# iden3/rapidsnark-old

Measured on AMD Instinct MI355X. Metric: Groth16 proofs/sec, higher is better.
Workload: dtype i64 (v_mad_i64_i32 column sums over 9x29-bit signed limbs, BN254 Fr/Fq)

## Files before the change

### include/zkhip.h

```cpp
#ifndef ZKHIP_H
#define ZKHIP_H

#include <stdint.h>
#include <stddef.h>

#ifdef __cplusplus
extern "C" {
#endif

typedef struct zk_prover zk_prover;

typedef struct zk_zkey_view {
    uint32_t nVars;
    uint32_t nPublic;
    uint32_t domainSize;
    uint64_t nCoefs;
    const void *vk_alpha1;
    const void *vk_beta1;
    const void *vk_beta2;
    const void *vk_delta1;
    const void *vk_delta2;
    const void *coefs;
    const void *pointsA;
    const void *pointsB1;
// ... 36 lines not shown

const char *zk_last_error(void);
int zk_device_count(int *count);

int zk_prover_create(zk_prover **out, const zk_zkey_view *zkey, const zk_opts *opts);
void zk_prover_destroy(zk_prover *p);

int zk_prove(zk_prover *p, const uint8_t *wtns, const uint8_t *r32, const uint8_t *s32, zk_proof *out);
int zk_prove_dev(zk_prover *p, const void *d_wtns, const uint8_t *r32, const uint8_t *s32, zk_proof *out);

#define ZK_MAX_IN_FLIGHT 8
int zk_prove_dev_submit(zk_prover *p, const void *d_wtns, const uint8_t *r32, const uint8_t *s32);
int zk_prove_submit(zk_prover *p, const uint8_t *wtns, const uint8_t *r32, const uint8_t *s32);
int zk_host_alloc(void **out, size_t bytes);
void zk_host_free(void *ptr);
int zk_prove_collect(zk_prover *p, zk_proof *out);
int zk_prover_reserve(zk_prover *p, uint32_t in_flight, uint32_t host_witnesses);
typedef struct zk_prover_plan {
    uint32_t size;
    uint32_t window_bits_h, windows_h;
    uint32_t window_bits_w, windows_w;
    uint32_t precomputed_tables;
    uint32_t msm_a_b1_c_one_launch;
    uint32_t lanes;
    uint32_t follow_up_streams;
    uint32_t max_in_flight;
    uint32_t depth_host_witness;
    uint32_t depth_resident_witness;
    uint32_t batch;
    uint32_t shard_index, shard_count, chain_partitioned;
    uint64_t device_bytes_in_use;
    uint64_t device_bytes_total;
    uint64_t kernel_launches_last_proof;
    uint32_t table_rows_h, table_rows_w;
    uint32_t bucket_sets_h, bucket_sets_w;
    uint32_t spmv_row_cut;
    uint32_t spmv_long_rows;
    uint32_t spmv_longest_row;
    uint32_t spmv_chunks;
} zk_prover_plan;
int zk_prover_info(zk_prover *p, zk_prover_plan *plan);
int zk_prove_msm_collect(zk_prover *p, zk_msm_sums *partial);
int zk_prove_batch_submit(zk_prover *p, const uint8_t *const *wtns, uint32_t count, const uint8_t *r32s, const uint8_t *s32s);
int zk_prove_batch_collect(zk_prover *p, zk_proof *out, uint32_t count);

int zk_prove_msm_dev(zk_prover *p, const void *d_wtns, zk_msm_sums *partial);
int zk_prove_msm(zk_prover *p, const uint8_t *wtns, zk_msm_sums *partial);
int zk_prove_finish(zk_prover *p, const zk_msm_sums *partials, uint32_t n_partials,
                    const uint8_t *r32, const uint8_t *s32, zk_proof *out);

typedef struct zk_multi_prover zk_multi_prover;
int zk_multi_prover_create(zk_multi_prover **out, const zk_zkey_view *zkey, const int32_t *devices, uint32_t n_devices,
                           const zk_opts *opts );
void zk_multi_prover_destroy(zk_multi_prover *mp);
int zk_multi_prove(zk_multi_prover *mp, const uint8_t *wtns, const uint8_t *r32, const uint8_t *s32, zk_proof *out);
int zk_multi_prove_submit(zk_multi_prover *mp, const uint8_t *wtns, const uint8_t *r32, const uint8_t *s32);
int zk_multi_prove_collect(zk_multi_prover *mp, zk_proof *out);
int zk_multi_prover_info(zk_multi_prover *mp, uint32_t *n_shards, uint32_t *chain_partitioned);
int zk_multi_prover_shard_info(zk_multi_prover *mp, uint32_t shard, zk_prover_plan *plan);
enum { ZK_STEP_CROSS_INVERSE = 1, ZK_STEP_LOCAL = 2, ZK_STEP_CROSS_FORWARD = 3, ZK_STEP_FINISH = 4 };
int zk_shard_info(zk_prover *p, uint64_t *block_elems, uint32_t *chain_partitioned);
int zk_shard_set_exchange(zk_prover *p, void *d_send, void *d_recv);
int zk_shard_begin(zk_prover *p, const uint8_t *wtns, const void *d_wtns, const uint8_t *r32, const uint8_t *s32, void *stream);
int zk_shard_step(zk_prover *p, int step, void *stream);

int zk_assemble(const void *vk_alpha1, const void *vk_beta1, const void *vk_beta2, const void *vk_delta1,
                const void *vk_delta2, const zk_msm_sums *partials, uint32_t n_partials,
                const uint8_t *r32, const uint8_t *s32, zk_proof *out);

enum {
    ZK_T_SPMV = 0, ZK_T_NTT, ZK_T_DIGITS_SORT, ZK_T_MSM_H, ZK_T_JOIN_WAIT, ZK_T_MSM_REDUCE,
    ZK_T_TOTAL_DEVICE, ZK_T_G1_L1_KERNEL, ZK_T_G2_L1_KERNEL, ZK_T_WTNS_H2D, ZK_T_COUNT
};
int zk_prover_timings(zk_prover *p, double *ms, uint32_t n);

int zk_fr_mul_vec(uint8_t *out, const uint8_t *a, const uint8_t *b, uint64_t n);
int zk_fq_mul_vec(uint8_t *out, const uint8_t *a, const uint8_t *b, uint64_t n);
int zk_fr_coef_accumulate(uint8_t *a, uint8_t *b, const void *coefs, uint64_t nCoefs, uint32_t domainSize,
                          const uint8_t *wtns, uint32_t nVars);
int zk_fr_ntt(uint8_t *data, uint64_t n, int inverse);
int zk_fr_abc_to_h(uint8_t *h, const uint8_t *a, const uint8_t *b, uint64_t n);
int zk_msm_g1(uint8_t out[64], const uint8_t *bases, const uint8_t *scalars, uint64_t n);
int zk_msm_g2(uint8_t out[128], const uint8_t *bases, const uint8_t *scalars, uint64_t n);

int zk_synth_chain_g1(uint8_t *out, uint64_t n, const uint8_t p0[64], const uint8_t q[64]);
int zk_synth_chain_g2(uint8_t *out, uint64_t n, const uint8_t p0[128], const uint8_t q[128]);
int zk_fixed_base_g1(uint8_t *out, const uint8_t base[64], const uint8_t *scalars, uint64_t n);
int zk_fixed_base_g2(uint8_t *out, const uint8_t base[128], const uint8_t *scalars, uint64_t n);
int zk_g1_mul(uint8_t out[64], const uint8_t p[64], const uint8_t k[32]);
int zk_g2_mul(uint8_t out[128], const uint8_t p[128], const uint8_t k[32]);

size_t zk_proof_to_json(const zk_proof *proof, char *buf, size_t cap);
size_t zk_public_to_json(const uint8_t *wtns, uint32_t nPublic, char *buf, size_t cap);

typedef struct zk_r1cs zk_r1cs;
typedef struct zk_r1cs_view {
    uint32_t nWires, nPubOut, nPubIn, nPrvIn, nConstraints;
    const void *constraints;
    uint64_t constraints_bytes;
} zk_r1cs_view;
typedef struct zk_r1cs_report {
    uint32_t size;
    uint64_t failed;
    uint32_t first_failed;
    uint8_t a[32], b[32], c[32];
    uint32_t one_ok;
    uint32_t first_unreduced;
} zk_r1cs_report;
int zk_r1cs_create(zk_r1cs **out, const zk_r1cs_view *v, int32_t device);
void zk_r1cs_destroy(zk_r1cs *r);
int zk_r1cs_check(zk_r1cs *r, const uint8_t *wtns, uint32_t nVars, zk_r1cs_report *rep);
int zk_r1cs_check_dev(zk_r1cs *r, const void *d_wtns, uint32_t nVars, zk_r1cs_report *rep);
int zk_r1cs_match_zkey(zk_r1cs *r, const zk_zkey_view *zkey, uint64_t *rows_differing, uint32_t *first_row);

typedef struct zk_ptau_view {
    uint32_t power;
    const void *alpha1, *beta1, *beta2;
    const void *lagrange_g1, *lagrange_g2, *lagrange_alpha_g1, *lagrange_beta_g1;
    uint64_t lagrange_g1_bytes, lagrange_g2_bytes, lagrange_alpha_g1_bytes, lagrange_beta_g1_bytes;
} zk_ptau_view;
typedef struct zk_setup_sizes {
    uint32_t nVars, nPublic, domainSize, log_domain;
    uint64_t nCoefs;
} zk_setup_sizes;
typedef struct zk_setup_out {
    uint8_t *coefs;
    uint8_t *pointsIC;
    uint8_t *pointsA;
    uint8_t *pointsB1;
    uint8_t *pointsB2;
    uint8_t *pointsC;
    uint8_t *pointsH;
} zk_setup_out;
int zk_groth16_setup_sizes(const zk_r1cs_view *r1cs, const zk_ptau_view *ptau, zk_setup_sizes *sizes);
int zk_groth16_setup(const zk_r1cs_view *r1cs, const zk_ptau_view *ptau, int32_t device, zk_setup_out *out);

int zk_g1_lagrange(uint8_t *out, const uint8_t *points, uint64_t n_points, uint32_t log_n, int32_t device);
int zk_g2_lagrange(uint8_t *out, const uint8_t *points, uint64_t n_points, uint32_t log_n, int32_t device);
typedef struct zk_ptau_powers_view {
    uint32_t power;
    const void *tau_g1, *tau_g2, *alpha_tau_g1, *beta_tau_g1;
    uint64_t tau_g1_bytes, tau_g2_bytes, alpha_tau_g1_bytes, beta_tau_g1_bytes;
} zk_ptau_powers_view;
typedef struct zk_ptau_lagrange_sizes {
    uint64_t lagrange_g1_bytes, lagrange_g2_bytes, lagrange_alpha_g1_bytes, lagrange_beta_g1_bytes;
    uint64_t device_bytes;
} zk_ptau_lagrange_sizes;
typedef struct zk_ptau_lagrange_out {
    uint8_t *lagrange_g1, *lagrange_g2, *lagrange_alpha_g1, *lagrange_beta_g1;
} zk_ptau_lagrange_out;
int zk_ptau_prepare_sizes(const zk_ptau_powers_view *ptau, zk_ptau_lagrange_sizes *sizes);
int zk_ptau_prepare(const zk_ptau_powers_view *ptau, int32_t device, zk_ptau_lagrange_out *out);

int zk_g1_scale(uint8_t *out, const uint8_t *points, uint64_t n, const uint8_t k[32], int32_t device);
#define ZK_SCALE_PLAN_MAX 130
int zk_g1_scale_plan(const uint8_t k[32], int8_t *digits_p, int8_t *digits_phi, uint32_t cap, uint32_t *len);
typedef struct zk_zkey_contrib_view {
    const void *vk_delta1;
    const void *vk_delta2;
    const void *pointsC;
    const void *pointsH;
    uint64_t pointsC_bytes, pointsH_bytes;
} zk_zkey_contrib_view;
typedef struct zk_zkey_contrib_sizes {
    uint64_t pointsC_bytes, pointsH_bytes;
    uint64_t chunk_points;
// ... 125 lines not shown
```

### rapidsnark-old_amd/csrc/hiputil.hpp

```cpp
#pragma once
#include <hip/hip_runtime.h>
#include <string.h>
#include <stdexcept>
#include <exception>
#include <string>
#include <thread>
#include <vector>

#include "../../include/zkhip.h"
#include "common.hpp"
#include "hipcheck.hpp"
#include "kernels.hpp"

using namespace zk;

namespace zkp {

#define HIP_TRY(expr) ZK_HIP(expr)

template <class T>
struct DevBuf {
    T *p = nullptr;
    size_t n = 0;
    DevBuf() {}
// ... 30 lines not shown
                (void)hipEventDestroy(done[i]);
            }
            if (pin[i]) (void)hipHostFree(pin[i]);
        }
    }
    void copy(void *dst, const void *src, size_t bytes) {
        if (!bytes) return;
        hipPointerAttribute_t attr;
        const bool pinned = hipPointerGetAttributes(&attr, src) == hipSuccess && attr.type == hipMemoryTypeHost;
        (void)hipGetLastError();
        if (pinned || bytes < ((size_t)4 << 20)) {
            HIP_TRY(hipMemcpyAsync(dst, src, bytes, hipMemcpyHostToDevice, s));
            return;
        }
        for (size_t off = 0; off < bytes; off += CHUNK, k ^= 1) {
            const size_t len = bytes - off < CHUNK ? bytes - off : CHUNK;
            if (!pin[k]) {
                HIP_TRY(hipHostMalloc((void **)&pin[k], CHUNK, hipHostMallocDefault));
                HIP_TRY(hipEventCreateWithFlags(&done[k], hipEventDisableTiming));
            } else {
                HIP_TRY(hipEventSynchronize(done[k]));
            }
            const uint8_t *from = (const uint8_t *)src + off;
            uint8_t *to = pin[k];
            const size_t nt = 4, per = (len / nt + 4095) & ~(size_t)4095;
            std::vector<std::thread> th;
            for (size_t t = 1; t < nt; t++) {
                const size_t lo = t * per, hi = lo + per < len ? lo + per : len;
                if (lo < hi) th.emplace_back([=] { memcpy(to + lo, from + lo, hi - lo); });
            }
            memcpy(to, from, per < len ? per : len);
            for (auto &t : th) t.join();
            HIP_TRY(hipMemcpyAsync((uint8_t *)dst + off, to, len, hipMemcpyHostToDevice, s));
            HIP_TRY(hipEventRecord(done[k], s));
        }
    }
};

struct Stream {
    hipStream_t s = nullptr;
    Stream() { HIP_TRY(hipStreamCreateWithFlags(&s, hipStreamNonBlocking)); }
    Stream(const Stream &) = delete;
    Stream &operator=(const Stream &) = delete;
    ~Stream() {
        (void)hipStreamSynchronize(s);
        (void)hipStreamDestroy(s);
    }
};

struct SortBufs {
    MsmPlan plan;
    uint64_t n = 0;
    DevBuf<uint16_t> lo;
    DevBuf<uint32_t> counts, starts, offsets, entries, codes, val, bin_counts, bin_starts;
    uint32_t total_buckets() const { return plan.sets * plan.nbuckets; }
    uint64_t max_entries() const { return (n ? n : 1) * plan.W; }
    void alloc(uint64_t n_, uint32_t window_bits, uint32_t precomp = 0, uint32_t batch = 1) {
        plan = make_msm_plan(n_ ? n_ : 1, window_bits, precomp, batch);
        n = n_ * (batch > 1 ? batch : 1);
        if ((n ? n : 1) * plan.W >= (1ull << 32)) throw std::invalid_argument("MSM too large: n * windows >= 2^32 sort entries");
        if ((n ? n : 1) * msm_table_rows(plan) >= (1ull << 31)) throw std::invalid_argument("MSM too large: table rows >= 2^31");
        MsmSortSizes z = msm_sort_sizes(n, plan);
        lo.alloc(z.lo_u16);
        counts.alloc(z.counts_u32);
        starts.alloc(z.starts_u32);
        offsets.alloc(z.offsets_u32);
        entries.alloc(z.entries_u32);
        codes.alloc(z.codes_u32);
        val.alloc(z.val_u32);
        bin_counts.alloc(z.bin_counts_u32);
        bin_starts.alloc(z.bin_starts_u32);
    }
    void release() {
        lo.release(); counts.release(); starts.release(); offsets.release(); entries.release();
        codes.release(); val.release(); bin_counts.release(); bin_starts.release();
        n = 0; ran = false;
    }
    size_t bytes() const {
        return lo.bytes() + counts.bytes() + starts.bytes() + offsets.bytes() + entries.bytes() + codes.bytes() + val.bytes()
             + bin_counts.bytes() + bin_starts.bytes();
    }
    bool ran = false;
    void run(const Fr *scalars, hipStream_t s) {
        static const bool skip = probe_env("ZKHIP_PROBE_SKIP_SORT") != nullptr;
        if (skip && ran) return;
        ran = true;
        MsmSortBufs b{offsets.p, entries.p, counts.p, starts.p, codes.p, val.p, bin_counts.p, bin_starts.p, lo.p};
        launch_msm_sort(b, scalars, n, plan, s);
    }
};

inline void need_device_count() {
    int ndev = 0;
    HIP_TRY(hipGetDeviceCount(&ndev));
    if (ndev <= 0) throw std::runtime_error("no HIP device available (libzkhip has no CPU fallback)");
}

inline int resolve_device(int32_t device) {
    need_device_count();
    int dev = device;
    if (dev < 0) HIP_TRY(hipGetDevice(&dev));
    return dev;
}

struct DeviceGuard {
    int prev = -1;
    explicit DeviceGuard(int dev) {
        if (hipGetDevice(&prev) != hipSuccess) prev = -1;
        HIP_TRY(hipSetDevice(dev));
    }
    ~DeviceGuard() {
        if (prev >= 0) (void)hipSetDevice(prev);
    }
};

inline void need_hbm(const char *who, uint64_t need) {
    size_t fr = 0, tot = 0;
    HIP_TRY(hipMemGetInfo(&fr, &tot));
    const uint64_t margin = need / 32 + ((uint64_t)256 << 20);
    if (fr < need + margin)
        throw HipError(std::string(who) + ": out of memory (needs " + std::to_string((need + margin) >> 20) + " MiB of HBM, " +
                       std::to_string(fr >> 20) + " MiB free)");
}

template <class Fn>
int guarded(Fn fn) {
    try {
        fn();
        return 0;
    } catch (const HipError &e) {
        set_error(std::string("HIP failure: ") + e.what());
        return 2;
    } catch (const std::exception &e) {
        set_error(e.what());
        return 1;
    }
}

inline uint32_t ilog2_exact(uint64_t n) {
    uint32_t l = 0;
    while ((1ull << l) < n) l++;
    if ((1ull << l) != n) throw std::invalid_argument("domainSize is not a power of two");
    return l;
}

inline uint32_t nblocks(uint64_t n, uint32_t b) { return (uint32_t)((n + b - 1) / b); }

inline void normalize(G1Affine *out, const G1XYZZ *tmp, Fq *pref, uint64_t n, hipStream_t s) { launch_normalize_g1(out, tmp, pref, n, s); }
inline void normalize(G2Affine *out, const G2XYZZ *tmp, Fq2 *pref, uint64_t n, hipStream_t s) { launch_normalize_g2(out, tmp, pref, n, s); }

}
using namespace zkp;
```

### rapidsnark-old_amd/csrc/kernels.hpp

```cpp
#pragma once
#include <hip/hip_runtime.h>
#include <stdint.h>
#include "field.hpp"
#include "curve.hpp"

namespace zk {

void launch_fr_mul_vec(Fr *out, const Fr *a, const Fr *b, uint64_t n, hipStream_t s);
void launch_fq_mul_vec(Fq *out, const Fq *a, const Fq *b, uint64_t n, hipStream_t s);

struct CsrDev {
    const uint32_t *rowptr;
    const uint32_t *col;
    const Fr *val;
    const uint4 *chunk_desc = nullptr;
    const uint4 *long_desc = nullptr;
    uint32_t chunks = 0, long_rows = 0, cut = 0;
};
constexpr uint32_t SPMV_LANE_TERMS = 16;
constexpr uint32_t SPMV_ROW_CUT = 16;
uint32_t spmv_row_cut();
void launch_spmv_abc(Fr *a, Fr *b, Fr *c, CsrDev csr, const Fr *wtns, uint32_t n, hipStream_t s, uint32_t vectors = 1, uint64_t abc_stride = 0,
                     uint64_t wtns_stride = 0, Fr *partials = nullptr);
void launch_csr_build(uint32_t *rowptr, uint32_t *col, Fr *val, uint32_t *cursor, uint32_t *err, const uint8_t *records,
                      uint64_t nCoefs, uint32_t n, uint32_t nVars, uint32_t row_lo, uint32_t row_hi, uint32_t row_cut, hipStream_t s);
void launch_csr_long_rows(uint4 *long_desc, uint4 *chunk_desc, uint32_t *counters, const uint32_t *rowptr, uint32_t rows, uint32_t row_cut,
                          uint32_t long_rows, uint32_t chunks, hipStream_t s);
void launch_exclusive_scan_u32(uint32_t *out, const uint32_t *counts, uint32_t total, hipStream_t s);

struct TwEntry {
    uint32_t l[12];
};
struct NttTables {
    uint32_t logn;
    const TwEntry *fwd;
    const TwEntry *inv;
    const Fr *coset;
    const Fr *ninv;
};
struct NttPair {
    uint32_t L = 0, Lg = 0, m = 0;
    uint32_t ngroups = 0, g[2] = {0, 0};
    TwEntry *rfwd = nullptr, *rinv = nullptr;
    Fr *tinv = nullptr, *tfwd = nullptr, *dtab = nullptr, *t2inv = nullptr, *t2fwd = nullptr;
    NttPair() {}
    NttPair(const NttPair &) = delete;
    NttPair &operator=(const NttPair &) = delete;
    ~NttPair() { release(); }
    void build(uint32_t logn_global, uint32_t logn_local, uint32_t block_index, hipStream_t s, bool plain = false);
    void release();
};
bool ntt_pair_supported(uint32_t local_logn);
void launch_ntt_coset_pair(Fr *data, uint64_t stride_elems, uint32_t batch, const NttPair &t, hipStream_t s);
void launch_ntt_plain(Fr *out, Fr *data, uint64_t stride_elems, uint32_t batch, const NttPair &t, bool inverse, hipStream_t s);

void launch_ntt_build_tables(TwEntry *fwd, TwEntry *inv, Fr *coset, Fr *ninv, uint32_t logn, hipStream_t s);
#define NTT_FULL 0xffffffffu
void launch_ntt_dif_inverse(Fr *data, uint64_t stride_elems, uint32_t batch, const NttTables &t, hipStream_t s, uint32_t local_logn = NTT_FULL);
void launch_ntt_dit_forward(Fr *data, uint64_t stride_elems, uint32_t batch, const NttTables &t, hipStream_t s, const Fr *premul = nullptr,
                            uint32_t local_logn = NTT_FULL);
void launch_ntt_cross(bool inverse, const Fr *xb, uint64_t in_src_stride, uint64_t in_poly_stride, Fr *const out_base[8],
                      uint64_t out_poly_stride, uint64_t out_offset, uint32_t batch,
                      const NttTables &t, uint32_t log_shards, uint32_t rank, hipStream_t s);
void launch_chunk_scatter(Fr *const xb_of_gpu[8], const Fr *blockdata, uint32_t batch, uint32_t logn, uint32_t log_shards, uint32_t rank,
                          hipStream_t s);
void launch_chunk_pack(Fr *packed, const Fr *blockdata, uint32_t batch, uint32_t logn, uint32_t log_shards, hipStream_t s);
void launch_chunk_unpack(Fr *blockdata, const Fr *packed, uint32_t batch, uint32_t logn, uint32_t log_shards, hipStream_t s);
void launch_fr_to_internal(Fr *x, uint64_t n, int times, hipStream_t s);
void launch_fr_from_internal(Fr *x, uint64_t n, hipStream_t s);
void launch_fr_scale_by_table(Fr *data, uint64_t stride_elems, uint32_t batch, const Fr *table, uint64_t n, hipStream_t s);
void launch_fr_scale_const(Fr *data, const Fr *k, uint64_t n, hipStream_t s);
void launch_bitrev_permute(Fr *data, uint32_t logn, hipStream_t s);
void launch_abc_to_h(Fr *h, const Fr *a, const Fr *b, const Fr *c, uint64_t n, hipStream_t s, uint32_t vectors = 1, uint64_t abc_stride = 0);

struct MsmPlan {
    uint32_t c;
    uint32_t W;
    uint32_t nbuckets;
    uint32_t sets;
    uint32_t precomp;
    uint32_t batch;
    uint32_t batch_n;
};
MsmPlan make_msm_plan(uint64_t n, uint32_t window_bits, uint32_t precomp = 0, uint32_t batch = 1);
inline uint32_t msm_table_rows(const MsmPlan &p) { return p.precomp ? (p.W + p.precomp - 1) / p.precomp : 1u; }

struct MsmSortSizes {
    uint64_t counts_u32, starts_u32, offsets_u32, entries_u32;
    uint64_t codes_u32, lo_u16, val_u32, bin_counts_u32, bin_starts_u32;
};
struct MsmSortBufs {
    uint32_t *offsets, *entries;
    uint32_t *counts, *starts;
    uint32_t *codes, *val, *bin_counts, *bin_starts;
    uint16_t *lo;
};
MsmSortSizes msm_sort_sizes(uint64_t n, MsmPlan p);
uint32_t msm_scan_extra_words(uint32_t total);
void launch_msm_sort(const MsmSortBufs &b, const Fr *scalars, uint64_t n, MsmPlan p, hipStream_t s);
void launch_msm_precomp_g1(G1Affine *table, G1XYZZ *tmp, Fq *pref, uint64_t n, MsmPlan p, hipStream_t s);
void launch_msm_precomp_g2(G2Affine *table, G2XYZZ *tmp, Fq2 *pref, uint64_t n, MsmPlan p, hipStream_t s);
struct alignas(16) G1Acc {
    int32_t l[36];
};
struct alignas(16) G2Acc {
    int32_t l[72];
};
uint64_t msm_accum_workspace_slots(uint64_t max_entries);
struct AccumTail {
    hipStream_t stream = nullptr;
    hipEvent_t l1_done = nullptr;
    bool buckets_zeroed = false;
    uint32_t chunk_min = 0;
    uint32_t chunk_max = 0;
};
struct AccumBatch {
    uint32_t n;
    const void *points[3];
    uint32_t idx_min[3], idx_sub[3];
    uint64_t bucket_stride, ws_stride;
    uint32_t gather_mask;
};
void launch_msm_accum_g1_batch(G1Acc *buckets, const uint32_t *offsets, const uint32_t *entries, const AccumBatch &batch, uint32_t total_buckets,
                               uint64_t max_entries, G1Acc *ws_part, uint32_t *ws_key, uint32_t *ws_flag, hipStream_t s, hipEvent_t *ev = nullptr,
                               AccumTail tail = AccumTail());
void launch_msm_accum_g1(G1Acc *buckets, const uint32_t *offsets, const uint32_t *entries, const G1Affine *points,
                         uint32_t idx_min, uint32_t idx_sub, uint32_t total_buckets, uint64_t max_entries,
                         G1Acc *ws_part, uint32_t *ws_key, uint32_t *ws_flag, hipStream_t s, hipEvent_t *ev = nullptr,
                         AccumTail tail = AccumTail());
void launch_msm_accum_g2(G2Acc *buckets, const uint32_t *offsets, const uint32_t *entries, const G2Affine *points,
                         uint32_t idx_min, uint32_t idx_sub, uint32_t total_buckets, uint64_t max_entries,
                         G2Acc *ws_part, uint32_t *ws_key, uint32_t *ws_flag, hipStream_t s, hipEvent_t *ev = nullptr,
                         AccumTail tail = AccumTail());
void launch_msm_reduce_g1(G1XYZZ *window_sums, G1Acc *scratch, const G1Acc *buckets, uint32_t n_msm, MsmPlan p, hipStream_t s);
void launch_msm_reduce_g2(G2XYZZ *window_sums, G2Acc *scratch, const G2Acc *buckets, uint32_t n_msm, MsmPlan p, hipStream_t s);
uint64_t msm_reduce_scratch_points(uint32_t n_msm, MsmPlan p);
uint32_t msm_wsum_rc(MsmPlan p);

void launch_fq_to_internal(Fq *coords, uint64_t n, hipStream_t s);

void launch_chain_g1(G1Affine *d_out, G1XYZZ *d_tmp, Fq *d_pref, const G1Affine &P0, const G1Affine &Q, uint64_t n, hipStream_t s);
void launch_chain_g2(G2Affine *d_out, G2XYZZ *d_tmp, Fq2 *d_pref, const G2Affine &P0, const G2Affine &Q, uint64_t n, hipStream_t s);
void launch_normalize_g1(G1Affine *d_out, const G1XYZZ *d_tmp, Fq *d_pref, uint64_t n, hipStream_t s);
void launch_normalize_g2(G2Affine *d_out, const G2XYZZ *d_tmp, Fq2 *d_pref, uint64_t n, hipStream_t s);
void launch_fixed_base_g1(G1Affine *d_out, G1XYZZ *d_tmp, Fq *d_pref, const G1Affine &B, const uint32_t *d_scalars, uint64_t n, hipStream_t s);
void launch_fixed_base_g2(G2Affine *d_out, G2XYZZ *d_tmp, Fq2 *d_pref, const G2Affine &B, const uint32_t *d_scalars, uint64_t n, hipStream_t s);

}
```

### rapidsnark-old_amd/csrc/msm_accum.hip

```cpp
#include <stdlib.h>
#include <string.h>
#include <algorithm>
#include "hipcheck.hpp"
#include "msm_lanes.hpp"

namespace zk {

#define ACC_CHUNK_MAX 160u
#define ACC_CHUNK_MIN 32u
__device__ __forceinline__ uint32_t accum_chunk_dev(uint32_t E, uint32_t nlanes, uint32_t chunk_min) {
    const uint32_t c = (uint32_t)(((uint64_t)E + nlanes - 1) / nlanes);
    return c < chunk_min ? chunk_min : c;
}
#ifdef ZK_PROBES
#define ZK_GATHER_ROW(i) ((i) & batch.gather_mask)
#else
#define ZK_GATHER_ROW(i) (i)
#endif
#define ACC_CHUNK_N 32u
#ifndef ZK_L1_BLOCK
#define ZK_L1_BLOCK 256
#endif
#ifndef ZK_L1_PREFETCH
#define ZK_L1_PREFETCH 1
// ... 274 lines not shown
        if (!__any(take)) break;
        XYZZ<FR> o{wave_up(v.x, d * LPE), wave_up(v.y, d * LPE), wave_up(v.zz, d * LPE), wave_up(v.zzz, d * LPE)};
        if (take) add(v, o);
    }
    if (e >= cnt) return;
    const uint32_t knext = __shfl_down(key, LPE);
    const uint32_t kbefore = __shfl_up(key, LPE);
    const bool last = e + 1 == cnt || knext != key;
    const bool first = e == 0 || kbefore != key;
    const uint64_t fmask = __ballot(first);
    const uint32_t start_lane = 63u - (uint32_t)__clzll(fmask & ((2ull << lane) - 1ull));
    const uint32_t sflag = (uint32_t)__shfl((int)flag, (int)start_lane);
    if (!last) return;
    const bool starts = (sflag & FLAG_STARTS) != 0, ends = (flag & FLAG_ENDS) != 0;
    if (starts && ends) {
        LM::store(buckets + key, v);
    } else if (!starts) {
        LM::store(out_part + 2 * (uint64_t)w, v);
        if (comp == 0) {
            out_key[2 * (uint64_t)w] = key;
            out_flag[2 * (uint64_t)w] = ends ? FLAG_ENDS : 0u;
        }
    } else {
        LM::store(out_part + 2 * (uint64_t)w + 1, v);
        if (comp == 0) {
            out_key[2 * (uint64_t)w + 1] = key;
            out_flag[2 * (uint64_t)w + 1] = FLAG_STARTS;
        }
    }
}

static inline uint32_t accum_chunk_min() {
    static const uint32_t cmin = [] { const char *e = probe_env("ZKHIP_ACC_CHUNK_MIN"); uint32_t v = e ? (uint32_t)atoi(e) : ACC_CHUNK_MIN; return v < 4u ? 4u : v; }();
    return cmin;
}
static inline uint32_t accum_chunk_max() {
    static const uint32_t cmax = [] { const char *e = probe_env("ZKHIP_ACC_CHUNK_MAX"); uint32_t v = e ? (uint32_t)atoi(e) : ACC_CHUNK_MAX; return v < 8u ? 8u : v; }();
    return cmax;
}
template <class F>
static uint64_t accum_round_lanes(uint32_t n_msm) {
    static const uint64_t threads = [] {
        int dev = 0, cus = 256, wgs = 0;
        hipError_t e = hipGetDevice(&dev);
        if (e == hipSuccess) e = hipDeviceGetAttribute(&cus, hipDeviceAttributeMultiprocessorCount, dev);
        if (e == hipSuccess) {
            if constexpr (sizeof(F) == sizeof(Fq2)) e = hipOccupancyMaxActiveBlocksPerMultiprocessor(&wgs, k_msm_accum_l1_g2s, ZK_L1_BLOCK, 0);
            else e = hipOccupancyMaxActiveBlocksPerMultiprocessor(&wgs, k_msm_accum_l1<F>, ZK_L1_BLOCK, 0);
        }
        if (e != hipSuccess || wgs < 1) { (void)hipGetLastError(); wgs = (sizeof(F) == sizeof(Fq2) ? 2 : 3) * (256 / ZK_L1_BLOCK); }
        if (const char *o = probe_env("ZKHIP_ACC_ROUND_WGS")) wgs = atoi(o) > 0 ? atoi(o) : wgs;
        return (uint64_t)wgs * (uint64_t)ZK_L1_BLOCK * (uint64_t)cus;
    }();
    uint64_t lanes = threads / LaneModel<F>::LPE / (n_msm ? n_msm : 1);
    return lanes ? lanes : 1;
}
template <class F>
static inline uint64_t accum_lanes_for(uint64_t max_entries, uint32_t n_msm, uint32_t chunk_min = 0, uint32_t chunk_max = 0) {
    if (!max_entries) max_entries = 1;
    const uint64_t R = accum_round_lanes<F>(n_msm), cmin = chunk_min ? chunk_min : accum_chunk_min(), cmax = chunk_max ? chunk_max : accum_chunk_max();
    if (max_entries <= R * cmin) return (max_entries + cmin - 1) / cmin;
    const uint64_t rounds = (max_entries + R * cmax - 1) / (R * cmax);
    return rounds * R;
}
uint64_t msm_accum_workspace_slots(uint64_t max_entries) {
    uint64_t lanes = accum_lanes_for<Fq>(max_entries, 1);
    for (uint32_t nb = 2; nb <= 3; nb++) lanes = std::max(lanes, accum_lanes_for<Fq>(max_entries, nb));
    lanes = std::max(lanes, accum_lanes_for<Fq2>(max_entries, 1));
    uint64_t total = 0;
    for (;;) {
        uint64_t slots = 2 * lanes;
        total += slots;
        if (lanes == 1) break;
        lanes = (slots + ACC_CHUNK_N - 1) / ACC_CHUNK_N;
    }
    return total;
}

template <class F>
static void launch_accum(ACCMEM *buckets, const uint32_t *offsets, const uint32_t *entries, AccumBatch batch,
                         uint32_t total_buckets, uint64_t max_entries,
                         ACCMEM *ws_part, uint32_t *ws_key, uint32_t *ws_flag, hipStream_t s, hipEvent_t *ev, AccumTail tail) {
    const uint32_t nb = batch.n ? batch.n : 1;
    if (!tail.buckets_zeroed) ZK_HIP(hipMemsetAsync(buckets, 0, ((size_t)(nb - 1) * batch.bucket_stride + total_buckets) * sizeof(ACCMEM), s));
    const uint32_t cmin = tail.chunk_min > accum_chunk_min() ? tail.chunk_min : accum_chunk_min();
    uint64_t lanes = accum_lanes_for<F>(max_entries, nb, cmin, tail.chunk_max > accum_chunk_max() ? tail.chunk_max : 0u);
    if (ev) ZK_HIP(hipEventRecord(ev[0], s));
    if constexpr (sizeof(F) == sizeof(Fq2)) {
        ZK_LAUNCH(k_msm_accum_l1_g2s, dim3((uint32_t)((2 * lanes + ZK_L1_BLOCK - 1) / ZK_L1_BLOCK)), dim3(ZK_L1_BLOCK), 0, s, buckets, offsets, entries,
                           reinterpret_cast<const G2Affine *>(batch.points[0]), batch.idx_min[0], batch.idx_sub[0], total_buckets, ws_part, ws_key, ws_flag,
                           (uint32_t)lanes, cmin);
    } else {
        ZK_LAUNCH(k_msm_accum_l1<F>, dim3((uint32_t)((lanes + ZK_L1_BLOCK - 1) / ZK_L1_BLOCK), nb), dim3(ZK_L1_BLOCK), 0, s, buckets, offsets, entries,
                           batch, total_buckets, ws_part, ws_key, ws_flag, (uint32_t)lanes, cmin);
    }
    if (ev) ZK_HIP(hipEventRecord(ev[1], s));
    if (skip_followups_probe()) return;
    if (tail.stream && tail.stream != s) {
        ZK_HIP(hipEventRecord(tail.l1_done, s));
        ZK_HIP(hipStreamWaitEvent(tail.stream, tail.l1_done, 0));
        s = tail.stream;
    }
    if (lanes > 1)
        ZK_LAUNCH(k_msm_accum_pair<F>, dim3((uint32_t)((lanes * LaneModel<F>::LPE + 255) / 256), nb), dim3(256), 0, s, buckets,
                           (const ACCMEM *)ws_part, ws_key, (const uint32_t *)ws_flag, (uint32_t)lanes, batch.bucket_stride, batch.ws_stride);
    uint64_t off = 0;
    while (lanes > 1) {
        uint64_t items = 2 * lanes;
        uint64_t noff = off + items;
        const uint64_t epw = 64u / LaneModel<F>::LPE;
        const uint64_t nl = (items + epw - 1) / epw;
        ZK_LAUNCH(k_msm_accum_wave<F>, dim3((uint32_t)((nl + 3) / 4), nb), dim3(256), 0, s, buckets, ws_part + off,
                           ws_key + off, ws_flag + off, (uint32_t)items, ws_part + noff, ws_key + noff, ws_flag + noff, (uint32_t)nl,
                           batch.bucket_stride, batch.ws_stride);
        off = noff;
        lanes = nl;
    }
    ZK_LAUNCH_OK("msm bucket accumulation");
}

static uint32_t gather_mask_env() {
    static const uint32_t m = [] { const char *e = probe_env("ZKHIP_GATHER_MASK"); return e ? (uint32_t)strtoul(e, nullptr, 0) : 0xffffffffu; }();
    return m;
}
static AccumBatch single(const void *points, uint32_t idx_min, uint32_t idx_sub) {
    AccumBatch b;
    memset(&b, 0, sizeof b);
    b.n = 1;
    b.gather_mask = gather_mask_env();
    b.points[0] = points;
    b.idx_min[0] = idx_min;
    b.idx_sub[0] = idx_sub;
    return b;
}

void launch_msm_accum_g1(G1Acc *buckets, const uint32_t *offsets, const uint32_t *entries, const G1Affine *points,
                         uint32_t idx_min, uint32_t idx_sub, uint32_t total, uint64_t max_entries, G1Acc *ws_part,
                         uint32_t *ws_key, uint32_t *ws_flag, hipStream_t s, hipEvent_t *ev, AccumTail tail) {
    launch_accum<Fq>(buckets, offsets, entries, single(points, idx_min, idx_sub), total, max_entries, ws_part, ws_key, ws_flag, s, ev, tail);
}
void launch_msm_accum_g1_batch(G1Acc *buckets, const uint32_t *offsets, const uint32_t *entries, const AccumBatch &batch, uint32_t total,
                               uint64_t max_entries, G1Acc *ws_part, uint32_t *ws_key, uint32_t *ws_flag, hipStream_t s, hipEvent_t *ev,
                               AccumTail tail) {
    AccumBatch b = batch;
    b.gather_mask = gather_mask_env();
    launch_accum<Fq>(buckets, offsets, entries, b, total, max_entries, ws_part, ws_key, ws_flag, s, ev, tail);
}
void launch_msm_accum_g2(G2Acc *buckets, const uint32_t *offsets, const uint32_t *entries, const G2Affine *points,
                         uint32_t idx_min, uint32_t idx_sub, uint32_t total, uint64_t max_entries, G2Acc *ws_part,
                         uint32_t *ws_key, uint32_t *ws_flag, hipStream_t s, hipEvent_t *ev, AccumTail tail) {
    launch_accum<Fq2>(buckets, offsets, entries, single(points, idx_min, idx_sub), total, max_entries, ws_part, ws_key, ws_flag, s, ev, tail);
}

}
```

### rapidsnark-old_amd/csrc/msm_reduce.hip

```cpp
#include <stdlib.h>
#include "hipcheck.hpp"
#include "msm_lanes.hpp"

namespace zk {

#define REDUCE_CHUNK 16u
#define REDUCE_THREADS 256u

template <class F>
__global__ __launch_bounds__(128) void k_msm_reduce_split(ACCMEM *A, uint32_t a_stride, ACCMEM *T, const ACCMEM *buckets, uint32_t nbuckets, uint32_t chunk, uint32_t L) {
    ZK_TAIL_PRIO();
    typedef LaneModel<F> LM;
    typedef typename LM::R FR;
    const uint32_t t = (blockIdx.x * blockDim.x + threadIdx.x) / LM::LPE;
    if (t >= L) return;
    const ACCMEM *B = buckets + (uint64_t)blockIdx.y * nbuckets + (uint64_t)t * chunk;
    XYZZ<FR> run = XYZZ<FR>::inf(), sum = XYZZ<FR>::inf();
    for (int j = (int)chunk - 1; j >= 0; j--) {
        add(run, LM::load(B + j));
        add(sum, run);
    }
    LM::store(A + (uint64_t)blockIdx.y * a_stride + t, sum);
    if (t == 0) run = XYZZ<FR>::inf();
    LM::store(T + (uint64_t)blockIdx.y * L + (t ? t - 1 : L - 1), run);
}

template <class F>
__global__ __launch_bounds__(128) void k_msm_reduce_chunks(ACCMEM *scratch, uint32_t out_stride, const ACCMEM *buckets, uint32_t nbuckets,
                                                           uint32_t chunk, uint32_t total_chunks) {
    ZK_TAIL_PRIO();
    typedef LaneModel<F> LM;
    typedef typename LM::R FR;
    uint32_t t = (blockIdx.x * blockDim.x + threadIdx.x) / LM::LPE;
    if (t >= total_chunks) return;
    const uint32_t chunks_per_window = nbuckets / chunk;
    const uint32_t cw = t % chunks_per_window;
    const ACCMEM *B = buckets + (uint64_t)t * chunk;
    XYZZ<FR> run = XYZZ<FR>::inf(), sum = XYZZ<FR>::inf();
    for (int j = (int)chunk - 1; j >= 0; j--) {
        add(run, LM::load(B + j));
        add(sum, run);
    }
    uint32_t k = cw * chunk;
    if (k) {
        XYZZ<FR> m = XYZZ<FR>::inf();
        for (int bit = 31 - __clz(k); bit >= 0; bit--) {
            m = dbl(m);
            if ((k >> bit) & 1u) add(m, run);
        }
        add(sum, m);
    }
    LM::store(scratch + (uint64_t)(t / chunks_per_window) * out_stride + cw, sum);
}

template <class F>
static constexpr uint32_t tree_in() { return 2u * REDUCE_THREADS / LaneModel<F>::LPE; }
#define TREE_IN_MIN REDUCE_THREADS
template <class F>
__global__ __launch_bounds__(REDUCE_THREADS) void k_msm_reduce_tree(ACCMEM *out, XYZZ<F> *out_final, const ACCMEM *in, uint32_t count, uint32_t last) {
    ZK_TAIL_PRIO();
    extern __shared__ uint32_t lds_raw[];
    typedef LaneModel<F> LM;
    typedef typename LM::R FR;
    constexpr uint32_t NE = REDUCE_THREADS / LM::LPE;
    XYZZ<FR> *lds = reinterpret_cast<XYZZ<FR> *>(lds_raw);
    const ACCMEM *X = in + (uint64_t)blockIdx.y * count;
    const uint32_t e = threadIdx.x / LM::LPE;
    const uint32_t i0 = blockIdx.x * (2u * NE) + e, i1 = i0 + NE;
    XYZZ<FR> acc = XYZZ<FR>::inf();
    if (i0 < count) acc = LM::load(X + i0);
    if (i1 < count) add(acc, LM::load(X + i1));
    lds[threadIdx.x] = acc;
    __syncthreads();
    for (uint32_t s = NE / 2; s > 0; s >>= 1) {
        if (e < s) {
            XYZZ<FR> o = lds[threadIdx.x + s * LM::LPE];
            add(acc, o);
            lds[threadIdx.x] = acc;
        }
        __syncthreads();
    }
    if (e == 0) {
        const uint64_t at = (uint64_t)blockIdx.y * gridDim.x + blockIdx.x;
        if (last) LM::store256(out_final + at, acc);
        else LM::store(out + at, acc);
    }
}

template <class F>
__global__ __launch_bounds__(REDUCE_THREADS) void k_msm_reduce_final2(XYZZ<F> *out_final, const ACCMEM *P, uint32_t cnt_x, uint32_t cnt_a, uint32_t scale_log) {
    ZK_TAIL_PRIO();
    extern __shared__ uint32_t lds_raw[];
    typedef LaneModel<F> LM;
    typedef typename LM::R FR;
    constexpr uint32_t H = REDUCE_THREADS / LM::LPE / 2;
    XYZZ<FR> *lds = reinterpret_cast<XYZZ<FR> *>(lds_raw);
    const uint32_t e = threadIdx.x / LM::LPE;
    const bool xs = e >= H;
    const uint32_t eh = xs ? e - H : e, cnt = xs ? cnt_x : cnt_a;
    const ACCMEM *in = P + (uint64_t)blockIdx.x * (cnt_x + cnt_a) + (xs ? 0u : cnt_x);
    XYZZ<FR> acc = XYZZ<FR>::inf();
    if (eh < cnt) acc = LM::load(in + eh);
// ... 57 lines not shown
        if (nblk == 1) LM::store256(final_out + (uint64_t)group * c + e, v);
        else LM::store(rec + ((uint64_t)group * nblk + blk) * BITS_RS + e, v);
    }
}
template <class F>
__global__ __launch_bounds__(REDUCE_THREADS) void k_msm_reduce_bits_top(XYZZ<F> *final_out, ACCMEM *rec, uint32_t nblk, uint32_t c) {
    ZK_TAIL_PRIO();
    typedef LaneModel<F> LM;
    typedef typename LM::R FR;
    constexpr uint32_t NE = REDUCE_THREADS / LM::LPE;
    constexpr uint32_t LB = LM::LPE == 1 ? 8u : 7u;
    const uint32_t e = threadIdx.x / LM::LPE;
    ACCMEM *R0 = rec + (uint64_t)blockIdx.x * nblk * BITS_RS;
#pragma unroll 1
    for (uint32_t m = LB; m + 1 < c; m++) {
        const uint32_t span = 1u << (m - LB), per = m + 2, ntasks = (nblk >> (m - LB + 1)) * per;
#pragma unroll 1
        for (uint32_t t = e; t < ntasks; t += NE) {
            const uint32_t g = t / per, i = t % per;
            ACCMEM *L = R0 + (uint64_t)g * 2u * span * BITS_RS, *R = L + (uint64_t)span * BITS_RS;
            if (i <= m) {
                XYZZ<FR> a = LM::load(L + i);
                add(a, LM::load(R + i));
                LM::store(L + i, a);
            } else {
                LM::store(L + m + 1, LM::load(R));
            }
        }
        __threadfence_block();
        __syncthreads();
    }
    if (e < c) LM::store256(final_out + (uint64_t)blockIdx.x * c + e, LM::load(R0 + e));
}
static inline bool reduce_bits_for(MsmPlan p) {
    static const int forced = [] { const char *e = probe_env("ZKHIP_REDUCE_BITS"); return e ? atoi(e) : -1; }();
    if (p.c > BITS_RS || (uint64_t)p.sets * p.nbuckets > (1u << 16)) return false;
    return forced < 0 ? true : forced != 0;
}
uint32_t msm_wsum_rc(MsmPlan p) { return reduce_bits_for(p) ? p.c : 1u; }

static inline uint32_t reduce_chunk_for(MsmPlan p) {
    static const uint32_t forced = [] { const char *e = probe_env("ZKHIP_REDUCE_CHUNK"); return e ? (uint32_t)atoi(e) : 0u; }();
    uint32_t chunk = REDUCE_CHUNK;
    if (forced) chunk = forced;
    else if ((uint64_t)p.sets * p.nbuckets <= (1u << 16)) chunk = 4;
    return p.nbuckets < chunk ? p.nbuckets : chunk;
}

#define REDUCE_SPLIT 16u
static inline uint32_t reduce_split_top(uint32_t L) {
    static const uint32_t forced = [] { const char *e = probe_env("ZKHIP_REDUCE_SPLIT_TOP"); const uint32_t t = e ? (uint32_t)atoi(e) : 0u; return t >= 2u && (t & (t - 1)) == 0 ? t : 0u; }();
    if (forced) return forced;
    return (L / 8u) % (2u * REDUCE_THREADS) == 0 ? 8u : 4u;
}
static inline uint32_t reduce_split_for(MsmPlan p) {
    static const int forced = [] { const char *e = probe_env("ZKHIP_REDUCE_SPLIT"); return e ? atoi(e) : -1; }();
    if (reduce_bits_for(p) || p.nbuckets < (1u << 14)) return 0;
    const uint32_t ch = forced >= 0 ? (uint32_t)forced : (p.nbuckets > (REDUCE_SPLIT << 15) ? p.nbuckets >> 15 : REDUCE_SPLIT);
    if (ch < 2 || (ch & (ch - 1)) != 0 || ch > p.nbuckets) return 0;
    const uint32_t L = p.nbuckets / ch;
    return L >= 8u && (L / reduce_split_top(L)) % (2u * REDUCE_THREADS) == 0 && L / TREE_IN_MIN <= REDUCE_THREADS / 2u ? ch : 0u;
}

static inline uint64_t tree_points(uint64_t groups, uint64_t cnt) {
    uint64_t total = 0;
    for (;;) {
        total += groups * cnt;
        if (cnt == 1) break;
        cnt = (cnt + TREE_IN_MIN - 1) / TREE_IN_MIN;
    }
    return total + groups;
}
uint64_t msm_reduce_scratch_points(uint32_t n_msm, MsmPlan p) {
    if (reduce_bits_for(p)) return (uint64_t)n_msm * p.sets * (p.nbuckets / 128u + 1u) * BITS_RS;
    const uint64_t groups = (uint64_t)n_msm * p.sets;
    if (const uint32_t ch = reduce_split_for(p)) {
        const uint64_t L = p.nbuckets / ch;
        return groups * L + tree_points(groups, L / reduce_split_top((uint32_t)L) + L);
    }
    return tree_points(groups, p.nbuckets / reduce_chunk_for(p));
}

template <class F>
static void launch_reduce(XYZZ<F> *window_sums, ACCMEM *scratch, const ACCMEM *buckets, uint32_t n_msm, MsmPlan p, hipStream_t s) {
    if (skip_followups_probe()) return;
    if (reduce_bits_for(p)) {
        const uint32_t NE = REDUCE_THREADS / LaneModel<F>::LPE, groups = n_msm * p.sets;
        const uint32_t nblk = p.nbuckets > NE ? p.nbuckets / NE : 1u;
        const size_t lds = REDUCE_THREADS * sizeof(XYZZ<typename LaneModel<F>::R>);
        ZK_LAUNCH(k_msm_reduce_bits_block<F>, dim3(nblk, groups), dim3(REDUCE_THREADS), lds, s, scratch, window_sums, buckets, p.nbuckets, p.c, nblk);
        if (nblk > 1) ZK_LAUNCH(k_msm_reduce_bits_top<F>, dim3(groups), dim3(REDUCE_THREADS), 0, s, window_sums, scratch, nblk, p.c);
        ZK_LAUNCH_OK("msm bucket reduction (bit sums)");
        return;
    }
    const uint32_t groups = n_msm * p.sets;
    const size_t lds = REDUCE_THREADS * sizeof(XYZZ<typename LaneModel<F>::R>);
    const uint32_t TREE_IN = tree_in<F>();
    auto chunks = [&](ACCMEM *out, uint32_t out_stride, const ACCMEM *in, uint32_t n, uint32_t chunk) {
        const uint32_t total_chunks = groups * (n / chunk);
        ZK_LAUNCH(k_msm_reduce_chunks<F>, dim3((total_chunks * LaneModel<F>::LPE + 127) / 128), dim3(128), 0, s, out, out_stride, in, n, chunk, total_chunks);
    };
    if (const uint32_t ch = reduce_split_for(p)) {
        const uint32_t L = p.nbuckets / ch, top = reduce_split_top(L), nx = L / top, per = nx + L;
        ACCMEM *T = scratch, *Y = T + (uint64_t)groups * L, *P = Y + (uint64_t)groups * per;
        ZK_LAUNCH(k_msm_reduce_split<F>, dim3((L * LaneModel<F>::LPE + 127) / 128, groups), dim3(128), 0, s, Y + nx, per, T, buckets, p.nbuckets, ch, L);
        chunks(Y, per, T, L, top);
        const uint32_t bx = nx / TREE_IN, ba = L / TREE_IN;
        ZK_LAUNCH(k_msm_reduce_tree<F>, dim3(bx + ba, groups), dim3(REDUCE_THREADS), lds, s, P, window_sums, (const ACCMEM *)Y, per, 0u);
        ZK_LAUNCH(k_msm_reduce_final2<F>, dim3(groups), dim3(REDUCE_THREADS), lds, s, window_sums, (const ACCMEM *)P, bx, ba, (uint32_t)__builtin_ctz(ch));
        ZK_LAUNCH_OK("msm bucket reduction (split)");
        return;
    }
    const uint32_t chunk = reduce_chunk_for(p);
    uint32_t cnt = p.nbuckets / chunk;
    chunks(scratch, cnt, buckets, p.nbuckets, chunk);
    ACCMEM *in = scratch;
    for (;;) {
        const uint32_t blocks = (cnt + TREE_IN - 1) / TREE_IN;
        const bool last = blocks == 1;
        ACCMEM *out = in + (uint64_t)groups * cnt;
        ZK_LAUNCH(k_msm_reduce_tree<F>, dim3(blocks, groups), dim3(REDUCE_THREADS), lds, s, out, window_sums, (const ACCMEM *)in, cnt, last ? 1u : 0u);
        if (last) break;
        in = out;
        cnt = blocks;
    }
    ZK_LAUNCH_OK("msm bucket reduction");
}
void launch_msm_reduce_g1(G1XYZZ *ws, G1Acc *scratch, const G1Acc *buckets, uint32_t n_msm, MsmPlan p, hipStream_t s) {
    launch_reduce<Fq>(ws, scratch, buckets, n_msm, p, s);
}
void launch_msm_reduce_g2(G2XYZZ *ws, G2Acc *scratch, const G2Acc *buckets, uint32_t n_msm, MsmPlan p, hipStream_t s) {
    launch_reduce<Fq2>(ws, scratch, buckets, n_msm, p, s);
}

}
```

### rapidsnark-old_amd/csrc/msm_sort.hip

```cpp
#include "kernels.hpp"
#include "hipcheck.hpp"
#include "common.hpp"
#include "devmem.hpp"
#include <string.h>

namespace zk {

MsmPlan make_msm_plan(uint64_t n, uint32_t window_bits, uint32_t precomp, uint32_t batch) {
    if (precomp > 2) throw std::invalid_argument("table mode: 0 (as in the zkey), 1 (a row per window) or 2 (a row per second window)");
    MsmPlan p;
    uint32_t lg = 0;
    while ((1ull << (lg + 1)) <= n) lg++;
    uint32_t c = window_bits;
    if (precomp) {
        if (c == 0) {
            c = lg > 2 ? lg - 2 : 2;
            if (lg == 20) c = 19;
            if (lg == 21) c = 20;
            if (batch > 1) c++;
            if (c > 20) c = 20;
        }
        if (c > 22) c = 22;
    } else {
        if (c == 0) c = lg > 6 ? lg - 6 : 2;
        if (c > 16) c = 16;
    }
    if (c < 2) c = 2;
    p.c = c;
    p.W = (256 + c - 1) / c;
    {
        const uint32_t W255 = (255 + c - 1) / c;
        if (W255 < p.W) {
            const uint32_t sh = (W255 - 1) * c;
            uint64_t top = 0;
            for (int k = 7; k >= 0; k--) {
                const int lo_bit = 32 * k;
                if (lo_bit + 32 <= (int)sh) break;
                const uint64_t w = FrParams::P[k];
                top |= lo_bit >= (int)sh ? w << (lo_bit - sh) : w >> (sh - lo_bit);
            }
            if (top + 1 < (1ull << (c - 1))) p.W = W255;
        }
    }
    p.nbuckets = 1u << (c - 1);
    p.precomp = precomp;
    p.sets = precomp ? precomp : p.W;
    p.batch = 1;
    p.batch_n = 0;
    if (batch > 1) {
        if (precomp != 1) throw std::invalid_argument("batched MSMs need window-precomputed tables with a row per window");
        p.batch = batch;
        p.batch_n = (uint32_t)n;
        p.sets = batch;
    }
    return p;
}

#define CODE32_ZERO 0x7FFFFFFFu
#ifndef SORT_THREADS
#define SORT_THREADS 1024u
#endif

__global__ __launch_bounds__(256) void k_msm_digits(uint32_t *digits, const Fr *scalars, uint64_t n, MsmPlan p) {
    ZK_CHAIN_PRIO();
    uint64_t st = (uint64_t)gridDim.x * blockDim.x;
    const uint32_t c = p.c, W = p.W;
    const uint32_t mask = (1u << c) - 1u, half = 1u << (c - 1);
    const uint32_t set_stride = p.precomp == 1 ? 0u : p.nbuckets, set_mask = p.precomp == 2 ? 1u : 0xffffffffu;
    for (uint64_t i = (uint64_t)blockIdx.x * blockDim.x + threadIdx.x; i < n; i += st) {
        Fr s = load_el(scalars + i);
        const uint32_t vec_base = p.batch > 1 ? (uint32_t)(i / p.batch_n) * p.nbuckets : 0u;
        for (int k = 0; k < 6; k++) {
            Fr d;
            u32 bw = 0;
#pragma unroll
            for (int j = 0; j < 8; j++) d.v[j] = subb(s.v[j], FrParams::P[j], bw);
            if (bw) break;
            s = d;
        }
        uint64_t buf = 0;
        uint32_t nb = 0, w = 0, carry = 0;
        auto emit = [&](uint32_t raw) {
            uint32_t d = raw + carry;
            const bool neg = d >= half;
            carry = neg ? 1u : 0u;
            uint32_t mag = neg ? (1u << c) - d : d;
            uint32_t code = mag ? ((mag - 1u + (w & set_mask) * set_stride + vec_base) | (neg ? 0x80000000u : 0u)) : CODE32_ZERO;
            digits[(uint64_t)w * n + i] = code;
            w++;
        };
#pragma unroll
        for (int k = 0; k < 8; k++) {
            buf |= (uint64_t)s.v[k] << nb;
            nb += 32;
            while (nb >= c && w + 1 < W) {
                emit((uint32_t)buf & mask);
                buf >>= c;
                nb -= c;
            }
        }
        emit((uint32_t)buf & mask);
    }
}

__global__ __launch_bounds__(256) void k_msm_compact_offsets(uint32_t *offsets, const uint32_t *starts, uint32_t total, uint32_t slices) {
    ZK_CHAIN_PRIO();
    uint32_t k = blockIdx.x * blockDim.x + threadIdx.x;
    if (k <= total) offsets[k] = starts[(uint64_t)k * slices];
}

#define BIN_MAX 256u

__global__ __launch_bounds__(SORT_THREADS) void k_bin_count(uint32_t *bin_counts, const uint32_t *codes, uint64_t total, uint32_t nbins,
                                                            uint32_t nblocks, uint32_t shift, uint32_t span) {
    ZK_CHAIN_PRIO();
    __shared__ uint32_t hist[BIN_MAX];
    if (threadIdx.x < BIN_MAX) hist[threadIdx.x] = 0;
    __syncthreads();
    const uint64_t base = (uint64_t)blockIdx.x * span;
    for (uint32_t k = threadIdx.x; k < span; k += SORT_THREADS) {
        uint64_t i = base + k;
        if (i < total) {
            uint32_t code = codes[i];
            if ((code & 0x7FFFFFFFu) != CODE32_ZERO) atomicAdd(&hist[(code & 0x7FFFFFFFu) >> shift], 1u);
        }
    }
    __syncthreads();
    if (threadIdx.x < nbins) bin_counts[(uint64_t)threadIdx.x * nblocks + blockIdx.x] = hist[threadIdx.x];
}

#define BIN_ITEMS 8u
__global__ __launch_bounds__(SORT_THREADS) void k_bin_scatter(uint16_t *lo, uint32_t *val, const uint32_t *bin_starts, const uint32_t *codes,
                                                              uint64_t total, uint32_t nbins, uint32_t nblocks, uint32_t shift, uint32_t span, uint64_t n,
                                                              uint32_t set_shift, uint32_t batch_n, uint32_t tstride) {
    ZK_CHAIN_PRIO();
    extern __shared__ uint32_t smem[];
    uint32_t *cnt = smem;
    uint32_t *gdelta = smem + BIN_MAX;
    uint32_t *st_dst = smem + 2 * BIN_MAX;
    uint32_t *st_val = st_dst + span;
    uint16_t *st_lo = (uint16_t *)(st_val + span);
    const uint32_t tid = threadIdx.x;
    if (tid < BIN_MAX) cnt[tid] = 0;
    __syncthreads();
    const uint64_t base = (uint64_t)blockIdx.x * span;
    const uint32_t lomask = (1u << shift) - 1u;
    const uint64_t w_base = tstride > 1 && n ? base / n : 0, r_base = tstride > 1 && n ? base - w_base * n : 0;
    uint32_t code[BIN_ITEMS], rank[BIN_ITEMS];
#pragma unroll
    for (uint32_t k = 0; k < BIN_ITEMS; k++) {
        uint64_t i = base + (uint64_t)k * SORT_THREADS + tid;
        code[k] = i < total ? codes[i] : CODE32_ZERO;
    }
#pragma unroll
    for (uint32_t k = 0; k < BIN_ITEMS; k++) {
        uint32_t mag = code[k] & 0x7FFFFFFFu;
        rank[k] = mag != CODE32_ZERO ? atomicAdd(&cnt[mag >> shift], 1u) : 0u;
    }
    __syncthreads();
    if (tid < 64) {
        uint32_t c0 = cnt[4 * tid], c1 = cnt[4 * tid + 1], c2 = cnt[4 * tid + 2], c3 = cnt[4 * tid + 3];
        uint32_t sum = c0 + c1 + c2 + c3, x = sum;
#pragma unroll
        for (int d = 1; d < 64; d <<= 1) {
            uint32_t y = __shfl_up(x, d);
            if (tid >= (uint32_t)d) x += y;
        }
        uint32_t off = x - sum;
        uint32_t o[4] = {off, off + c0, off + c0 + c1, off + c0 + c1 + c2};
#pragma unroll
        for (int q = 0; q < 4; q++) {
            uint32_t bin = 4 * tid + q;
            cnt[bin] = o[q];
            gdelta[bin] = bin < nbins ? bin_starts[(uint64_t)bin * nblocks + blockIdx.x] - o[q] : 0u;
        }
        if (tid == 63) smem[2 * BIN_MAX + 2 * span + span / 2] = x;
    }
    __syncthreads();
#pragma unroll
    for (uint32_t k = 0; k < BIN_ITEMS; k++) {
        uint32_t mag = code[k] & 0x7FFFFFFFu;
        if (mag != CODE32_ZERO) {
            uint32_t bin = mag >> shift, slot = cnt[bin] + rank[k];
            uint64_t i = base + (uint64_t)k * SORT_THREADS + tid - (uint64_t)(set_shift < 32 ? mag >> set_shift : 0u) * n;
            if (tstride > 1) {
                uint64_t w = w_base, r = r_base + (uint64_t)k * SORT_THREADS + tid;
                while (n && r >= n) { r -= n; w++; }
                i = (w / tstride) * n + r;
            }
            if (batch_n) {
                const uint64_t j = i / n, r = (i % n) % batch_n;
                i = j * batch_n + r;
            }
            st_dst[slot] = slot + gdelta[bin];
            st_val[slot] = (uint32_t)i | (code[k] & 0x80000000u);
            st_lo[slot] = (uint16_t)(mag & lomask);
        }
    }
    __syncthreads();
    const uint32_t kept = smem[2 * BIN_MAX + 2 * span + span / 2];
    for (uint32_t sidx = tid; sidx < kept; sidx += SORT_THREADS) {
        uint32_t d = st_dst[sidx];
        val[d] = st_val[sidx];
        lo[d] = st_lo[sidx];
    }
}

__device__ __forceinline__ bool bin_slice_of_block(uint32_t nbins, uint32_t slices, uint32_t &bin, uint32_t &slice) {
    const uint32_t xcd = blockIdx.x & 7u, k = blockIdx.x >> 3;
    bin = (k / slices) * 8u + xcd;
    slice = k % slices;
    return bin < nbins;
}

// ... 145 lines not shown
        }
#pragma unroll
        for (uint32_t k = 0; k < PER; k++) rank[k] = key[k] != 0xFFFFFFFFu ? atomicAdd(&loc[key[k]], 1u) : 0u;
        __syncthreads();
        const uint32_t c0 = loc[2 * tid], c1 = loc[2 * tid + 1];
        uint32_t total;
        const uint32_t ex = block_exclusive_scan(c0 + c1, scan_lds, total);
        __syncthreads();
        loc[2 * tid] = ex;
        loc[2 * tid + 1] = ex + c0;
        __syncthreads();
#pragma unroll
        for (uint32_t k = 0; k < PER; k++) {
            if (key[k] != 0xFFFFFFFFu) {
                const uint32_t pos = loc[key[k]] + rank[k];
                sval[pos] = v[k];
                slo[pos] = (uint16_t)key[k];
            }
        }
        __syncthreads();
        for (uint32_t p = tid; p < cnt; p += SCAN_BLOCK) {
            const uint32_t kk = slo[p];
            entries[gcur[kk] + (p - loc[kk])] = sval[p];
        }
        __syncthreads();
        const uint32_t a0 = loc[2 * tid], a1 = loc[2 * tid + 1], a2 = 2 * tid + 2 < 2048u ? loc[2 * tid + 2] : cnt;
        gcur[2 * tid] += a1 - a0;
        gcur[2 * tid + 1] += a2 - a1;
        __syncthreads();
    }
}

static void launch_scan(uint32_t *out, const uint32_t *counts, uint32_t total, hipStream_t s) {
    uint32_t nblocks = (total + SCAN_ELEMS - 1) / SCAN_ELEMS;
    uint32_t *block_sums = out + total + 1;
    ZK_LAUNCH(k_scan_local, dim3(nblocks), dim3(SCAN_BLOCK), 0, s, out, block_sums, counts, total);
    ZK_LAUNCH(k_scan_sums, dim3(1), dim3(SCAN_BLOCK), 0, s, block_sums, nblocks, out + total);
    ZK_LAUNCH(k_scan_add, dim3(nblocks), dim3(SCAN_BLOCK), 0, s, out, (const uint32_t *)block_sums, total);
}
uint32_t msm_scan_extra_words(uint32_t total) { return (total + SCAN_ELEMS - 1) / SCAN_ELEMS; }
void launch_exclusive_scan_u32(uint32_t *out, const uint32_t *counts, uint32_t total, hipStream_t s) { launch_scan(out, counts, total, s); }

#define BIN_SHIFT 11u
#define BIN_SLICES 32u
static inline uint32_t plan_total_buckets(MsmPlan p) { return p.sets * p.nbuckets; }
static inline uint32_t plan_bin_shift(MsmPlan p) {
    uint32_t sh = BIN_SHIFT;
    while (((plan_total_buckets(p) + (1u << sh) - 1) >> sh) > BIN_MAX) sh++;
    return sh;
}
static inline uint32_t plan_nbins(MsmPlan p) { uint32_t sh = plan_bin_shift(p); return (plan_total_buckets(p) + (1u << sh) - 1) >> sh; }
static inline uint32_t bin_span() { return BIN_ITEMS * SORT_THREADS; }
static inline uint32_t plan_bin_blocks(uint64_t n, MsmPlan p) { return (uint32_t)(((n ? n : 1) * p.W + bin_span() - 1) / bin_span()); }

MsmSortSizes msm_sort_sizes(uint64_t n, MsmPlan p) {
    MsmSortSizes z;
    memset(&z, 0, sizeof z);
    const uint64_t tb = plan_total_buckets(p), items = (n ? n : 1) * p.W;
    const uint64_t bb = (uint64_t)plan_nbins(p) * plan_bin_blocks(n, p);
    z.counts_u32 = tb * BIN_SLICES;
    z.starts_u32 = tb * BIN_SLICES + 1 + msm_scan_extra_words((uint32_t)(tb * BIN_SLICES));
    z.offsets_u32 = tb + 1;
    z.entries_u32 = items;
    z.codes_u32 = items;
    z.lo_u16 = items;
    z.val_u32 = items;
    z.bin_counts_u32 = bb;
    z.bin_starts_u32 = bb + 1 + msm_scan_extra_words((uint32_t)bb);
    return z;
}

static inline size_t bin_scatter_lds_bytes() { return (size_t)(2 * BIN_MAX + 2 * bin_span() + bin_span() / 2 + 1) * 4; }
static void sort_lds_attr() {
    static PerDeviceOnce attr;
    if (!attr.need()) return;
    ZK_HIP(hipFuncSetAttribute((const void *)k_bin_count_lds, hipFuncAttributeMaxDynamicSharedMemorySize, 160 * 1024));
    ZK_HIP(hipFuncSetAttribute((const void *)k_bin_scatter_lds, hipFuncAttributeMaxDynamicSharedMemorySize, 160 * 1024));
    ZK_HIP(hipFuncSetAttribute((const void *)k_bin_scatter, hipFuncAttributeMaxDynamicSharedMemorySize, 160 * 1024));
    ZK_HIP(hipFuncSetAttribute((const void *)k_bin_scatter_staged, hipFuncAttributeMaxDynamicSharedMemorySize, 160 * 1024));
    attr.done();
}

void launch_msm_sort(const MsmSortBufs &b, const Fr *scalars, uint64_t n, MsmPlan p, hipStream_t s) {
    const uint32_t tb = plan_total_buckets(p);
    sort_lds_attr();
    uint64_t g = (n + 255) / 256;
    if (g > 8192) g = 8192;
    const uint32_t sh = plan_bin_shift(p), nbins = plan_nbins(p), nblocks = plan_bin_blocks(n, p);
    uint32_t slices = BIN_SLICES;
    {
        const uint64_t per_bin = (n * p.W) / (nbins ? nbins : 1);
        while (slices > 4u && per_bin / slices < STAGE_CAP * 3u / 4u) slices >>= 1;
    }
    const uint32_t bpb = tb < (1u << sh) ? tb : (1u << sh);
    const uint64_t total = n * p.W;
    const size_t lds = (size_t)bpb * 4;
    const uint32_t grid2 = ((nbins + 7u) / 8u) * 8u * slices;
    const uint32_t set_shift = p.precomp ? 32u : p.c - 1u;
    if (n) ZK_LAUNCH(k_msm_digits, dim3((uint32_t)g), dim3(256), 0, s, b.codes, scalars, n, p);
    ZK_LAUNCH(k_bin_count, dim3(nblocks), dim3(SORT_THREADS), 0, s, b.bin_counts, (const uint32_t *)b.codes, total, nbins, nblocks, sh, bin_span());
    launch_scan(b.bin_starts, b.bin_counts, nbins * nblocks, s);
    ZK_LAUNCH(k_bin_scatter, dim3(nblocks), dim3(SORT_THREADS), bin_scatter_lds_bytes(), s, b.lo, b.val, (const uint32_t *)b.bin_starts,
                       (const uint32_t *)b.codes, total, nbins, nblocks, sh, bin_span(), n, set_shift, p.batch > 1 ? p.batch_n : 0u, p.precomp);
    ZK_LAUNCH(k_bin_count_lds, dim3(grid2), dim3(SORT_THREADS), lds, s, b.counts, (const uint16_t *)b.lo,
                       (const uint32_t *)b.bin_starts, nblocks, bpb, nbins, slices, tb);
    launch_scan(b.starts, b.counts, tb * slices, s);
    static const bool direct = probe_env("ZKHIP_SORT_DIRECT") != nullptr;
    if (bpb <= 2048u && SORT_THREADS == SCAN_BLOCK && !direct)
        ZK_LAUNCH(k_bin_scatter_staged, dim3(grid2), dim3(SCAN_BLOCK), (size_t)(4096 + 16 + STAGE_CAP) * 4 + (size_t)STAGE_CAP * 2, s, b.entries,
                           (const uint32_t *)b.starts, (const uint16_t *)b.lo, (const uint32_t *)b.val, (const uint32_t *)b.bin_starts, nblocks, bpb, nbins,
                           slices, tb);
    else
        ZK_LAUNCH(k_bin_scatter_lds, dim3(grid2), dim3(SORT_THREADS), lds, s, b.entries, (const uint32_t *)b.starts,
                           (const uint16_t *)b.lo, (const uint32_t *)b.val, (const uint32_t *)b.bin_starts, nblocks, bpb, nbins, slices, tb);
    ZK_LAUNCH(k_msm_compact_offsets, dim3((tb + 256) / 256), dim3(256), 0, s, b.offsets, (const uint32_t *)b.starts, tb, slices);
    ZK_LAUNCH_OK("msm sort");
}

}
```

### rapidsnark-old_amd/csrc/operators.hip

```cpp
#include <map>
#include <memory>
#include <mutex>
#include "hiputil.hpp"
#include "csr_long.hpp"

static void need_device() { need_device_count(); }

template <class F>
static void mul_vec(uint8_t *out, const uint8_t *a, const uint8_t *b, uint64_t n, void (*launch)(F *, const F *, const F *, uint64_t, hipStream_t)) {
    need_device();
    if (!n) return;
    DevBuf<F> da, db;
    da.alloc(n);
    db.alloc(n);
    da.upload(a, n, 0);
    db.upload(b, n, 0);
    launch(da.p, da.p, db.p, n, 0);
    HIP_TRY(hipMemcpy(out, da.p, n * 32, hipMemcpyDeviceToHost));
}

struct Tables {
    DevBuf<TwEntry> fwd, inv;
    DevBuf<Fr> coset, ninv;
    NttTables t;
// ... 154 lines not shown
    const uint64_t emax = sb.max_entries(), slots = msm_accum_workspace_slots(emax);
    ws.alloc(slots);
    wkey.alloc(slots);
    wflag.alloc(slots);
    buckets.alloc(sb.total_buckets());
    scratch.alloc(msm_reduce_scratch_points(1, sb.plan));
    const uint32_t rc = msm_wsum_rc(sb.plan);
    wsum.alloc((uint64_t)sb.plan.sets * rc);
    std::vector<uint8_t> w((size_t)sb.plan.sets * rc * sizeof(XT));
    if constexpr (sizeof(AffT) == 64) {
        launch_msm_accum_g1((G1Acc *)buckets.p, sb.offsets.p, sb.entries.p, (const G1Affine *)pts.p, 0, 0, sb.total_buckets(), emax, (G1Acc *)ws.p, wkey.p, wflag.p, 0);
        launch_msm_reduce_g1((G1XYZZ *)wsum.p, (G1Acc *)scratch.p, (const G1Acc *)buckets.p, 1, sb.plan, 0);
    } else {
        launch_msm_accum_g2((G2Acc *)buckets.p, sb.offsets.p, sb.entries.p, (const G2Affine *)pts.p, 0, 0, sb.total_buckets(), emax, (G2Acc *)ws.p, wkey.p, wflag.p, 0);
        launch_msm_reduce_g2((G2XYZZ *)wsum.p, (G2Acc *)scratch.p, (const G2Acc *)buckets.p, 1, sb.plan, 0);
    }
    HIP_TRY(hipMemcpy(w.data(), wsum.p, w.size(), hipMemcpyDeviceToHost));
    if (g2) HostTail::combine_windows_g2(w.data(), sb.plan.sets, sb.plan.c, rc, out);
    else HostTail::combine_windows_g1(w.data(), sb.plan.sets, sb.plan.c, rc, out);
}

template <class AffT, class XT, class FT>
static void synth_chain(uint8_t *out, uint64_t n, const uint8_t *p0, const uint8_t *q,
                        void (*launch)(AffT *, XT *, FT *, const AffT &, const AffT &, uint64_t, hipStream_t)) {
    need_device();
    if (!n) return;
    DevBuf<AffT> d_out;
    DevBuf<XT> d_tmp;
    DevBuf<FT> d_pref;
    d_out.alloc(n);
    d_tmp.alloc(n);
    d_pref.alloc(n);
    AffT P0, Q;
    memcpy(&P0, p0, sizeof(AffT));
    memcpy(&Q, q, sizeof(AffT));
    launch(d_out.p, d_tmp.p, d_pref.p, P0, Q, n, 0);
    HIP_TRY(hipMemcpy(out, d_out.p, n * sizeof(AffT), hipMemcpyDeviceToHost));
}

template <class AffT, class XT, class FT>
static void fixed_base_batch(uint8_t *out, const uint8_t *base, const uint8_t *scalars, uint64_t n,
                             void (*launch)(AffT *, XT *, FT *, const AffT &, const uint32_t *, uint64_t, hipStream_t)) {
    need_device();
    if (!n) return;
    if (!out || !base || !scalars) throw std::invalid_argument("null argument");
    DevBuf<AffT> d_out;
    DevBuf<XT> d_tmp;
    DevBuf<FT> d_pref;
    DevBuf<uint32_t> d_sc;
    d_out.alloc(n);
    d_tmp.alloc(n);
    d_pref.alloc(n);
    d_sc.alloc(n * 8);
    AffT B;
    memcpy(&B, base, sizeof(AffT));
    HIP_TRY(hipMemcpy(d_sc.p, scalars, n * 32, hipMemcpyHostToDevice));
    launch(d_out.p, d_tmp.p, d_pref.p, B, d_sc.p, n, 0);
    HIP_TRY(hipMemcpy(out, d_out.p, n * sizeof(AffT), hipMemcpyDeviceToHost));
}

extern "C" {

int zk_fixed_base_g1(uint8_t *out, const uint8_t base[64], const uint8_t *scalars, uint64_t n) {
    return guarded([&] { fixed_base_batch<G1Affine, G1XYZZ, Fq>(out, base, scalars, n, launch_fixed_base_g1); });
}
int zk_fixed_base_g2(uint8_t *out, const uint8_t base[128], const uint8_t *scalars, uint64_t n) {
    return guarded([&] { fixed_base_batch<G2Affine, G2XYZZ, Fq2>(out, base, scalars, n, launch_fixed_base_g2); });
}

int zk_synth_chain_g1(uint8_t *out, uint64_t n, const uint8_t p0[64], const uint8_t q[64]) {
    return guarded([&] { synth_chain<G1Affine, G1XYZZ, Fq>(out, n, p0, q, launch_chain_g1); });
}
int zk_synth_chain_g2(uint8_t *out, uint64_t n, const uint8_t p0[128], const uint8_t q[128]) {
    return guarded([&] { synth_chain<G2Affine, G2XYZZ, Fq2>(out, n, p0, q, launch_chain_g2); });
}

int zk_msm_g1(uint8_t out[64], const uint8_t *bases, const uint8_t *scalars, uint64_t n) {
    return guarded([&] { msm_generic<G1Affine, G1XYZZ, G1Acc>(out, bases, scalars, n, false); });
}
int zk_msm_g2(uint8_t out[128], const uint8_t *bases, const uint8_t *scalars, uint64_t n) {
    return guarded([&] { msm_generic<G2Affine, G2XYZZ, G2Acc>(out, bases, scalars, n, true); });
}

}
```

### rapidsnark-old_amd/csrc/prover_create.hip

```cpp
#include "prover_internal.hpp"

__attribute__((constructor)) static void zk_default_hw_queues() { setenv("GPU_MAX_HW_QUEUES", "16", 0); }

namespace zkp {

void alloc_slot(zk_prover *p, int i) {
    zk_prover::ProofSlot &q = p->slot[i];
    if (q.allocated) return;
    const uint64_t nv = p->sv.size();
    q.sort_w.alloc(nv, p->wbits, p->table_mode, p->batch);
    const MsmPlan pw = q.sort_w.plan, ph = p->sort_h.plan;
    const uint64_t tbw = q.sort_w.total_buckets(), tbh = p->sort_h.total_buckets();
    q.buckets_g1.alloc(3 * tbw + tbh);
    q.buckets_g2.alloc(tbw);
    q.scratch_g1.alloc(msm_reduce_scratch_points(3, pw) + msm_reduce_scratch_points(1, ph));
    const uint64_t ew = (uint64_t)pw.sets * msm_wsum_rc(pw), eh = (uint64_t)ph.sets * msm_wsum_rc(ph);
    q.wsum_g1.alloc(3 * ew + eh);
    q.scratch_g2.alloc(msm_reduce_scratch_points(1, pw));
    q.wsum_g2.alloc(ew);
    const uint64_t slots = msm_accum_workspace_slots(q.sort_w.max_entries()), slots_h = msm_accum_workspace_slots(p->sort_h.max_entries());
    q.acc_stride = slots;
    q.acc_ws_g1_all.alloc(3 * slots + slots_h);
    q.acc_ws_g2.alloc(slots);
    q.acc_key_all.alloc(4 * slots + slots_h);
    q.acc_flag_all.alloc(4 * slots + slots_h);
    if (p->csr_long.chunks) q.spmv_part.alloc((uint64_t)p->csr_long.chunks * p->batch);
    for (int m = 0; m < 5; m++) {
        const uint64_t at = m < 3 ? m * slots : (m == 3 ? 3 * slots : 3 * slots + slots_h);
        if (m < 4) q.acc_ws_g1[m] = q.acc_ws_g1_all.p + at;
        q.acc_key[m] = q.acc_key_all.p + at;
        q.acc_flag[m] = q.acc_flag_all.p + at;
    }
    q.w1_bytes = (size_t)(3 * ew + eh) * sizeof(G1XYZZ);
    q.w2_bytes = (size_t)ew * sizeof(G2XYZZ);
    if (!q.w1) HIP_TRY(hipHostMalloc((void **)&q.w1, q.w1_bytes, hipHostMallocDefault));
    if (!q.w2) HIP_TRY(hipHostMalloc((void **)&q.w2, q.w2_bytes, hipHostMallocDefault));
    for (auto &e : q.ev_l1)
        if (!e) HIP_TRY(hipEventCreateWithFlags(&e, hipEventDisableTiming));
    for (hipEvent_t *e : {&q.ev_fork, &q.ev_join, &q.ev_sortw, &q.ev_main, &q.ev_done, &q.ev_chain})
        if (!*e) HIP_TRY(hipEventCreateWithFlags(e, hipEventDisableTiming));
    for (auto &e : q.ev_tail)
        if (!e) HIP_TRY(hipEventCreateWithFlags(&e, hipEventDisableTiming));
    for (auto &e : q.ev)
        if (!e) HIP_TRY(hipEventCreate(&e));
    q.have_events = true;
    q.allocated = true;
}

void ensure_witness_buffer(zk_prover *p, zk_prover::ProofSlot &q) {
    if (!q.wtns_dev.p) q.wtns_dev.alloc((uint64_t)p->nVars * p->batch);
    if (!q.ev_h2d) HIP_TRY(hipEventCreateWithFlags(&q.ev_h2d, hipEventDisableTiming));
    if (!q.ev_h2d_start) HIP_TRY(hipEventCreate(&q.ev_h2d_start));
}

struct PhaseClock {
    bool on;
    std::chrono::steady_clock::time_point t;
    PhaseClock() : on(getenv("ZKHIP_VERBOSE") != nullptr), t(std::chrono::steady_clock::now()) {}
    void lap(const char *what, hipStream_t s) {
        if (!on) return;
        (void)hipStreamSynchronize(s);
        auto now = std::chrono::steady_clock::now();
        fprintf(stderr, "[zkhip] create: %-28s %8.1f ms\n", what, std::chrono::duration<double, std::milli>(now - t).count());
        t = now;
    }
};

void prover_create(zk_prover **out, const zk_zkey_view *z, const zk_opts *o) {
    if (!out || !z) throw std::invalid_argument("null argument");
    PhaseClock clk;
    const int dev = resolve_device(o ? o->device : -1);
    std::unique_ptr<zk_prover> p(new zk_prover());
    p->device = dev;
    DeviceGuard g(dev);
    p->flags = o ? o->flags : 0;
    p->shard_count = (o && o->shard_count > 1) ? o->shard_count : 1;
    p->shard_index = o ? o->shard_index : 0;
    p->batch = (o && o->batch > 1) ? o->batch : 1;
    if (p->batch > ZK_MAX_BATCH) throw std::invalid_argument("opts.batch > ZK_MAX_BATCH");
    if (p->flags & ZK_FLAG_PRECOMP_HALF) p->flags |= ZK_FLAG_PRECOMP;
    if (p->batch > 1 && (!(p->flags & ZK_FLAG_PRECOMP) || (p->flags & ZK_FLAG_PRECOMP_HALF) || p->shard_count != 1 || (p->flags & ZK_FLAG_PARTITIONED_CHAIN)))
        throw std::invalid_argument("opts.batch needs ZK_FLAG_PRECOMP (a row per window) on an unsharded prover");
    if (p->shard_index >= p->shard_count) throw std::invalid_argument("shard_index >= shard_count");
    const uint32_t wbits = o ? o->window_bits : 0;

    p->nVars = z->nVars;
    p->nPublic = z->nPublic;
    p->domainSize = z->domainSize;
    p->nCoefs = z->nCoefs;
    if (z->nVars == 0 || z->nPublic + 1 > z->nVars) throw std::invalid_argument("invalid nVars/nPublic");
    p->logn = ilog2_exact(z->domainSize);
    if (p->logn > 27) throw std::invalid_argument("domainSize exceeds 2^27: the coset needs a root of order 2*domainSize and BN254 Fr has 2-adicity 28");
    if (z->nCoefs >= (1ull << 32)) throw std::invalid_argument("nCoefs >= 2^32 is not supported (32-bit CSR positions)");
    const uint64_t n = z->domainSize, nV = z->nVars, nC = nV - z->nPublic - 1;
    if (z->coefs_bytes && z->coefs_bytes < 4 + z->nCoefs * 44) throw std::invalid_argument("zkey section 4 too small");
    if (z->pointsA_bytes && z->pointsA_bytes < nV * 64) throw std::invalid_argument("zkey section 5 too small");
    if (z->pointsB1_bytes && z->pointsB1_bytes < nV * 64) throw std::invalid_argument("zkey section 6 too small");
    if (z->pointsB2_bytes && z->pointsB2_bytes < nV * 128) throw std::invalid_argument("zkey section 7 too small");
    if (z->pointsC_bytes && z->pointsC_bytes < nC * 64) throw std::invalid_argument("zkey section 8 too small");
    if (z->pointsH_bytes && z->pointsH_bytes < n * 64) throw std::invalid_argument("zkey section 9 too small");
    memcpy(p->vk_alpha1, z->vk_alpha1, 64);
    memcpy(p->vk_beta1, z->vk_beta1, 64);
    memcpy(p->vk_beta2, z->vk_beta2, 128);
    memcpy(p->vk_delta1, z->vk_delta1, 64);
    memcpy(p->vk_delta2, z->vk_delta2, 128);

    {
        const char *e = probe_env("ZKHIP_S1_PRIO");
        const bool s1_hi = e ? atoi(e) != 0 : p->shard_count >= 2;
        if (s1_hi && !getenv("ZKHIP_SERIAL")) {
            int lo_pr = 0, hi_pr = 0;
            HIP_TRY(hipDeviceGetStreamPriorityRange(&lo_pr, &hi_pr));
            HIP_TRY(hipStreamCreateWithPriority(&p->stream, hipStreamNonBlocking, hi_pr));
        } else {
            HIP_TRY(hipStreamCreateWithFlags(&p->stream, hipStreamNonBlocking));
        }
    }
    struct SideStreams {
        std::thread th;
        std::exception_ptr err;
        ~SideStreams() {
            if (th.joinable()) th.join();
// ... 67 lines not shown
        if (nnz) up.copy(raw.p, (const uint8_t *)z->coefs + 4, nnz * 44);
        clk.lap("coefficient records upload", s);
        launch_csr_build(p->csr_rowptr.p, p->csr_col.p, p->csr_val.p, cursor.p, err.p, raw.p, nnz, z->domainSize, z->nVars,
                         p->part ? (uint32_t)p->sh.lo : 0u, p->part ? (uint32_t)p->sh.hi : z->domainSize, row_cut, s);
        launch_fr_to_internal(p->csr_val.p, nnz, 2, s);
        uint32_t bad[4] = {0, 0, 0, 0};
        HIP_TRY(hipMemcpyAsync(bad, err.p, 16, hipMemcpyDeviceToHost, s));
        HIP_TRY(hipStreamSynchronize(s));
        if (bad[0]) throw std::invalid_argument("zkey coefficient record out of range");
        p->csr_long.build(p->csr_rowptr.p, rows, row_cut, bad, s);
        clk.lap("CSR build (device)", s);
    }

    {
        const uint32_t local_logn = p->logn - p->log_shards_chain();
        const bool pair = ntt_pair_supported(local_logn) && !probe_env("ZKHIP_NTT_RADIX2");
        if (pair) p->pair.build(p->logn, local_logn, p->part ? p->shard_index : 0u, s);
        if (!pair || p->part) {
            p->tw_fwd.alloc(n > 1 ? n / 2 : 1);
            p->tw_inv.alloc(n > 1 ? n / 2 : 1);
            if (!pair) p->tw_coset.alloc(n);
            p->tw_ninv.alloc(1);
            launch_ntt_build_tables(p->tw_fwd.p, p->tw_inv.p, p->tw_coset.p, p->tw_ninv.p, p->logn, s);
        }
    }
    clk.lap("twiddle tables", s);

    const uint64_t nv = p->sv.size(), nh = p->sh.size();
    p->precomp = (p->flags & ZK_FLAG_PRECOMP) != 0;
    p->table_mode = (p->flags & ZK_FLAG_PRECOMP_HALF) ? 2u : p->precomp ? 1u : 0u;
    p->sort_h.alloc(nh, wbits, p->table_mode, p->batch);
    alloc_slot(p.get(), 0);
    const uint64_t rows_w = msm_table_rows(p->slot[0].sort_w.plan), rows_h = msm_table_rows(p->sort_h.plan);
    p->ptsA.alloc((nv ? nv : 1) * rows_w);
    p->ptsB1.alloc((nv ? nv : 1) * rows_w);
    p->ptsB2.alloc((nv ? nv : 1) * rows_w);
    p->ptsH.alloc((nh ? nh : 1) * rows_h);
    clk.lap("workspace allocation", s);
    up.copy(p->ptsA.p, (const uint8_t *)z->pointsA + p->sv.lo * 64, nv * 64);
    up.copy(p->ptsB1.p, (const uint8_t *)z->pointsB1 + p->sv.lo * 64, nv * 64);
    up.copy(p->ptsB2.p, (const uint8_t *)z->pointsB2 + p->sv.lo * 128, nv * 128);
    up.copy(p->ptsH.p, (const uint8_t *)z->pointsH + p->sh.lo * 64, nh * 64);
    {
        uint64_t first = z->nPublic + 1;
        uint64_t lo = p->sv.lo > first ? p->sv.lo : first;
        uint64_t hi = p->sv.hi > lo ? p->sv.hi : lo;
        uint64_t cnt = hi - lo;
        uint32_t skip = (uint32_t)(lo - p->sv.lo);
        if (p->precomp) {
            p->ptsC.alloc((nv ? nv : 1) * rows_w);
            HIP_TRY(hipMemsetAsync(p->ptsC.p, 0, (size_t)(nv ? nv : 1) * 64, s));
            if (cnt) up.copy(p->ptsC.p + skip, (const uint8_t *)z->pointsC + (lo - first) * 64, cnt * 64);
            p->c_idx_min = 0;
            launch_fq_to_internal((Fq *)p->ptsC.p, nv * 2, s);
        } else {
            p->c_idx_min = skip;
            p->ptsC.alloc(cnt ? cnt : 1);
            up.copy(p->ptsC.p, (const uint8_t *)z->pointsC + (lo - first) * 64, cnt * 64);
            launch_fq_to_internal((Fq *)p->ptsC.p, cnt * 2, s);
        }
    }
    launch_fq_to_internal((Fq *)p->ptsA.p, nv * 2, s);
    launch_fq_to_internal((Fq *)p->ptsB1.p, nv * 2, s);
    launch_fq_to_internal((Fq *)p->ptsB2.p, nv * 4, s);
    launch_fq_to_internal((Fq *)p->ptsH.p, nh * 2, s);
    clk.lap("point tables upload+convert", s);
    if (p->precomp) {
        const MsmPlan plan_w = p->slot[0].sort_w.plan;
        const uint64_t tw = (uint64_t)(rows_w - 1) * (nv ? nv : 1), th = (uint64_t)(rows_h - 1) * (nh ? nh : 1);
        const uint64_t tmax = tw > th ? tw : th;
        DevBuf<G2XYZZ> tmp;
        DevBuf<Fq2> pref;
        tmp.alloc(tmax ? tmax : 1);
        pref.alloc(tmax ? tmax : 1);
        launch_msm_precomp_g1(p->ptsA.p, (G1XYZZ *)tmp.p, (Fq *)pref.p, nv, plan_w, s);
        launch_msm_precomp_g1(p->ptsB1.p, (G1XYZZ *)tmp.p, (Fq *)pref.p, nv, plan_w, s);
        launch_msm_precomp_g1(p->ptsC.p, (G1XYZZ *)tmp.p, (Fq *)pref.p, nv, plan_w, s);
        launch_msm_precomp_g1(p->ptsH.p, (G1XYZZ *)tmp.p, (Fq *)pref.p, nh, p->sort_h.plan, s);
        launch_msm_precomp_g2(p->ptsB2.p, tmp.p, pref.p, nv, plan_w, s);
        HIP_TRY(hipStreamSynchronize(s));
    }

    p->abc.alloc(3 * p->nloc * p->batch);
    p->h.alloc(p->nloc * p->batch);
    if (p->part) p->xb.alloc(3 * p->nloc);
    p->abc_use = p->abc.p;
    p->xb_use = p->xb.p;
    {
        const char *e = getenv("ZKHIP_LANES");
        int lanes = e ? atoi(e) : (p->domainSize <= (1u << 17) && p->batch == 1 ? 8 : p->domainSize <= (1u << 22) ? 4 : 1);
        if (lanes < 1) lanes = 1;
        if (lanes > zk_prover::MAX_LANES) lanes = zk_prover::MAX_LANES;
        if (p->part || getenv("ZKHIP_SERIAL")) lanes = 1;
        for (int l = 1; l < lanes; l++) {
            auto x = std::make_unique<zk_prover::LaneExtra>();
            const char *ls = getenv("ZKHIP_LANE_STREAMS");
            x->one_stream = ls && atoi(ls) == 1;
            x->n_abc = 3 * p->nloc * p->batch;
            x->n_h = p->nloc * p->batch;
            x->nh_sort = nh;
            x->wbits = wbits;
            x->precomp = p->table_mode;
            x->batch = p->batch;
            p->extra[l - 1] = std::move(x);
        }
        p->lanes = lanes;
        const char *ge = getenv("ZKHIP_GRAPH");
        p->use_graph = ge && atoi(ge) != 0 && !p->part && p->batch == 1 && !(p->flags & ZK_FLAG_TIMINGS) && !getenv("ZKHIP_SERIAL");
    }
    HIP_TRY(hipStreamSynchronize(s));
    side.finish();
    clk.lap(p->precomp ? "window pre-computation" : "finish", s);
    *out = p.release();
}

}

extern "C" {

int zk_device_count(int *count) {
    return guarded([&] {
        int n = 0;
        HIP_TRY(hipGetDeviceCount(&n));
        *count = n;
    });
}

int zk_prover_create(zk_prover **out, const zk_zkey_view *zkey, const zk_opts *opts) {
    return guarded([&] { prover_create(out, zkey, opts); });
}

void zk_prover_destroy(zk_prover *p) {
    if (!p) return;
    int prev = -1;
    (void)hipGetDevice(&prev);
    (void)hipSetDevice(p->device);
    delete p;
    if (prev >= 0) (void)hipSetDevice(prev);
}

int zk_host_alloc(void **out, size_t bytes) {
    return guarded([&] {
        if (!out) throw std::invalid_argument("null argument");
        need_device_count();
        HIP_TRY(hipHostMalloc(out, bytes ? bytes : 1, hipHostMallocDefault));
    });
}

void zk_host_free(void *ptr) {
    if (ptr) (void)hipHostFree(ptr);
}

int zk_prover_reserve(zk_prover *p, uint32_t in_flight, uint32_t host_witnesses) {
    return guarded([&] {
        if (!p) throw std::invalid_argument("null argument");
        if (in_flight > ZK_MAX_IN_FLIGHT) throw std::invalid_argument("in_flight > ZK_MAX_IN_FLIGHT");
        std::lock_guard<std::mutex> lk(p->mtx);
        DeviceGuard g(p->device);
        const int nslots = in_flight >= 2 ? (int)std::min<uint32_t>(ZK_MAX_IN_FLIGHT, in_flight + 1) : 1;
        if (p->in_flight || p->phase_open >= 0) throw std::invalid_argument("proofs in flight");
        p->ring = nslots == 1 ? ZK_MAX_IN_FLIGHT : (uint32_t)nslots;
        p->next_submit = p->next_collect = 0;
        HIP_TRY(hipDeviceSynchronize());
        for (int i = nslots; i < (int)ZK_MAX_IN_FLIGHT; i++)
            p->slot[i].release_memory();
        for (int lane = nslots < 1 ? 1 : nslots; lane < p->lanes; lane++)
            if (p->extra[lane - 1]) p->extra[lane - 1]->release_memory();
        {
            const size_t slot_b = p->slot[0].device_bytes(), wtns_b = (size_t)p->nVars * sizeof(Fr) * p->batch;
            const size_t lane_b = p->abc.bytes() + p->h.bytes() + p->sort_h.bytes();
            size_t need = 0;
            for (int i = 0; i < nslots; i++) {
                if (!p->slot[i].allocated) need += slot_b;
                if (host_witnesses && !p->slot[i].wtns_dev.p) need += wtns_b;
            }
            for (int lane = 1; lane < p->lanes && lane < nslots; lane++)
                if (!p->extra[lane - 1]->ready) need += lane_b;
            if (need) need_hbm("zk_prover_reserve", need);
        }
        for (int i = 0; i < nslots; i++) {
            alloc_slot(p, i);
            if (host_witnesses) {
                zk_prover::ProofSlot &q = p->slot[i];
                ensure_witness_buffer(p, q);
                if (!q.wtns_pin) HIP_TRY(hipHostMalloc((void **)&q.wtns_pin, (size_t)p->nVars * 32 * p->batch, hipHostMallocDefault));
            }
        }
        for (int lane = 1; lane < p->lanes && lane < nslots; lane++) p->extra[lane - 1]->ensure();
    });
}

int zk_prover_info(zk_prover *p, zk_prover_plan *plan) {
    return guarded([&] {
        if (!p || !plan) throw std::invalid_argument("null argument");
        if (plan->size < 8 || plan->size > 4096) throw std::invalid_argument("zk_prover_plan.size not set");
        zk_prover_plan o;
        memset(&o, 0, sizeof o);
        const MsmPlan ph = p->sort_h.plan, pw = p->slot[0].sort_w.plan;
        o.window_bits_h = ph.c; o.windows_h = ph.W;
        o.window_bits_w = pw.c; o.windows_w = pw.W;
        o.precomputed_tables = p->table_mode;
        o.table_rows_h = msm_table_rows(ph); o.table_rows_w = msm_table_rows(pw);
        o.bucket_sets_h = ph.sets; o.bucket_sets_w = pw.sets;
        o.msm_a_b1_c_one_launch = p->batch_abc ? 1u : 0u;
        o.lanes = (uint32_t)p->lanes;
        o.follow_up_streams = (uint32_t)p->tail_streams;
        o.max_in_flight = ZK_MAX_IN_FLIGHT;
        const bool small = p->logn < 19, mid = p->logn <= 22 && p->shard_count == 1;
        o.depth_host_witness = small ? ZK_MAX_IN_FLIGHT : mid ? 6u : 3u;
        o.depth_resident_witness = small ? ZK_MAX_IN_FLIGHT : mid ? 6u : 2u;
        o.batch = p->batch;
        o.shard_index = p->shard_index; o.shard_count = p->shard_count; o.chain_partitioned = p->part ? 1u : 0u;
        {
            DeviceGuard g(p->device);
            size_t fr = 0, tot = 0;
            HIP_TRY(hipMemGetInfo(&fr, &tot));
            o.device_bytes_in_use = tot - fr; o.device_bytes_total = tot;
        }
        o.kernel_launches_last_proof = p->launches_last_proof;
        o.spmv_row_cut = p->csr_long.cut; o.spmv_long_rows = p->csr_long.long_rows;
        o.spmv_longest_row = p->csr_long.longest; o.spmv_chunks = p->csr_long.chunks;
        const uint32_t nb = plan->size < sizeof o ? plan->size : (uint32_t)sizeof o;
        o.size = nb;
        memcpy(plan, &o, nb);
    });
}

}
```

### rapidsnark-old_amd/csrc/prover_internal.hpp

```cpp
#pragma once
#include <hip/hip_runtime.h>
#include <string.h>
#include <stdio.h>
#include <stdlib.h>
#include <chrono>
#include <sys/random.h>
#include <string>
#include <vector>
#include <atomic>
#include <condition_variable>
#include <deque>
#include <map>
#include <mutex>
#include <thread>
#include <memory>
#include <stdexcept>
#include <exception>
#include <functional>

#include "../../include/zkhip.h"
#include "common.hpp"
#include "hipcheck.hpp"
#include "kernels.hpp"
#include "hiputil.hpp"
#include "csr_long.hpp"
#include "tail_pool.hpp"

namespace zkp {

struct Slice {
    uint64_t lo, hi;
    uint64_t size() const { return hi - lo; }
};
inline Slice shard_slice(uint64_t n, uint32_t idx, uint32_t cnt) {
    uint64_t per = (n + cnt - 1) / cnt;
    uint64_t lo = per * idx, hi = lo + per;
    if (lo > n) lo = n;
    if (hi > n) hi = n;
    return Slice{lo, hi};
}

}
using namespace zkp;

struct StageJob {
    uint8_t *dst;
    const uint8_t *src;
    size_t bytes;
};

struct zk_prover {
    int device = 0;
    uint32_t flags = 0;
    uint32_t nVars = 0, nPublic = 0, domainSize = 0, logn = 0;
    uint64_t nCoefs = 0;
    uint32_t shard_index = 0, shard_count = 1;
    uint8_t vk_alpha1[64], vk_beta1[64], vk_beta2[128], vk_delta1[64], vk_delta2[128];
    hipStream_t stream = nullptr, stream2 = nullptr;
    std::mutex mtx, cmtx, sync_mtx;

    DevBuf<uint32_t> csr_rowptr, csr_col;
    DevBuf<Fr> csr_val;
    CsrLong csr_long;
    DevBuf<TwEntry> tw_fwd, tw_inv;
    DevBuf<Fr> tw_coset, tw_ninv;
    NttPair pair;
    Slice sv, sh;
    uint32_t c_idx_min = 0;
    bool precomp = false;
    uint32_t table_mode = 0;
    DevBuf<G1Affine> ptsA, ptsB1, ptsC, ptsH;
    DevBuf<G2Affine> ptsB2;

    DevBuf<Fr> abc, h;
    SortBufs sort_h;
    struct ProofSlot {
        bool allocated = false, busy = false;
        bool use_tails = true;
        uint32_t l1_chunk_min = 0, l1_chunk_max = 0;
        SortBufs sort_w;
        DevBuf<G1Acc> buckets_g1;
        DevBuf<G2Acc> buckets_g2;
        DevBuf<G1Acc> scratch_g1, acc_ws_g1_all;
        G1Acc *acc_ws_g1[4] = {nullptr, nullptr, nullptr, nullptr};
        DevBuf<uint32_t> acc_key_all, acc_flag_all;
        uint32_t *acc_key[5] = {nullptr}, *acc_flag[5] = {nullptr};
        uint64_t acc_stride = 0;
        DevBuf<G2Acc> scratch_g2, acc_ws_g2;
        DevBuf<G1XYZZ> wsum_g1;
        DevBuf<G2XYZZ> wsum_g2;
        hipEvent_t ev_l1[5] = {nullptr, nullptr, nullptr, nullptr, nullptr};
        hipEvent_t ev_fork = nullptr, ev_join = nullptr, ev_sortw = nullptr, ev_main = nullptr, ev_done = nullptr, ev_chain = nullptr;
        bool zeroed = false;
        bool defer_w = false;
        hipEvent_t ev_tail[5] = {nullptr, nullptr, nullptr, nullptr, nullptr};
        hipEvent_t ev[20] = {};
        bool have_events = false;
        uint8_t *w1 = nullptr, *w2 = nullptr;
        size_t w1_bytes = 0, w2_bytes = 0;
        DevBuf<Fr> wtns_dev;
        DevBuf<Fr> spmv_part;
        uint8_t *wtns_pin = nullptr;
        uint8_t *pin_ring = nullptr;
        StageJob stage[ZK_MAX_BATCH];
        StageJob stage_chunk[16];
        hipEvent_t ev_h2d_b = nullptr;
        hipEvent_t ev_h2d = nullptr, ev_h2d_start = nullptr;
        uint8_t r32[ZK_MAX_BATCH][32], s32[ZK_MAX_BATCH][32];
        bool have_r = false, have_s = false;
        bool host_witness = false;
        uint32_t count = 1;
        hipGraph_t graph = nullptr;
        hipGraphExec_t gexec = nullptr;
        const Fr *graph_wtns = nullptr;
        hipEvent_t ev_gdone = nullptr;
        bool via_graph = false;
        size_t device_bytes() const {
            return sort_w.bytes() + buckets_g1.bytes() + buckets_g2.bytes() + scratch_g1.bytes() + acc_ws_g1_all.bytes() + acc_key_all.bytes()
                 + acc_flag_all.bytes() + scratch_g2.bytes() + acc_ws_g2.bytes() + wsum_g1.bytes() + wsum_g2.bytes() + spmv_part.bytes();
        }
        void release_memory() {
            allocated = false;
            sort_w.release();
            buckets_g1.release(); buckets_g2.release(); scratch_g1.release(); acc_ws_g1_all.release();
            acc_key_all.release(); acc_flag_all.release(); scratch_g2.release(); acc_ws_g2.release();
            wsum_g1.release(); wsum_g2.release(); wtns_dev.release(); spmv_part.release();
            if (w1) { (void)hipHostFree(w1); w1 = nullptr; }
            if (w2) { (void)hipHostFree(w2); w2 = nullptr; }
            if (wtns_pin) { (void)hipHostFree(wtns_pin); wtns_pin = nullptr; }
            if (pin_ring) { (void)hipHostFree(pin_ring); pin_ring = nullptr; }
            if (gexec) { (void)hipGraphExecDestroy(gexec); gexec = nullptr; }
            if (graph) { (void)hipGraphDestroy(graph); graph = nullptr; }
            graph_wtns = nullptr;
        }
        ~ProofSlot() {
            if (gexec) (void)hipGraphExecDestroy(gexec);
            if (graph) (void)hipGraphDestroy(graph);
            if (ev_gdone) (void)hipEventDestroy(ev_gdone);
            for (auto &e : ev_l1) if (e) (void)hipEventDestroy(e);
            for (hipEvent_t e : {ev_fork, ev_join, ev_sortw, ev_main, ev_done, ev_chain}) if (e) (void)hipEventDestroy(e);
            for (auto &e : ev_tail) if (e) (void)hipEventDestroy(e);
            for (auto &e : ev) if (e) (void)hipEventDestroy(e);
            if (w1) (void)hipHostFree(w1);
            if (w2) (void)hipHostFree(w2);
            if (wtns_pin) (void)hipHostFree(wtns_pin);
            if (pin_ring) (void)hipHostFree(pin_ring);
            if (ev_h2d) (void)hipEventDestroy(ev_h2d);
            if (ev_h2d_b) (void)hipEventDestroy(ev_h2d_b);
            if (ev_h2d_start) (void)hipEventDestroy(ev_h2d_start);
        }
    };
    ProofSlot slot[ZK_MAX_IN_FLIGHT];
    uint32_t next_submit = 0, next_collect = 0, in_flight = 0;
    uint32_t ring = ZK_MAX_IN_FLIGHT;
    uint32_t batch = 1;
    struct LaneExtra {
        hipStream_t stream = nullptr, stream2 = nullptr;
        DevBuf<Fr> abc, h;
        SortBufs sort_h;
        uint64_t n_abc = 0, n_h = 0, nh_sort = 0;
        uint32_t wbits = 0, batch = 1;
        uint32_t precomp = 0;
        bool one_stream = false;
        bool ready = false;
        void ensure() {
            if (ready) return;
            if (!stream) HIP_TRY(hipStreamCreateWithFlags(&stream, hipStreamNonBlocking));
            if (!stream2) {
                if (one_stream) stream2 = stream;
                else HIP_TRY(hipStreamCreateWithFlags(&stream2, hipStreamNonBlocking));
            }
            if (!abc.p) abc.alloc(n_abc);
            if (!h.p) h.alloc(n_h);
            sort_h.alloc(nh_sort, wbits, precomp, batch);
            ready = true;
        }
        void release_memory() {
            ready = false;
            abc.release(); h.release(); sort_h.release();
        }
        ~LaneExtra() {
            if (stream2 && stream2 != stream) { (void)hipStreamSynchronize(stream2); (void)hipStreamDestroy(stream2); }
            if (stream) { (void)hipStreamSynchronize(stream); (void)hipStreamDestroy(stream); }
        }
    };
    static constexpr int MAX_LANES = 8;
    std::unique_ptr<LaneExtra> extra[MAX_LANES - 1];
    int lanes = 1;
    uint32_t wbits = 0;
    bool part = false;
    uint32_t log_shards = 0;
    uint64_t nloc = 0;
    DevBuf<Fr> xb;
    Fr *abc_use = nullptr, *xb_use = nullptr;
    Fr *pk_use = nullptr;
    Fr *peer_abc[8] = {nullptr}, *peer_xb[8] = {nullptr};
    bool have_peers = false;
    int phase_open = -1, phase_next = 0;
    hipEvent_t ev_ext_in = nullptr, ev_ext_out = nullptr;
    uint32_t log_shards_chain() const { return part ? log_shards : 0; }
    hipStream_t tail_pool[5] = {nullptr, nullptr, nullptr, nullptr, nullptr};
    hipStream_t tail[5] = {nullptr, nullptr, nullptr, nullptr, nullptr};
    int tail_streams = 0;
    bool use_graph = false;
    bool capturing = false;
    bool batch_abc = false;
    hipStream_t stream_fin = nullptr;
    hipStream_t stream_h2d = nullptr;

    double timings[ZK_T_COUNT] = {0};
    uint32_t accum_launches = 0;
    uint64_t launches_at_front = 0, launches_last_proof = 0;

    ~zk_prover() {
        for (auto &x : extra)
            if (x && x->stream) { (void)hipStreamSynchronize(x->stream); (void)hipStreamSynchronize(x->stream2); }
        for (hipStream_t st : {stream_h2d, stream, stream2, tail_pool[0], tail_pool[1], tail_pool[2], tail_pool[3], tail_pool[4], stream_fin})
            if (st) (void)hipStreamSynchronize(st);
        if (ev_ext_in) (void)hipEventDestroy(ev_ext_in);
        if (ev_ext_out) (void)hipEventDestroy(ev_ext_out);
        if (stream_h2d) (void)hipStreamDestroy(stream_h2d);
        if (stream_fin) (void)hipStreamDestroy(stream_fin);
        for (hipStream_t st : tail_pool)
            if (st) (void)hipStreamDestroy(st);
        if (stream2 && stream2 != stream) (void)hipStreamDestroy(stream2);
        if (stream) (void)hipStreamDestroy(stream);
    }
};

namespace zkp {

void prover_create(zk_prover **out, const zk_zkey_view *z, const zk_opts *o);
void alloc_slot(zk_prover *p, int i);
void ensure_witness_buffer(zk_prover *p, zk_prover::ProofSlot &q);

struct BatchIn {
    const uint8_t *const *wtns;
    uint32_t count;
    const uint8_t *r32s, *s32s;
};
void stage_job_run(void *arg);
int phase_front(zk_prover *p, const Fr *d_wtns, const uint8_t *h_wtns, const uint8_t *r32, const uint8_t *s32, hipEvent_t src_ready = nullptr,
                const BatchIn *bi = nullptr);
void phase_cross_push(zk_prover *p, hipEvent_t pushed);
void phase_cross_run(zk_prover *p, bool inverse, hipEvent_t done);
void phase_local(zk_prover *p);
void phase_back(zk_prover *p);
struct PhaseAbort {
    zk_prover *p;
    bool armed = true;
    ~PhaseAbort() { if (armed) p->phase_open = -1; }
};
struct SubmittedRS {
    uint8_t r32[32], s32[32];
    bool have_r = false, have_s = false;
};
struct DirectProof {
    zk_proof *out;
    const uint8_t *r32, *s32;
    bool use_submitted;
    uint32_t count = 1;
};
void collect_sums(zk_prover *p, zk_msm_sums *out, SubmittedRS *rs = nullptr, const DirectProof *direct = nullptr);
void prove_finish(zk_prover *p, const zk_msm_sums *parts, uint32_t nparts, const uint8_t *r32, const uint8_t *s32, zk_proof *out);

}
```

### rapidsnark-old_amd/csrc/prover_pipeline.hip

```cpp
#include "prover_internal.hpp"

namespace {
struct StagePool {
    struct Seg { uint8_t *dst; const uint8_t *src; size_t len; std::atomic<int> *left; };
    std::mutex m;
    std::condition_variable cv, done;
    std::deque<Seg> q;
    std::vector<std::thread> th;
    bool stop = false;
    StagePool() {
        for (int i = 0; i < 4; i++) th.emplace_back([this] { run(); });
    }
    ~StagePool() {
        {
            std::lock_guard<std::mutex> lk(m);
            stop = true;
        }
        cv.notify_all();
        for (auto &t : th) t.join();
    }
    void run() {
        for (;;) {
            Seg s;
            {
// ... 31 lines not shown
        memcpy(dst + mine_lo, src + mine_lo, mine_hi - mine_lo);
        if (nseg > 1) {
            std::unique_lock<std::mutex> lk(m);
            done.wait(lk, [&] { return left.load() == 0; });
        }
    }
};
StagePool &stage_pool() {
    static StagePool *pool = new StagePool();
    return *pool;
}
}
void zkp::stage_job_run(void *arg) {
    const StageJob *j = (const StageJob *)arg;
    stage_pool().copy(j->dst, j->src, j->bytes);
}
static const Fr *upload_witnesses(zk_prover *p, zk_prover::ProofSlot &q, const uint8_t *const *h_wtns, uint32_t count,
                                  hipEvent_t src_ready = nullptr, const Fr *d_src = nullptr) {
    const size_t bytes = (size_t)p->nVars * 32;
    ensure_witness_buffer(p, q);
    hipStream_t sh = p->stream_h2d;
    if (src_ready) HIP_TRY(hipStreamWaitEvent(sh, src_ready, 0));
    const bool tm = (p->flags & ZK_FLAG_TIMINGS) != 0;
    for (uint32_t k = 0; k < count; k++) {
        uint8_t *dst = (uint8_t *)q.wtns_dev.p + (size_t)k * bytes;
        if (d_src) {
            if (tm && k == 0) HIP_TRY(hipEventRecord(q.ev_h2d_start, sh));
            HIP_TRY(hipMemcpyAsync(dst, d_src, bytes, hipMemcpyDeviceToDevice, sh));
            continue;
        }
        hipPointerAttribute_t attr;
        const bool pinned = hipPointerGetAttributes(&attr, h_wtns[k]) == hipSuccess && attr.type == hipMemoryTypeHost;
        (void)hipGetLastError();
        const uint8_t *src = h_wtns[k];
        if (!pinned) {
            if (count == 1 && bytes >= ((size_t)4 << 20) && p->in_flight == 0) {
                const size_t npc = bytes >= ((size_t)32 << 20) ? 8 : 4, per = ((bytes / npc) + 4095) & ~(size_t)4095;
                if (!q.wtns_pin && !q.pin_ring) HIP_TRY(hipHostMalloc((void **)&q.pin_ring, 2 * per, hipHostMallocDefault));
                if (!q.ev_h2d_b) HIP_TRY(hipEventCreateWithFlags(&q.ev_h2d_b, hipEventDisableTiming));
                hipStream_t sb = p->stream_fin;
                if (src_ready) HIP_TRY(hipStreamWaitEvent(sb, src_ready, 0));
                HIP_TRY(hipEventRecord(q.ev_h2d_b, sh));
                HIP_TRY(hipStreamWaitEvent(sb, q.ev_h2d_b, 0));
                if (tm) HIP_TRY(hipEventRecord(q.ev_h2d_start, sh));
                for (size_t c = 0, off = 0; off < bytes; c++, off += per) {
                    const size_t len = off + per < bytes ? per : bytes - off;
                    hipStream_t st = (c & 1) ? sb : sh;
                    uint8_t *stg = q.wtns_pin ? q.wtns_pin + off : q.pin_ring + (c & 1) * per;
                    q.stage_chunk[c] = StageJob{stg, h_wtns[k] + off, len};
                    HIP_TRY(hipLaunchHostFunc(st, stage_job_run, &q.stage_chunk[c]));
                    HIP_TRY(hipMemcpyAsync(dst + off, stg, len, hipMemcpyHostToDevice, st));
                }
                HIP_TRY(hipEventRecord(q.ev_h2d_b, sb));
                HIP_TRY(hipStreamWaitEvent(sh, q.ev_h2d_b, 0));
                continue;
            }
            if (!q.wtns_pin) HIP_TRY(hipHostMalloc((void **)&q.wtns_pin, bytes * p->batch, hipHostMallocDefault));
            q.stage[k] = StageJob{q.wtns_pin + (size_t)k * bytes, h_wtns[k], bytes};
            static const bool sync_stage = probe_env("ZKHIP_STAGE_SYNC") != nullptr;
            if (sync_stage) stage_job_run(&q.stage[k]);
            else HIP_TRY(hipLaunchHostFunc(sh, stage_job_run, &q.stage[k]));
            src = q.stage[k].dst;
        }
        if (tm && k == 0) HIP_TRY(hipEventRecord(q.ev_h2d_start, sh));
        HIP_TRY(hipMemcpyAsync(dst, src, bytes, hipMemcpyHostToDevice, sh));
    }
    if (count < p->batch) HIP_TRY(hipMemsetAsync((uint8_t *)q.wtns_dev.p + (size_t)count * bytes, 0, (size_t)(p->batch - count) * bytes, sh));
    HIP_TRY(hipEventRecord(q.ev_h2d, sh));
    if (tm) HIP_TRY(hipEventRecord(q.ev[12], sh));
    return q.wtns_dev.p;
}
static const Fr *upload_witness(zk_prover *p, zk_prover::ProofSlot &q, const uint8_t *h_wtns, hipEvent_t src_ready = nullptr) {
    return upload_witnesses(p, q, &h_wtns, 1, src_ready);
}

namespace {

struct PhaseCtx {
    zk_prover *p;
    zk_prover::ProofSlot &q;
    hipStream_t s, s2, sf;
    hipStream_t tail[5] = {nullptr, nullptr, nullptr, nullptr, nullptr};
    int ntails = 0;
    Fr *abc, *h;
    SortBufs *sort_h;
    bool tm;
    uint32_t tbw, tbh, Ww;
    uint64_t ew, eh;
    MsmPlan pw;
    G1Acc *bA, *bB1, *bC, *bH;
    PhaseCtx(zk_prover *p_, int si) : p(p_), q(p_->slot[si]) {
        const int lane = si % p->lanes;
        if (lane == 0) {
            s = p->stream; s2 = p->stream2; sf = p->stream_fin;
            if (q.use_tails) {
                for (int m = 0; m < 5; m++) tail[m] = p->tail[m];
                ntails = p->tail_streams;
            }
            abc = p->abc_use; h = p->h.p; sort_h = &p->sort_h;
        } else {
            zk_prover::LaneExtra &x = *p->extra[lane - 1];
            x.ensure();
            s = x.stream; s2 = x.stream2; sf = x.stream;
            abc = x.abc.p; h = x.h.p; sort_h = &x.sort_h;
        }
        tm = (p->flags & ZK_FLAG_TIMINGS) != 0;
        tbw = q.sort_w.total_buckets(); tbh = p->sort_h.total_buckets();
        ew = q.sort_w.max_entries(); eh = p->sort_h.max_entries();
        pw = q.sort_w.plan; Ww = pw.sets * msm_wsum_rc(pw);
        bA = q.buckets_g1.p; bB1 = bA + tbw; bC = bB1 + tbw; bH = bC + tbw;
    }
    void mark(int i) const { if (tm) HIP_TRY(hipEventRecord(q.ev[i], s)); }
    AccumTail tail_of(int m) const { AccumTail t; t.stream = tail[m]; t.l1_done = q.ev_l1[m]; t.buckets_zeroed = q.zeroed; t.chunk_min = q.l1_chunk_min; t.chunk_max = q.l1_chunk_max; return t; }
    hipStream_t after(int m, hipStream_t own) const { return tail[m] ? tail[m] : own; }
    NttTables tables() const { return NttTables{p->logn, p->tw_fwd.p, p->tw_inv.p, p->tw_coset.p, p->tw_ninv.p}; }
};


static bool lone_order(const zk_prover *p) {
    static const int forced = [] { const char *e = probe_env("ZKHIP_LONE_ORDER"); return e ? atoi(e) : -1; }();
    return forced > 0 && p->shard_count == 1 && !p->part;
}

static void enqueue_witness_msms(zk_prover *p, PhaseCtx &c) {
    zk_prover::ProofSlot &q = c.q;
    hipStream_t s2 = c.s2;
    const bool tails = c.ntails != 0;
    const bool tm = c.tm;
    const uint32_t tbw = c.tbw, Ww = c.Ww;
    const uint64_t ew = c.ew;
    const MsmPlan pw = c.pw;
    static const uint32_t g2_aside_maxlog = [] { const char *e = probe_env("ZKHIP_G2_ASIDE_MAXLOG"); return e ? (uint32_t)atoi(e) : 21u; }();
    const bool g2_aside = !tails && c.sf != s2 && c.sf != c.s && p->in_flight == 0 && !p->capturing && !p->use_graph &&
                          p->sv.size() <= ((uint64_t)1 << g2_aside_maxlog);
    AccumTail t4 = c.tail_of(4);
    if (g2_aside) t4.stream = c.sf;
    launch_msm_accum_g2(q.buckets_g2.p, q.sort_w.offsets.p, q.sort_w.entries.p, p->ptsB2.p, 0, 0, tbw, ew, q.acc_ws_g2.p, q.acc_key[4], q.acc_flag[4], s2, tm ? &q.ev[10] : nullptr, t4);
    if (tails) launch_msm_reduce_g2(q.wsum_g2.p, q.scratch_g2.p, q.buckets_g2.p, 1, pw, c.tail[4]);
    else if (g2_aside) launch_msm_reduce_g2(q.wsum_g2.p, q.scratch_g2.p, q.buckets_g2.p, 1, pw, c.sf);
    if (p->batch_abc) {
        AccumBatch b;
        memset(&b, 0, sizeof b);
        b.n = 3;
        b.points[0] = p->ptsA.p; b.points[1] = p->ptsB1.p; b.points[2] = p->ptsC.p;
        static const bool one_table = probe_env("ZKHIP_PROBE_ONE_TABLE") != nullptr;
        if (one_table) b.points[1] = b.points[2] = p->ptsA.p;
        b.idx_min[2] = b.idx_sub[2] = p->c_idx_min;
        b.bucket_stride = tbw;
        b.ws_stride = q.acc_stride;
        launch_msm_accum_g1_batch(c.bA, q.sort_w.offsets.p, q.sort_w.entries.p, b, tbw, ew, q.acc_ws_g1[0], q.acc_key[0], q.acc_flag[0], s2, tm ? &q.ev[8] : nullptr, c.tail_of(0));
        if (tm) for (int e : {13, 14, 15, 16}) HIP_TRY(hipEventRecord(q.ev[e], s2));
        launch_msm_reduce_g1(q.wsum_g1.p, q.scratch_g1.p, c.bA, 3, pw, c.after(0, s2));
        if (!tails && !g2_aside) launch_msm_reduce_g2(q.wsum_g2.p, q.scratch_g2.p, q.buckets_g2.p, 1, pw, s2);
        HIP_TRY(hipEventRecord(q.ev_join, s2));
    } else {
    launch_msm_accum_g1(c.bA, q.sort_w.offsets.p, q.sort_w.entries.p, p->ptsA.p, 0, 0, tbw, ew, q.acc_ws_g1[0], q.acc_key[0], q.acc_flag[0], s2, tm ? &q.ev[8] : nullptr, c.tail_of(0));
    if (tails) launch_msm_reduce_g1(q.wsum_g1.p, q.scratch_g1.p, c.bA, 1, pw, c.tail[0]);
    launch_msm_accum_g1(c.bB1, q.sort_w.offsets.p, q.sort_w.entries.p, p->ptsB1.p, 0, 0, tbw, ew, q.acc_ws_g1[1], q.acc_key[1], q.acc_flag[1], s2, tm ? &q.ev[13] : nullptr, c.tail_of(1));
    if (tails) {
        launch_msm_reduce_g1(q.wsum_g1.p + Ww, q.scratch_g1.p + msm_reduce_scratch_points(1, pw), c.bB1, 1, pw, c.tail[1]);
    } else {
        if (!g2_aside) launch_msm_reduce_g2(q.wsum_g2.p, q.scratch_g2.p, q.buckets_g2.p, 1, pw, s2);
        launch_msm_reduce_g1(q.wsum_g1.p, q.scratch_g1.p, c.bA, 2, pw, s2);
    }
    HIP_TRY(hipEventRecord(q.ev_join, s2));
    }

}

}

namespace zkp {

int phase_front(zk_prover *p, const Fr *d_wtns, const uint8_t *h_wtns, const uint8_t *r32, const uint8_t *s32, hipEvent_t src_ready, const BatchIn *bi) {
    DeviceGuard g(p->device);
    if (p->in_flight >= p->ring) throw std::invalid_argument("too many proofs in flight (ZK_MAX_IN_FLIGHT, or the depth given to zk_prover_reserve): collect one first");
    if (p->phase_open >= 0) throw std::invalid_argument("a proof is still being submitted phase by phase");
    if (p->in_flight == 0 && !p->capturing) p->next_submit = p->next_collect = 0;
    const int si = (int)(p->next_submit % p->ring);
    alloc_slot(p, si);
    if (!p->capturing) p->slot[si].use_tails = p->in_flight > 0 || p->use_graph;
    if (!p->capturing) {
        static const uint32_t thr_min = [] { const char *e = probe_env("ZKHIP_L1_CHUNK_MIN_BUSY"); return e ? (uint32_t)atoi(e) : 128u; }();
        static const uint32_t thr_log = [] { const char *e = probe_env("ZKHIP_L1_CHUNK_MIN_BUSY_LOG"); return e ? (uint32_t)atoi(e) : 17u; }();
        static const uint32_t thr_max = [] { const char *e = probe_env("ZKHIP_L1_CHUNK_MAX_BUSY"); return e ? (uint32_t)atoi(e) : 1280u; }();
        static const bool shards_too = [] { const char *e = probe_env("ZKHIP_L1_BUSY_SHARDS"); return e ? atoi(e) != 0 : true; }();
        uint32_t lg_sh = 0;
        while ((1u << (lg_sh + 1)) <= p->shard_count) lg_sh++;
        const bool busy = p->in_flight > 0 && !p->use_graph && ((p->shard_count == 1 && !p->part) || shards_too) && p->batch == 1 && p->logn >= thr_log + lg_sh;
        p->slot[si].l1_chunk_min = busy ? thr_min : 0u;
        p->slot[si].l1_chunk_max = busy ? thr_max : 0u;
    }
    PhaseCtx c(p, si);
    zk_prover::ProofSlot &q = c.q;
    if (!p->capturing) p->launches_at_front = g_kernel_launches.load(std::memory_order_relaxed);
    bool staged = h_wtns != nullptr;
    q.count = 1;
    if (bi) {
        if (bi->count < 1 || bi->count > p->batch) throw std::invalid_argument("batch submission: between 1 and opts.batch witnesses");
        d_wtns = upload_witnesses(p, q, bi->wtns, bi->count, src_ready);
        staged = true;
        q.count = bi->count;
        r32 = bi->r32s;
        s32 = bi->s32s;
    } else if (staged) {
        d_wtns = upload_witness(p, q, h_wtns, src_ready);
    } else if (p->batch > 1) {
        d_wtns = upload_witnesses(p, q, nullptr, 1, src_ready, d_wtns);
        staged = true;
    }
    q.host_witness = h_wtns != nullptr || bi != nullptr;
    q.have_r = r32 != nullptr;
    q.have_s = s32 != nullptr;
    if (r32) memcpy(q.r32, r32, (size_t)32 * q.count);
    if (s32) memcpy(q.s32, s32, (size_t)32 * q.count);
    hipStream_t s = c.s, s2 = c.s2;
    const bool tails = c.ntails != 0;
    const bool tm = c.tm;

    c.mark(0);
    q.zeroed = !p->capturing && !p->use_graph;
    if (q.zeroed) {
        HIP_TRY(hipMemsetAsync(c.bA, 0, (size_t)3 * c.tbw * sizeof(G1Acc), s2));
        HIP_TRY(hipMemsetAsync(q.buckets_g2.p, 0, (size_t)c.tbw * sizeof(G2Acc), s2));
        HIP_TRY(hipMemsetAsync(c.bH, 0, (size_t)c.tbh * sizeof(G1Acc), s));
    }
    if (staged) {
        HIP_TRY(hipStreamWaitEvent(s, q.ev_h2d, 0));
        HIP_TRY(hipStreamWaitEvent(s2, q.ev_h2d, 0));
    }
    if (p->capturing && s2 != s) {
        HIP_TRY(hipEventRecord(q.ev_fork, s));
        HIP_TRY(hipStreamWaitEvent(s2, q.ev_fork, 0));
    }
    q.sort_w.run(d_wtns + p->sv.lo, s2);
    HIP_TRY(hipEventRecord(q.ev_sortw, s2));
    q.defer_w = lone_order(p) && !p->capturing && !p->use_graph && p->in_flight == 0 && s2 != s;
    if (!q.defer_w) enqueue_witness_msms(p, c);

    const uint64_t nl = p->nloc;
    Fr *abc = c.abc;
    const CsrDev csr = p->csr_long.view(p->csr_rowptr.p, p->csr_col.p, p->csr_val.p);
    launch_spmv_abc(abc, abc + nl, abc + 2 * nl, csr, d_wtns, (uint32_t)nl, s, q.count, 3 * nl, p->nVars, q.spmv_part.p);
    c.mark(1);
    if (p->part && !p->have_peers && p->pk_use) launch_chunk_pack(p->pk_use, abc, 3, p->logn, p->log_shards, s);
    p->phase_open = si;
    p->phase_next = p->part ? 1 : 2;
    return si;
}

void phase_cross_push(zk_prover *p, hipEvent_t pushed) {
    DeviceGuard g(p->device);
    launch_chunk_scatter(p->peer_xb, p->abc_use, 3, p->logn, p->log_shards, p->shard_index, p->stream);
    HIP_TRY(hipEventRecord(pushed, p->stream));
}
void phase_cross_run(zk_prover *p, bool inverse, hipEvent_t done) {
    if (p->phase_open < 0 || p->phase_next != (inverse ? 1 : 3)) throw std::invalid_argument("chain phases out of order");
    DeviceGuard g(p->device);
    PhaseCtx c(p, p->phase_open);
    const uint64_t nl = p->nloc, chunk = nl >> p->log_shards;
    if (p->have_peers) {
        launch_ntt_cross(inverse, p->xb_use, chunk, nl, p->peer_abc, nl, (uint64_t)p->shard_index * chunk, 3, c.tables(), p->log_shards, p->shard_index, c.s);
    } else {
        if (!p->pk_use) throw std::invalid_argument("no exchange buffers registered (zk_shard_set_exchange)");
        Fr *inplace[8];
        for (uint32_t i = 0; i < 8; i++) inplace[i] = p->xb_use + (uint64_t)i * 3 * chunk;
        launch_ntt_cross(inverse, p->xb_use, 3 * chunk, chunk, inplace, chunk, 0, 3, c.tables(), p->log_shards, p->shard_index, c.s);
    }
    if (done) HIP_TRY(hipEventRecord(done, c.s));
    p->phase_next = inverse ? 2 : 4;
}

void phase_local(zk_prover *p) {
    if (p->phase_open < 0 || p->phase_next != 2) throw std::invalid_argument("chain phases out of order");
    DeviceGuard g(p->device);
    PhaseCtx c(p, p->phase_open);
    const uint32_t local_logn = p->logn - p->log_shards_chain();
    const uint64_t nl = p->nloc;
    NttTables tb = c.tables();
    const bool a2a = p->part && !p->have_peers;
    if (a2a) launch_chunk_unpack(c.abc, p->pk_use, 3, p->logn, p->log_shards, c.s);
    if (p->pair.L) {
        static const bool skip_ntt = probe_env("ZKHIP_PROBE_SKIP_NTT") != nullptr;
        launch_ntt_coset_pair(c.abc, nl, (skip_ntt ? 1 : 3) * c.q.count, p->pair, c.s);
    } else {
        launch_ntt_dif_inverse(c.abc, nl, 3 * c.q.count, tb, c.s, local_logn);
        launch_ntt_dit_forward(c.abc, nl, 3 * c.q.count, tb, c.s, p->tw_coset.p + (p->part ? p->sh.lo : 0), local_logn);
    }
    if (a2a) launch_chunk_pack(p->pk_use, c.abc, 3, p->logn, p->log_shards, c.s);
    if (c.q.defer_w) {
        HIP_TRY(hipEventRecord(c.q.ev_chain, c.s));
        HIP_TRY(hipStreamWaitEvent(c.s2, c.q.ev_chain, 0));
        enqueue_witness_msms(p, c);
        c.q.defer_w = false;
    }
    p->phase_next = p->part ? 3 : 4;
}

void phase_back(zk_prover *p) {
    if (p->phase_open < 0 || p->phase_next != 4) throw std::invalid_argument("chain phases out of order");
    DeviceGuard g(p->device);
    PhaseCtx c(p, p->phase_open);
    zk_prover::ProofSlot &q = c.q;
    hipStream_t s = c.s;
    const uint64_t nl = p->nloc;
    Fr *abc = c.abc;
    if (p->part && !p->have_peers) launch_chunk_unpack(abc, p->pk_use, 3, p->logn, p->log_shards, s);
    launch_abc_to_h(c.h, abc, abc + nl, abc + 2 * nl, nl, s, q.count, 3 * nl);
    if (q.count < p->batch) HIP_TRY(hipMemsetAsync(c.h + nl * q.count, 0, (size_t)(p->batch - q.count) * nl * sizeof(Fr), s));
    c.mark(2);
    c.sort_h->run(c.h + (p->part ? 0 : p->sh.lo), s);
    c.mark(3);
    launch_msm_accum_g1(c.bH, c.sort_h->offsets.p, c.sort_h->entries.p, p->ptsH.p, 0, 0, c.tbh, c.eh, q.acc_ws_g1[3], q.acc_key[3], q.acc_flag[3], s, c.tm ? &q.ev[17] : nullptr, c.tail_of(3));
    c.mark(4);
    launch_msm_reduce_g1(q.wsum_g1.p + 3 * c.Ww, q.scratch_g1.p + msm_reduce_scratch_points(3, c.pw), c.bH, 1, p->sort_h.plan, c.after(3, s));
    if (!p->batch_abc) {
    HIP_TRY(hipStreamWaitEvent(s, q.ev_sortw, 0));
    launch_msm_accum_g1(c.bC, q.sort_w.offsets.p, q.sort_w.entries.p, p->ptsC.p, p->c_idx_min, p->c_idx_min, c.tbw, c.ew, q.acc_ws_g1[2], q.acc_key[2], q.acc_flag[2], s, c.tm ? &q.ev[15] : nullptr, c.tail_of(2));
    launch_msm_reduce_g1(q.wsum_g1.p + 2 * c.Ww, q.scratch_g1.p + msm_reduce_scratch_points(2, c.pw), c.bC, 1, c.pw, c.after(2, s));
    }
    c.mark(5);
    HIP_TRY(hipEventRecord(q.ev_main, s));

    hipStream_t sf = c.sf;
    HIP_TRY(hipStreamWaitEvent(sf, q.ev_main, 0));
    HIP_TRY(hipStreamWaitEvent(sf, q.ev_join, 0));
    for (int i = 0; i < c.ntails; i++) {
        HIP_TRY(hipEventRecord(q.ev_tail[i], p->tail_pool[i]));
        HIP_TRY(hipStreamWaitEvent(sf, q.ev_tail[i], 0));
    }
    if (c.tm) HIP_TRY(hipEventRecord(q.ev[6], sf));
    HIP_TRY(hipMemcpyAsync(q.w1, q.wsum_g1.p, q.w1_bytes, hipMemcpyDeviceToHost, sf));
    HIP_TRY(hipMemcpyAsync(q.w2, q.wsum_g2.p, q.w2_bytes, hipMemcpyDeviceToHost, sf));
    HIP_TRY(hipEventRecord(q.ev_done, sf));
    if (p->capturing && sf != s) HIP_TRY(hipStreamWaitEvent(s, q.ev_done, 0));
    HIP_TRY(hipGetLastError());
    if (!p->capturing) p->launches_last_proof = g_kernel_launches.load(std::memory_order_relaxed) - p->launches_at_front;
    q.busy = true;
    q.via_graph = false;
    p->phase_open = -1;
    p->next_submit++;
    p->in_flight++;
}


}

static void submit_graph(zk_prover *p, const Fr *d_wtns, const uint8_t *h_wtns, const uint8_t *r32, const uint8_t *s32) {
    if (p->in_flight >= p->ring) throw std::invalid_argument("too many proofs in flight (ZK_MAX_IN_FLIGHT, or the depth given to zk_prover_reserve): collect one first");
    if (p->phase_open >= 0) throw std::invalid_argument("a proof is still being submitted phase by phase");
    if (p->in_flight == 0) p->next_submit = p->next_collect = 0;
    const int si = (int)(p->next_submit % p->ring);
    alloc_slot(p, si);
    PhaseCtx c(p, si);
    zk_prover::ProofSlot &q = c.q;
    if (!q.ev_gdone) HIP_TRY(hipEventCreateWithFlags(&q.ev_gdone, hipEventDisableTiming));
    const bool staged = h_wtns != nullptr;
    if (staged) d_wtns = upload_witness(p, q, h_wtns);
    if (!q.gexec || q.graph_wtns != d_wtns) {
        if (q.gexec) { (void)hipGraphExecDestroy(q.gexec); q.gexec = nullptr; }
        if (q.graph) { (void)hipGraphDestroy(q.graph); q.graph = nullptr; }
        const uint32_t ns = p->next_submit, nf = p->in_flight;
        HIP_TRY(hipStreamBeginCapture(c.s, hipStreamCaptureModeRelaxed));
        p->capturing = true;
        hipError_t end = hipSuccess;
        try {
            PhaseAbort guard{p};
            phase_front(p, d_wtns, nullptr, r32, s32);
            phase_local(p);
            phase_back(p);
            guard.armed = false;
        } catch (...) {
            p->capturing = false;
            hipGraph_t dead = nullptr;
            (void)hipStreamEndCapture(c.s, &dead);
            if (dead) (void)hipGraphDestroy(dead);
            p->next_submit = ns; p->in_flight = nf; q.busy = false;
            throw;
        }
        p->capturing = false;
        end = hipStreamEndCapture(c.s, &q.graph);
        p->next_submit = ns; p->in_flight = nf; q.busy = false;
        HIP_TRY(end);
        HIP_TRY(hipGraphInstantiate(&q.gexec, q.graph, nullptr, nullptr, 0));
        q.graph_wtns = d_wtns;
    }
    q.host_witness = staged;
    q.have_r = r32 != nullptr;
    q.have_s = s32 != nullptr;
    if (r32) memcpy(q.r32, r32, 32);
    if (s32) memcpy(q.s32, s32, 32);
    if (staged) HIP_TRY(hipStreamWaitEvent(c.s, q.ev_h2d, 0));
    HIP_TRY(hipGraphLaunch(q.gexec, c.s));
    HIP_TRY(hipEventRecord(q.ev_gdone, c.s));
    q.busy = true;
    q.via_graph = true;
    p->next_submit++;
    p->in_flight++;
}

static void submit_locked(zk_prover *p, const Fr *d_wtns, const uint8_t *h_wtns, const uint8_t *r32, const uint8_t *s32, const BatchIn *bi = nullptr) {
    if (p->part) throw std::invalid_argument("this prover holds one block of a partitioned chain: drive it through zk_multi_prove* or zk_shard_*");
// ... 260 lines not shown
```

### rapidsnark-old_amd/lib.py

```python
import ctypes as C
import os

import numpy as np

_HERE = os.path.dirname(os.path.abspath(__file__))
_LIB = None


class ZkHipError(RuntimeError):
    pass


def library_path():
    return os.environ.get("ZKHIP_LIB") or os.path.join(_HERE, "libzkhip.so")


class zk_zkey_view(C.Structure):
    _fields_ = [("nVars", C.c_uint32), ("nPublic", C.c_uint32), ("domainSize", C.c_uint32), ("nCoefs", C.c_uint64),
                ("vk_alpha1", C.c_void_p), ("vk_beta1", C.c_void_p), ("vk_beta2", C.c_void_p),
                ("vk_delta1", C.c_void_p), ("vk_delta2", C.c_void_p), ("coefs", C.c_void_p),
                ("pointsA", C.c_void_p), ("pointsB1", C.c_void_p), ("pointsB2", C.c_void_p),
                ("pointsC", C.c_void_p), ("pointsH", C.c_void_p),
                ("coefs_bytes", C.c_uint64), ("pointsA_bytes", C.c_uint64), ("pointsB1_bytes", C.c_uint64),
                ("pointsB2_bytes", C.c_uint64), ("pointsC_bytes", C.c_uint64), ("pointsH_bytes", C.c_uint64)]
# ... 74 lines not shown

class zk_vkey_view(C.Structure):
    _fields_ = [("vk_alpha1", C.c_void_p), ("vk_beta2", C.c_void_p), ("vk_gamma2", C.c_void_p), ("vk_delta2", C.c_void_p),
                ("IC", C.c_void_p), ("nPublic", C.c_uint32)]


class zk_vkey_plan(C.Structure):
    _fields_ = [("coop_max", C.c_uint32), ("last_path", C.c_uint32), ("last_launches", C.c_uint32), ("reserved", C.c_uint32),
                ("proofs_coop", C.c_uint64), ("proofs_lanes", C.c_uint64)]


class zk_ptau_file_view(C.Structure):
    _fields_ = [("power", C.c_uint32), ("sec", C.c_void_p * 16), ("sec_bytes", C.c_uint64 * 16)]


class zk_ptau_check_sizes_t(C.Structure):
    _fields_ = [("prepared", C.c_uint32), ("chunk_points", C.c_uint64), ("device_bytes", C.c_uint64)]


class zk_ptau_report(C.Structure):
    _fields_ = [("verdict", C.c_uint32), ("failed", C.c_uint32), ("lagrange_failed", C.c_uint32 * 4), ("bad_section", C.c_uint32),
                ("bad_kind", C.c_uint32), ("bad_index", C.c_uint64)]


class zk_ptau_contrib_sizes(C.Structure):
    _fields_ = [("tau_g1_bytes", C.c_uint64), ("tau_g2_bytes", C.c_uint64), ("alpha_tau_g1_bytes", C.c_uint64), ("beta_tau_g1_bytes", C.c_uint64),
                ("beta_g2_bytes", C.c_uint64), ("chunk_points", C.c_uint64), ("device_bytes", C.c_uint64)]


class zk_ptau_contrib_out(C.Structure):
    _fields_ = [("tau_g1", C.c_void_p), ("tau_g2", C.c_void_p), ("alpha_tau_g1", C.c_void_p), ("beta_tau_g1", C.c_void_p), ("beta_g2", C.c_void_p)]


class zk_zkey_verify_view(C.Structure):
    _fields_ = [("key", zk_zkey_view), ("vk_gamma2", C.c_void_p), ("pointsIC", C.c_void_p), ("pointsIC_bytes", C.c_uint64)]


class zk_zkey_verify_sizes_t(C.Structure):
    _fields_ = [("log_domain", C.c_uint32), ("shape_failed", C.c_uint32), ("chunk_points", C.c_uint64), ("device_bytes", C.c_uint64)]


class zk_zkey_verify_report(C.Structure):
    _fields_ = [("size", C.c_uint32), ("verdict", C.c_uint32), ("failed", C.c_uint32), ("not_checked", C.c_uint32), ("shape_failed", C.c_uint32),
                ("bad_section", C.c_uint32), ("bad_kind", C.c_uint32), ("bad_index", C.c_uint64), ("coef_rows_differing", C.c_uint64),
                ("coef_first_row", C.c_uint32), ("delta_is_generator", C.c_uint32)]


class zk_setup_out(C.Structure):
    _fields_ = [("coefs", C.c_void_p), ("pointsIC", C.c_void_p), ("pointsA", C.c_void_p), ("pointsB1", C.c_void_p),
                ("pointsB2", C.c_void_p), ("pointsC", C.c_void_p), ("pointsH", C.c_void_p)]


def prover_info(lib, handle):
    plan = zk_prover_plan()
    plan.size = C.sizeof(zk_prover_plan)
    check(lib.zk_prover_info(handle, C.byref(plan)))
    return {name: int(getattr(plan, name)) for name, _ in zk_prover_plan._fields_ if name != "size"}


def multi_prover_shard_info(lib, handle, shard):
    plan = zk_prover_plan()
    plan.size = C.sizeof(zk_prover_plan)
    check(lib.zk_multi_prover_shard_info(handle, shard, C.byref(plan)))
    return {name: int(getattr(plan, name)) for name, _ in zk_prover_plan._fields_ if name != "size"}


ZK_FLAG_TIMINGS = 1
ZK_FLAG_PRECOMP = 2
ZK_FLAG_PARTITIONED_CHAIN = 4
ZK_FLAG_SPARSE_WITNESS = 8
ZK_FLAG_PRECOMP_HALF = 16


def precomp_flags(precomp):
    mode = int(precomp)
    if mode not in (0, 1, 2):
        raise ValueError("precomp: 0, 1 or 2")
    return (0, ZK_FLAG_PRECOMP, ZK_FLAG_PRECOMP | ZK_FLAG_PRECOMP_HALF)[mode]
ZK_STEP_CROSS_INVERSE, ZK_STEP_LOCAL, ZK_STEP_CROSS_FORWARD, ZK_STEP_FINISH = 1, 2, 3, 4
ZK_T_NAMES = ["spmv", "ntt_chain_wall", "sort_h", "msm_h_wall", "join_wait", "msm_reduce", "total_device", "g1_l1_kernel", "g2_l1_kernel", "wtns_h2d"]

EXPORTS = ["zk_last_error", "zk_device_count", "zk_prover_create", "zk_prover_destroy", "zk_prove", "zk_prove_dev",
           "zk_prove_dev_submit", "zk_prove_submit", "zk_prove_batch_submit", "zk_prove_batch_collect", "zk_host_alloc", "zk_host_free", "zk_prove_collect", "zk_prover_reserve", "zk_prover_info", "zk_prove_msm_collect", "zk_prove_msm_dev", "zk_prove_msm", "zk_prove_finish", "zk_prover_timings", "zk_fr_mul_vec",
           "zk_fq_mul_vec", "zk_fr_coef_accumulate", "zk_fr_ntt", "zk_fr_abc_to_h", "zk_msm_g1", "zk_msm_g2", "zk_proof_to_json",
           "zk_public_to_json", "zk_synth_chain_g1", "zk_synth_chain_g2", "zk_fixed_base_g1", "zk_fixed_base_g2", "zk_g1_mul", "zk_g2_mul", "zk_assemble",
           "zk_multi_prover_create", "zk_multi_prover_destroy", "zk_multi_prove", "zk_multi_prove_submit", "zk_multi_prove_collect",
           "zk_multi_prover_info", "zk_multi_prover_shard_info", "zk_shard_info", "zk_shard_set_exchange", "zk_shard_begin", "zk_shard_step",
           "zk_r1cs_create", "zk_r1cs_destroy", "zk_r1cs_check", "zk_r1cs_check_dev", "zk_r1cs_match_zkey",
           "zk_groth16_setup_sizes", "zk_groth16_setup",
           "zk_g1_lagrange", "zk_g2_lagrange", "zk_ptau_prepare_sizes", "zk_ptau_prepare",
           "zk_g1_scale", "zk_g1_scale_plan", "zk_zkey_contribute_sizes", "zk_zkey_contribute",
           "zk_pairing", "zk_vkey_create", "zk_vkey_destroy", "zk_vkey_verify", "zk_vkey_info", "zk_pairing_last_path",
           "zk_g2_in_subgroup", "zk_g1_power_msm", "zk_g2_power_msm", "zk_fr_power_dft", "zk_ptau_check_sizes", "zk_ptau_check",
           "zk_zkey_verify_sizes", "zk_zkey_verify",
           "zk_g1_mul_vec", "zk_g2_mul_vec", "zk_g1_power_scale", "zk_g2_power_scale", "zk_glv_split", "zk_ptau_contribute_sizes", "zk_ptau_contribute"]
ZK_SCALE_PLAN_MAX = 130
ZK_VERIFY_OK, ZK_VERIFY_INVALID, ZK_VERIFY_MALFORMED = 0, 1, 2
ZK_VERIFY_PATH_LANES, ZK_VERIFY_PATH_COOP = 0, 1
ZK_PTAU_OK, ZK_PTAU_INVALID, ZK_PTAU_MALFORMED = 0, 1, 2


def load_library():
    global _LIB
    if _LIB is not None:
        return _LIB
    path = library_path()
    if not os.path.exists(path):
        raise ZkHipError("libzkhip.so not built (%s): run `python -c 'import __graft_entry__ as g; g.build()'` "
                         "or `make -C rapidsnark-old_amd/csrc`; there is no CPU fallback" % path)
    os.environ.setdefault("GPU_MAX_HW_QUEUES", "16")
    try:
        import torch
    except ImportError:
        pass
    lib = C.CDLL(path)
    lib.zk_last_error.restype = C.c_char_p
    u8p = C.c_void_p
    lib.zk_device_count.argtypes = [C.POINTER(C.c_int)]
    lib.zk_prover_create.argtypes = [C.POINTER(C.c_void_p), C.POINTER(zk_zkey_view), C.POINTER(zk_opts)]
    lib.zk_prover_destroy.argtypes = [C.c_void_p]
    lib.zk_prover_destroy.restype = None
    lib.zk_prove.argtypes = [C.c_void_p, u8p, u8p, u8p, C.POINTER(zk_proof)]
    lib.zk_prove_dev.argtypes = [C.c_void_p, C.c_void_p, u8p, u8p, C.POINTER(zk_proof)]
    lib.zk_prove_dev_submit.argtypes = [C.c_void_p, C.c_void_p, u8p, u8p]
    lib.zk_prove_submit.argtypes = [C.c_void_p, u8p, u8p, u8p]
    lib.zk_prove_batch_submit.argtypes = [C.c_void_p, C.c_void_p, C.c_uint32, u8p, u8p]
    lib.zk_prove_batch_collect.argtypes = [C.c_void_p, C.c_void_p, C.c_uint32]
    lib.zk_host_alloc.argtypes = [C.POINTER(C.c_void_p), C.c_size_t]
    lib.zk_host_free.argtypes = [C.c_void_p]
    lib.zk_host_free.restype = None
    lib.zk_prove_collect.argtypes = [C.c_void_p, C.POINTER(zk_proof)]
    lib.zk_prove_msm_collect.argtypes = [C.c_void_p, C.POINTER(zk_msm_sums)]
    lib.zk_prove_msm.argtypes = [C.c_void_p, u8p, C.POINTER(zk_msm_sums)]
    lib.zk_prove_msm_dev.argtypes = [C.c_void_p, C.c_void_p, C.POINTER(zk_msm_sums)]
    lib.zk_prove_finish.argtypes = [C.c_void_p, C.POINTER(zk_msm_sums), C.c_uint32, u8p, u8p, C.POINTER(zk_proof)]
    lib.zk_assemble.argtypes = [u8p, u8p, u8p, u8p, u8p, C.POINTER(zk_msm_sums), C.c_uint32, u8p, u8p, C.POINTER(zk_proof)]
    lib.zk_prover_timings.argtypes = [C.c_void_p, C.POINTER(C.c_double), C.c_uint32]
    if hasattr(lib, "zk_prover_reserve"):
        lib.zk_prover_reserve.argtypes = [C.c_void_p, C.c_uint32, C.c_uint32]
    if hasattr(lib, "zk_prover_info"):
        lib.zk_prover_info.argtypes = [C.c_void_p, C.POINTER(zk_prover_plan)]
    lib.zk_multi_prover_create.argtypes = [C.POINTER(C.c_void_p), C.POINTER(zk_zkey_view), C.POINTER(C.c_int32), C.c_uint32, C.POINTER(zk_opts)]
    lib.zk_multi_prover_destroy.argtypes = [C.c_void_p]
    lib.zk_multi_prover_destroy.restype = None
    lib.zk_multi_prove.argtypes = [C.c_void_p, u8p, u8p, u8p, C.POINTER(zk_proof)]
    lib.zk_multi_prove_submit.argtypes = [C.c_void_p, u8p, u8p, u8p]
    lib.zk_multi_prove_collect.argtypes = [C.c_void_p, C.POINTER(zk_proof)]
    lib.zk_multi_prover_info.argtypes = [C.c_void_p, C.POINTER(C.c_uint32), C.POINTER(C.c_uint32)]
    lib.zk_multi_prover_shard_info.argtypes = [C.c_void_p, C.c_uint32, C.POINTER(zk_prover_plan)]
    lib.zk_shard_info.argtypes = [C.c_void_p, C.POINTER(C.c_uint64), C.POINTER(C.c_uint32)]
    lib.zk_shard_set_exchange.argtypes = [C.c_void_p, C.c_void_p, C.c_void_p]
    lib.zk_shard_begin.argtypes = [C.c_void_p, u8p, C.c_void_p, u8p, u8p, C.c_void_p]
    lib.zk_shard_step.argtypes = [C.c_void_p, C.c_int, C.c_void_p]
    for name in ("zk_fr_mul_vec", "zk_fq_mul_vec"):
        getattr(lib, name).argtypes = [u8p, u8p, u8p, C.c_uint64]
    lib.zk_fr_coef_accumulate.argtypes = [u8p, u8p, u8p, C.c_uint64, C.c_uint32, u8p, C.c_uint32]
    lib.zk_fr_ntt.argtypes = [u8p, C.c_uint64, C.c_int]
    lib.zk_fr_abc_to_h.argtypes = [u8p, u8p, u8p, C.c_uint64]
    lib.zk_msm_g1.argtypes = [u8p, u8p, u8p, C.c_uint64]
    lib.zk_msm_g2.argtypes = [u8p, u8p, u8p, C.c_uint64]
    lib.zk_synth_chain_g1.argtypes = [u8p, C.c_uint64, u8p, u8p]
    lib.zk_synth_chain_g2.argtypes = [u8p, C.c_uint64, u8p, u8p]
    lib.zk_fixed_base_g1.argtypes = [u8p, u8p, u8p, C.c_uint64]
    lib.zk_fixed_base_g2.argtypes = [u8p, u8p, u8p, C.c_uint64]
    lib.zk_g1_mul.argtypes = [u8p, u8p, u8p]
    lib.zk_g2_mul.argtypes = [u8p, u8p, u8p]
    lib.zk_proof_to_json.argtypes = [C.POINTER(zk_proof), C.c_char_p, C.c_size_t]
    lib.zk_proof_to_json.restype = C.c_size_t
    lib.zk_public_to_json.argtypes = [u8p, C.c_uint32, C.c_char_p, C.c_size_t]
    lib.zk_public_to_json.restype = C.c_size_t
    if hasattr(lib, "zk_r1cs_create"):
        lib.zk_r1cs_create.argtypes = [C.POINTER(C.c_void_p), C.POINTER(zk_r1cs_view), C.c_int32]
        lib.zk_r1cs_destroy.argtypes = [C.c_void_p]
        lib.zk_r1cs_destroy.restype = None
        lib.zk_r1cs_check.argtypes = [C.c_void_p, u8p, C.c_uint32, C.POINTER(zk_r1cs_report)]
        lib.zk_r1cs_check_dev.argtypes = [C.c_void_p, C.c_void_p, C.c_uint32, C.POINTER(zk_r1cs_report)]
        lib.zk_r1cs_match_zkey.argtypes = [C.c_void_p, C.POINTER(zk_zkey_view), C.POINTER(C.c_uint64), C.POINTER(C.c_uint32)]
    if hasattr(lib, "zk_groth16_setup"):
        lib.zk_groth16_setup_sizes.argtypes = [C.POINTER(zk_r1cs_view), C.POINTER(zk_ptau_view), C.POINTER(zk_setup_sizes)]
        lib.zk_groth16_setup.argtypes = [C.POINTER(zk_r1cs_view), C.POINTER(zk_ptau_view), C.c_int32, C.POINTER(zk_setup_out)]
    if hasattr(lib, "zk_ptau_prepare"):
        lib.zk_g1_lagrange.argtypes = [u8p, u8p, C.c_uint64, C.c_uint32, C.c_int32]
        lib.zk_g2_lagrange.argtypes = [u8p, u8p, C.c_uint64, C.c_uint32, C.c_int32]
        lib.zk_ptau_prepare_sizes.argtypes = [C.POINTER(zk_ptau_powers_view), C.POINTER(zk_ptau_lagrange_sizes)]
        lib.zk_ptau_prepare.argtypes = [C.POINTER(zk_ptau_powers_view), C.c_int32, C.POINTER(zk_ptau_lagrange_out)]
    if hasattr(lib, "zk_g1_scale"):
        lib.zk_g1_scale.argtypes = [u8p, u8p, C.c_uint64, u8p, C.c_int32]
        lib.zk_g1_scale_plan.argtypes = [u8p, C.POINTER(C.c_int8), C.POINTER(C.c_int8), C.c_uint32, C.POINTER(C.c_uint32)]
        lib.zk_zkey_contribute_sizes.argtypes = [C.POINTER(zk_zkey_contrib_view), C.POINTER(zk_zkey_contrib_sizes)]
        lib.zk_zkey_contribute.argtypes = [C.POINTER(zk_zkey_contrib_view), u8p, C.c_int32, C.POINTER(zk_zkey_contrib_out)]
    if hasattr(lib, "zk_pairing"):
        lib.zk_pairing.argtypes = [u8p, u8p, u8p, C.c_uint64, C.c_uint32, C.c_int32]
        lib.zk_vkey_create.argtypes = [C.POINTER(C.c_void_p), C.POINTER(zk_vkey_view), C.c_int32]
        lib.zk_vkey_destroy.argtypes = [C.c_void_p]
        lib.zk_vkey_destroy.restype = None
        lib.zk_vkey_verify.argtypes = [C.c_void_p, u8p, u8p, C.c_uint64, u8p]
    if hasattr(lib, "zk_vkey_info"):
        lib.zk_vkey_info.argtypes = [C.c_void_p, C.POINTER(zk_vkey_plan)]
        lib.zk_pairing_last_path.argtypes = []
        lib.zk_pairing_last_path.restype = C.c_int
    if hasattr(lib, "zk_ptau_check"):
        lib.zk_g2_in_subgroup.argtypes = [u8p, u8p, C.c_uint64, C.c_int32]
        lib.zk_g1_power_msm.argtypes = [u8p, u8p, C.c_uint64, u8p, C.c_uint64, C.c_int32]
        lib.zk_g2_power_msm.argtypes = [u8p, u8p, C.c_uint64, u8p, C.c_uint64, C.c_int32]
        lib.zk_fr_power_dft.argtypes = [u8p, u8p, C.c_uint32, C.c_int32]
        lib.zk_ptau_check_sizes.argtypes = [C.POINTER(zk_ptau_file_view), C.POINTER(zk_ptau_check_sizes_t)]
        lib.zk_ptau_check.argtypes = [C.POINTER(zk_ptau_file_view), u8p, C.c_int32, C.POINTER(zk_ptau_report)]
    if hasattr(lib, "zk_zkey_verify"):
        lib.zk_zkey_verify_sizes.argtypes = [C.POINTER(zk_r1cs_view), C.POINTER(zk_ptau_view), C.POINTER(zk_zkey_verify_view),
                                             C.POINTER(zk_zkey_verify_sizes_t)]
        lib.zk_zkey_verify.argtypes = [C.POINTER(zk_r1cs_view), C.POINTER(zk_ptau_view), C.POINTER(zk_zkey_verify_view), u8p, C.c_int32,
                                       C.POINTER(zk_zkey_verify_report)]
    if hasattr(lib, "zk_ptau_contribute"):
        lib.zk_g1_mul_vec.argtypes = [u8p, u8p, u8p, C.c_uint64, C.c_int32]
        lib.zk_g2_mul_vec.argtypes = [u8p, u8p, u8p, C.c_uint64, C.c_int32]
        lib.zk_g1_power_scale.argtypes = [u8p, u8p, C.c_uint64, u8p, C.c_uint64, u8p, C.c_int32]
        lib.zk_g2_power_scale.argtypes = [u8p, u8p, C.c_uint64, u8p, C.c_uint64, u8p, C.c_int32]
        lib.zk_glv_split.argtypes = [u8p, u8p, u8p]
        lib.zk_ptau_contribute_sizes.argtypes = [C.POINTER(zk_ptau_file_view), C.POINTER(zk_ptau_contrib_sizes)]
        lib.zk_ptau_contribute.argtypes = [C.POINTER(zk_ptau_file_view), u8p, u8p, u8p, C.c_int32, C.POINTER(zk_ptau_contrib_out)]
    _LIB = lib
    return lib


def check(rc):
    if rc != 0:
        raise ZkHipError(load_library().zk_last_error().decode("utf-8", "replace"))


def _buf(b, nbytes=None):
    a = np.frombuffer(b, dtype=np.uint8) if not isinstance(b, np.ndarray) else np.ascontiguousarray(b).view(np.uint8).reshape(-1)
    if nbytes is not None and a.size != nbytes:
        raise ValueError("expected %d bytes, got %d" % (nbytes, a.size))
    return a


def _ptr(a):
    return C.c_void_p(a.ctypes.data)


def device_count():
    n = C.c_int(0)
    check(load_library().zk_device_count(C.byref(n)))
    return n.value


class PinnedBuffer:

    def __init__(self, nbytes):
        self._ptr = C.c_void_p()
        check(load_library().zk_host_alloc(C.byref(self._ptr), nbytes))
        self.nbytes = nbytes
        self.array = np.ctypeslib.as_array(C.cast(self._ptr, C.POINTER(C.c_uint8)), shape=(nbytes,))

    def free(self):
        if self._ptr is not None and self._ptr.value:
            self.array = None
            load_library().zk_host_free(self._ptr)
            self._ptr = C.c_void_p()

    __del__ = free


def _mul_vec(fn, a, b):
    a, b = _buf(a), _buf(b)
    assert a.size == b.size and a.size % 32 == 0
    out = np.empty_like(a)
    check(fn(_ptr(out), _ptr(a), _ptr(b), a.size // 32))
    return out.tobytes()


def fr_mul_vec(a, b):
    return _mul_vec(load_library().zk_fr_mul_vec, a, b)


def fq_mul_vec(a, b):
    return _mul_vec(load_library().zk_fq_mul_vec, a, b)


def fr_coef_accumulate(coefs, n_coefs, domain_size, wtns):
    coefs, wtns = _buf(coefs), _buf(wtns)
    a = np.empty(domain_size * 32, dtype=np.uint8)
    b = np.empty(domain_size * 32, dtype=np.uint8)
    check(load_library().zk_fr_coef_accumulate(_ptr(a), _ptr(b), _ptr(coefs), n_coefs, domain_size, _ptr(wtns), wtns.size // 32))
    return a, b


def fr_ntt(data, inverse=False):
    a = _buf(data).copy()
    check(load_library().zk_fr_ntt(_ptr(a), a.size // 32, 1 if inverse else 0))
    return a.tobytes()


def fr_abc_to_h(a, b):
    a, b = _buf(a), _buf(b)
    out = np.empty_like(a)
    check(load_library().zk_fr_abc_to_h(_ptr(out), _ptr(a), _ptr(b), a.size // 32))
    return out.tobytes()


def msm_g1(bases, scalars):
    bases, scalars = _buf(bases), _buf(scalars)
    n = scalars.size // 32
    assert bases.size == n * 64
    out = np.zeros(64, dtype=np.uint8)
    check(load_library().zk_msm_g1(_ptr(out), _ptr(bases), _ptr(scalars), n))
    return out.tobytes()


def msm_g2(bases, scalars):
    bases, scalars = _buf(bases), _buf(scalars)
    n = scalars.size // 32
    assert bases.size == n * 128
    out = np.zeros(128, dtype=np.uint8)
    check(load_library().zk_msm_g2(_ptr(out), _ptr(bases), _ptr(scalars), n))
    return out.tobytes()


def proof_to_json(proof_bytes):
    p = zk_proof.from_buffer_copy(bytes(proof_bytes))
    lib = load_library()
    n = lib.zk_proof_to_json(C.byref(p), None, 0)
    buf = C.create_string_buffer(n + 1)
    lib.zk_proof_to_json(C.byref(p), buf, n + 1)
    return buf.value.decode()


def public_to_json(wtns_values_bytes, n_public):
    a = _buf(wtns_values_bytes)
    lib = load_library()
    n = lib.zk_public_to_json(_ptr(a), n_public, None, 0)
    buf = C.create_string_buffer(n + 1)
    lib.zk_public_to_json(_ptr(a), n_public, buf, n + 1)
    return buf.value.decode()


def synth_chain_g1(n, p0, q):
    out = np.zeros(n * 64, dtype=np.uint8)
    a, b = _buf(p0).copy(), _buf(q).copy()
    check(load_library().zk_synth_chain_g1(_ptr(out), n, _ptr(a), _ptr(b)))
    return out


def synth_chain_g2(n, p0, q):
    out = np.zeros(n * 128, dtype=np.uint8)
    a, b = _buf(p0).copy(), _buf(q).copy()
    check(load_library().zk_synth_chain_g2(_ptr(out), n, _ptr(a), _ptr(b)))
    return out


def _scalars_le(scalars):
    if isinstance(scalars, np.ndarray) and scalars.dtype == np.uint8:
        return np.ascontiguousarray(scalars)
    return np.frombuffer(b"".join(int(k).to_bytes(32, "little") for k in scalars), dtype=np.uint8).copy()


def fixed_base_g1(base, scalars):
    sc = _scalars_le(scalars)
    n = sc.size // 32
    out = np.zeros(n * 64, dtype=np.uint8)
    b = _buf(base).copy()
    check(load_library().zk_fixed_base_g1(_ptr(out), _ptr(b), _ptr(sc), n))
    return out


def fixed_base_g2(base, scalars):
    sc = _scalars_le(scalars)
    n = sc.size // 32
    out = np.zeros(n * 128, dtype=np.uint8)
    b = _buf(base).copy()
    check(load_library().zk_fixed_base_g2(_ptr(out), _ptr(b), _ptr(sc), n))
    return out


def _lagrange(name, nb, points, log_n, device):
    pts = _buf(points)
    if pts.size % nb:
        raise ValueError("points: a multiple of %d bytes expected" % nb)
    out = np.zeros(nb << log_n, dtype=np.uint8)
    fn = getattr(load_library(), name, None)
    if fn is None:
        raise ZkHipError("%s is not in this build of libzkhip.so" % name)
    check(fn(_ptr(out), _ptr(pts) if pts.size else None, pts.size // nb, log_n, device))
    return out


def g1_lagrange(points, log_n, device=-1):
    return _lagrange("zk_g1_lagrange", 64, points, log_n, device)


def g2_lagrange(points, log_n, device=-1):
    return _lagrange("zk_g2_lagrange", 128, points, log_n, device)


def _scalar32(k):
    k = int(k)
    if not 0 <= k < 1 << 256:
        raise ValueError("scalar: 0 <= k < 2^256 expected")
    return np.frombuffer(k.to_bytes(32, "little"), dtype=np.uint8).copy()


# ... 132 lines not shown
```

Before: 30.18.

## Fuse abc-to-h into digit extraction, fuse bin count, skip empty buckets in reduce

The H-polynomial scalar computation (a*b-c, from Montgomery form) now happens inside the MSM digit kernel, so the separate abc_to_h pass and its intermediate buffer write are gone. The digit kernel can also build per-block bin histograms in LDS, which replaces the separate k_bin_count pass. The bucket reduce reads sort offsets to skip loading empty buckets, which allows skipping the bucket memsets when offsets are available. Extra event tracking serializes sort_h reuse against the previous reduce, and a sort-dump debug export is added. Risks are higher register pressure in the fused kernel and correctness depending on offsets covering every bucket that is not cleared.

```diff
diff --git a/include/zkhip.h b/include/zkhip.h
--- a/include/zkhip.h
+++ b/include/zkhip.h
@@ -142,6 +142,8 @@
 int zk_fr_abc_to_h(uint8_t *h, const uint8_t *a, const uint8_t *b, uint64_t n);
 int zk_msm_g1(uint8_t out[64], const uint8_t *bases, const uint8_t *scalars, uint64_t n);
 int zk_msm_g2(uint8_t out[128], const uint8_t *bases, const uint8_t *scalars, uint64_t n);
+int zk_msm_sort_dump(const uint8_t *scalars, uint64_t n, uint32_t window_bits, uint32_t table_mode, int32_t fuse_count, uint64_t sizes[3],
+                     uint32_t *offsets, uint32_t *entries, uint32_t *bin_counts);
 
 int zk_synth_chain_g1(uint8_t *out, uint64_t n, const uint8_t p0[64], const uint8_t q[64]);
 int zk_synth_chain_g2(uint8_t *out, uint64_t n, const uint8_t p0[128], const uint8_t q[128]);
diff --git a/rapidsnark-old_amd/csrc/hiputil.hpp b/rapidsnark-old_amd/csrc/hiputil.hpp
--- a/rapidsnark-old_amd/csrc/hiputil.hpp
+++ b/rapidsnark-old_amd/csrc/hiputil.hpp
@@ -136,11 +136,16 @@
     }
     bool ran = false;
     void run(const Fr *scalars, hipStream_t s) {
+        MsmScalarSrc src{};
+        src.scalars = scalars;
+        run(src, s);
+    }
+    void run(const MsmScalarSrc &src, hipStream_t s, bool fuse_count = true) {
         static const bool skip = probe_env("ZKHIP_PROBE_SKIP_SORT") != nullptr;
         if (skip && ran) return;
         ran = true;
         MsmSortBufs b{offsets.p, entries.p, counts.p, starts.p, codes.p, val.p, bin_counts.p, bin_starts.p, lo.p};
-        launch_msm_sort(b, scalars, n, plan, s);
+        launch_msm_sort_src(b, src, n, plan, s, fuse_count);
     }
 };
 
diff --git a/rapidsnark-old_amd/csrc/kernels.hpp b/rapidsnark-old_amd/csrc/kernels.hpp
--- a/rapidsnark-old_amd/csrc/kernels.hpp
+++ b/rapidsnark-old_amd/csrc/kernels.hpp
@@ -98,6 +98,13 @@
 MsmSortSizes msm_sort_sizes(uint64_t n, MsmPlan p);
 uint32_t msm_scan_extra_words(uint32_t total);
 void launch_msm_sort(const MsmSortBufs &b, const Fr *scalars, uint64_t n, MsmPlan p, hipStream_t s);
+struct MsmScalarSrc {
+    const Fr *scalars;
+    const Fr *a, *b, *c;
+    uint64_t abc_stride;
+    uint64_t live;
+};
+void launch_msm_sort_src(const MsmSortBufs &b, const MsmScalarSrc &src, uint64_t n, MsmPlan p, hipStream_t s, bool fuse_count = true);
 void launch_msm_precomp_g1(G1Affine *table, G1XYZZ *tmp, Fq *pref, uint64_t n, MsmPlan p, hipStream_t s);
 void launch_msm_precomp_g2(G2Affine *table, G2XYZZ *tmp, Fq2 *pref, uint64_t n, MsmPlan p, hipStream_t s);
 struct alignas(16) G1Acc {
@@ -110,7 +117,7 @@
 struct AccumTail {
     hipStream_t stream = nullptr;
     hipEvent_t l1_done = nullptr;
-    bool buckets_zeroed = false;
+    bool skip_clear = false;
     uint32_t chunk_min = 0;
     uint32_t chunk_max = 0;
 };
@@ -132,8 +139,9 @@
                          uint32_t idx_min, uint32_t idx_sub, uint32_t total_buckets, uint64_t max_entries,
                          G2Acc *ws_part, uint32_t *ws_key, uint32_t *ws_flag, hipStream_t s, hipEvent_t *ev = nullptr,
                          AccumTail tail = AccumTail());
-void launch_msm_reduce_g1(G1XYZZ *window_sums, G1Acc *scratch, const G1Acc *buckets, uint32_t n_msm, MsmPlan p, hipStream_t s);
-void launch_msm_reduce_g2(G2XYZZ *window_sums, G2Acc *scratch, const G2Acc *buckets, uint32_t n_msm, MsmPlan p, hipStream_t s);
+void launch_msm_reduce_g1(G1XYZZ *window_sums, G1Acc *scratch, const G1Acc *buckets, uint32_t n_msm, MsmPlan p, hipStream_t s, const uint32_t *offsets = nullptr);
+void launch_msm_reduce_g2(G2XYZZ *window_sums, G2Acc *scratch, const G2Acc *buckets, uint32_t n_msm, MsmPlan p, hipStream_t s, const uint32_t *offsets = nullptr);
+bool msm_reduce_skips_empty(MsmPlan p);
 uint64_t msm_reduce_scratch_points(uint32_t n_msm, MsmPlan p);
 uint32_t msm_wsum_rc(MsmPlan p);
 
diff --git a/rapidsnark-old_amd/csrc/msm_accum.hip b/rapidsnark-old_amd/csrc/msm_accum.hip
--- a/rapidsnark-old_amd/csrc/msm_accum.hip
+++ b/rapidsnark-old_amd/csrc/msm_accum.hip
@@ -380,7 +380,7 @@
                          uint32_t total_buckets, uint64_t max_entries,
                          ACCMEM *ws_part, uint32_t *ws_key, uint32_t *ws_flag, hipStream_t s, hipEvent_t *ev, AccumTail tail) {
     const uint32_t nb = batch.n ? batch.n : 1;
-    if (!tail.buckets_zeroed) ZK_HIP(hipMemsetAsync(buckets, 0, ((size_t)(nb - 1) * batch.bucket_stride + total_buckets) * sizeof(ACCMEM), s));
+    if (!tail.skip_clear) ZK_HIP(hipMemsetAsync(buckets, 0, ((size_t)(nb - 1) * batch.bucket_stride + total_buckets) * sizeof(ACCMEM), s));
     const uint32_t cmin = tail.chunk_min > accum_chunk_min() ? tail.chunk_min : accum_chunk_min();
     uint64_t lanes = accum_lanes_for<F>(max_entries, nb, cmin, tail.chunk_max > accum_chunk_max() ? tail.chunk_max : 0u);
     if (ev) ZK_HIP(hipEventRecord(ev[0], s));
diff --git a/rapidsnark-old_amd/csrc/msm_reduce.hip b/rapidsnark-old_amd/csrc/msm_reduce.hip
--- a/rapidsnark-old_amd/csrc/msm_reduce.hip
+++ b/rapidsnark-old_amd/csrc/msm_reduce.hip
@@ -8,16 +8,27 @@
 #define REDUCE_THREADS 256u
 
 template <class F>
-__global__ __launch_bounds__(128) void k_msm_reduce_split(ACCMEM *A, uint32_t a_stride, ACCMEM *T, const ACCMEM *buckets, uint32_t nbuckets, uint32_t chunk, uint32_t L) {
+__global__ __launch_bounds__(128) void k_msm_reduce_split(ACCMEM *A, uint32_t a_stride, ACCMEM *T, const ACCMEM *buckets, uint32_t nbuckets, uint32_t chunk, uint32_t L,
+                                                          const uint32_t *offsets, uint32_t sets) {
     ZK_TAIL_PRIO();
     typedef LaneModel<F> LM;
     typedef typename LM::R FR;
     const uint32_t t = (blockIdx.x * blockDim.x + threadIdx.x) / LM::LPE;
     if (t >= L) return;
     const ACCMEM *B = buckets + (uint64_t)blockIdx.y * nbuckets + (uint64_t)t * chunk;
+    const uint32_t *off = offsets ? offsets + (uint64_t)(blockIdx.y % sets) * nbuckets + (uint64_t)t * chunk : nullptr;
+    uint32_t end = off ? off[chunk] : 0u;
     XYZZ<FR> run = XYZZ<FR>::inf(), sum = XYZZ<FR>::inf();
     for (int j = (int)chunk - 1; j >= 0; j--) {
-        add(run, LM::load(B + j));
+        XYZZ<FR> b = XYZZ<FR>::inf();
+        bool filled = true;
+        if (off) {
+            const uint32_t start = off[j];
+            filled = start != end;
+            end = start;
+        }
+        if (filled) b = LM::load(B + j);
+        add(run, b);
         add(sum, run);
     }
     LM::store(A + (uint64_t)blockIdx.y * a_stride + t, sum);
@@ -241,7 +252,7 @@
 }
 
 template <class F>
-static void launch_reduce(XYZZ<F> *window_sums, ACCMEM *scratch, const ACCMEM *buckets, uint32_t n_msm, MsmPlan p, hipStream_t s) {
+static void launch_reduce(XYZZ<F> *window_sums, ACCMEM *scratch, const ACCMEM *buckets, uint32_t n_msm, MsmPlan p, hipStream_t s, const uint32_t *offsets) {
     if (skip_followups_probe()) return;
     if (reduce_bits_for(p)) {
         const uint32_t NE = REDUCE_THREADS / LaneModel<F>::LPE, groups = n_msm * p.sets;
@@ -262,7 +273,7 @@
     if (const uint32_t ch = reduce_split_for(p)) {
         const uint32_t L = p.nbuckets / ch, top = reduce_split_top(L), nx = L / top, per = nx + L;
         ACCMEM *T = scratch, *Y = T + (uint64_t)groups * L, *P = Y + (uint64_t)groups * per;
-        ZK_LAUNCH(k_msm_reduce_split<F>, dim3((L * LaneModel<F>::LPE + 127) / 128, groups), dim3(128), 0, s, Y + nx, per, T, buckets, p.nbuckets, ch, L);
+        ZK_LAUNCH(k_msm_reduce_split<F>, dim3((L * LaneModel<F>::LPE + 127) / 128, groups), dim3(128), 0, s, Y + nx, per, T, buckets, p.nbuckets, ch, L, offsets, p.sets);
         chunks(Y, per, T, L, top);
         const uint32_t bx = nx / TREE_IN, ba = L / TREE_IN;
         ZK_LAUNCH(k_msm_reduce_tree<F>, dim3(bx + ba, groups), dim3(REDUCE_THREADS), lds, s, P, window_sums, (const ACCMEM *)Y, per, 0u);
@@ -285,11 +296,12 @@
     }
     ZK_LAUNCH_OK("msm bucket reduction");
 }
-void launch_msm_reduce_g1(G1XYZZ *ws, G1Acc *scratch, const G1Acc *buckets, uint32_t n_msm, MsmPlan p, hipStream_t s) {
-    launch_reduce<Fq>(ws, scratch, buckets, n_msm, p, s);
-}
-void launch_msm_reduce_g2(G2XYZZ *ws, G2Acc *scratch, const G2Acc *buckets, uint32_t n_msm, MsmPlan p, hipStream_t s) {
-    launch_reduce<Fq2>(ws, scratch, buckets, n_msm, p, s);
-}
-
-}
+void launch_msm_reduce_g1(G1XYZZ *ws, G1Acc *scratch, const G1Acc *buckets, uint32_t n_msm, MsmPlan p, hipStream_t s, const uint32_t *offsets) {
+    launch_reduce<Fq>(ws, scratch, buckets, n_msm, p, s, offsets);
+}
+void launch_msm_reduce_g2(G2XYZZ *ws, G2Acc *scratch, const G2Acc *buckets, uint32_t n_msm, MsmPlan p, hipStream_t s, const uint32_t *offsets) {
+    launch_reduce<Fq2>(ws, scratch, buckets, n_msm, p, s, offsets);
+}
+bool msm_reduce_skips_empty(MsmPlan p) { return reduce_split_for(p) != 0; }
+
+}
diff --git a/rapidsnark-old_amd/csrc/msm_sort.hip b/rapidsnark-old_amd/csrc/msm_sort.hip
--- a/rapidsnark-old_amd/csrc/msm_sort.hip
+++ b/rapidsnark-old_amd/csrc/msm_sort.hip
@@ -1,6 +1,7 @@
 #include "kernels.hpp"
 #include "hipcheck.hpp"
 #include "common.hpp"
+#include "field29.hpp"
 #include "devmem.hpp"
 #include <string.h>
 
@@ -61,15 +62,38 @@
 #define SORT_THREADS 1024u
 #endif
 
-__global__ __launch_bounds__(256) void k_msm_digits(uint32_t *digits, const Fr *scalars, uint64_t n, MsmPlan p) {
-    ZK_CHAIN_PRIO();
-    uint64_t st = (uint64_t)gridDim.x * blockDim.x;
+#define BIN_ITEMS 8u
+template <bool ABC, bool COUNT>
+__global__ __launch_bounds__(COUNT ? SORT_THREADS : 256) void k_msm_digits(uint32_t *digits, MsmScalarSrc src, uint64_t n, MsmPlan p, uint32_t *bin_counts,
+                                                                           uint32_t nbins, uint32_t nblocks, uint32_t shift) {
+    ZK_CHAIN_PRIO();
+    extern __shared__ uint32_t dhist[];
     const uint32_t c = p.c, W = p.W;
     const uint32_t mask = (1u << c) - 1u, half = 1u << (c - 1);
     const uint32_t set_stride = p.precomp == 1 ? 0u : p.nbuckets, set_mask = p.precomp == 2 ? 1u : 0xffffffffu;
-    for (uint64_t i = (uint64_t)blockIdx.x * blockDim.x + threadIdx.x; i < n; i += st) {
-        Fr s = load_el(scalars + i);
-        const uint32_t vec_base = p.batch > 1 ? (uint32_t)(i / p.batch_n) * p.nbuckets : 0u;
+    if (COUNT) {
+        for (uint32_t k = threadIdx.x; k < W * nbins; k += blockDim.x) dhist[k] = 0;
+        __syncthreads();
+    }
+    const uint64_t st = COUNT ? (uint64_t)blockDim.x : (uint64_t)gridDim.x * blockDim.x;
+    const uint64_t i0 = COUNT ? (uint64_t)blockIdx.x * (BIN_ITEMS * SORT_THREADS) + threadIdx.x : (uint64_t)blockIdx.x * blockDim.x + threadIdx.x;
+    const uint64_t i1 = COUNT ? ((uint64_t)blockIdx.x + 1) * (BIN_ITEMS * SORT_THREADS) : n;
+    for (uint64_t i = i0; i < i1; i += st) {
+        const uint32_t vec = p.batch > 1 ? (uint32_t)(i / p.batch_n) : 0u;
+        Fr s;
+        if (ABC) {
+            if (i < src.live) {
+                const uint64_t j = p.batch > 1 ? (uint64_t)vec * src.abc_stride + (i - (uint64_t)vec * p.batch_n) : i;
+                Fr29 t = Fr29::sub(Fr29::mul(Fr29::load(load_el(src.a + j)), Fr29::load(load_el(src.b + j))), Fr29::load(load_el(src.c + j)));
+                s = Fr29::store(Fr29::from_mont(t));
+            } else {
+#pragma unroll
+                for (int j = 0; j < 8; j++) s.v[j] = 0;
+            }
+        } else {
+            s = load_el(src.scalars + i);
+        }
+        const uint32_t vec_base = vec * p.nbuckets;
         for (int k = 0; k < 6; k++) {
             Fr d;
             u32 bw = 0;
@@ -85,8 +109,10 @@
             const bool neg = d >= half;
             carry = neg ? 1u : 0u;
             uint32_t mag = neg ? (1u << c) - d : d;
-            uint32_t code = mag ? ((mag - 1u + (w & set_mask) * set_stride + vec_base) | (neg ? 0x80000000u : 0u)) : CODE32_ZERO;
+            const uint32_t key = mag - 1u + (w & set_mask) * set_stride + vec_base;
+            uint32_t code = mag ? (key | (neg ? 0x80000000u : 0u)) : CODE32_ZERO;
             digits[(uint64_t)w * n + i] = code;
+            if (COUNT && mag) atomicAdd(&dhist[w * nbins + (key >> shift)], 1u);
             w++;
         };
 #pragma unroll
@@ -101,6 +127,14 @@
         }
         emit((uint32_t)buf & mask);
     }
+    if (COUNT) {
+        __syncthreads();
+        const uint32_t per_w = nblocks / W;
+        for (uint32_t k = threadIdx.x; k < W * nbins; k += blockDim.x) {
+            const uint32_t w = k / nbins, bin = k - w * nbins;
+            bin_counts[(uint64_t)bin * nblocks + w * per_w + blockIdx.x] = dhist[k];
+        }
+    }
 }
 
 __global__ __launch_bounds__(256) void k_msm_compact_offsets(uint32_t *offsets, const uint32_t *starts, uint32_t total, uint32_t slices) {
@@ -129,7 +163,6 @@
     if (threadIdx.x < nbins) bin_counts[(uint64_t)threadIdx.x * nblocks + blockIdx.x] = hist[threadIdx.x];
 }
 
-#define BIN_ITEMS 8u
 __global__ __launch_bounds__(SORT_THREADS) void k_bin_scatter(uint16_t *lo, uint32_t *val, const uint32_t *bin_starts, const uint32_t *codes,
                                                               uint64_t total, uint32_t nbins, uint32_t nblocks, uint32_t shift, uint32_t span, uint64_t n,
                                                               uint32_t set_shift, uint32_t batch_n, uint32_t tstride) {
@@ -441,6 +474,11 @@
 }
 
 void launch_msm_sort(const MsmSortBufs &b, const Fr *scalars, uint64_t n, MsmPlan p, hipStream_t s) {
+    MsmScalarSrc src{};
+    src.scalars = scalars;
+    launch_msm_sort_src(b, src, n, p, s);
+}
+void launch_msm_sort_src(const MsmSortBufs &b, const MsmScalarSrc &src, uint64_t n, MsmPlan p, hipStream_t s, bool fuse_count) {
     const uint32_t tb = plan_total_buckets(p);
     sort_lds_attr();
     uint64_t g = (n + 255) / 256;
@@ -456,8 +494,16 @@
     const size_t lds = (size_t)bpb * 4;
     const uint32_t grid2 = ((nbins + 7u) / 8u) * 8u * slices;
     const uint32_t set_shift = p.precomp ? 32u : p.c - 1u;
-    if (n) ZK_LAUNCH(k_msm_digits, dim3((uint32_t)g), dim3(256), 0, s, b.codes, scalars, n, p);
-    ZK_LAUNCH(k_bin_count, dim3(nblocks), dim3(SORT_THREADS), 0, s, b.bin_counts, (const uint32_t *)b.codes, total, nbins, nblocks, sh, bin_span());
+    static const bool count_pass = probe_env("ZKHIP_SORT_COUNT_PASS") != nullptr;
+    const bool fused = fuse_count && !count_pass && n && n % bin_span() == 0 && (uint64_t)p.W * nbins * 4 <= 64 * 1024;
+    if (n) {
+        auto kern = src.scalars ? (fused ? k_msm_digits<false, true> : k_msm_digits<false, false>) : (fused ? k_msm_digits<true, true> : k_msm_digits<true, false>);
+        if (fused)
+            ZK_LAUNCH(kern, dim3((uint32_t)(n / bin_span())), dim3(SORT_THREADS), (size_t)p.W * nbins * 4, s, b.codes, src, n, p, b.bin_counts, nbins, nblocks, sh);
+        else
+            ZK_LAUNCH(kern, dim3((uint32_t)g), dim3(256), 0, s, b.codes, src, n, p, b.bin_counts, nbins, nblocks, sh);
+    }
+    if (!fused) ZK_LAUNCH(k_bin_count, dim3(nblocks), dim3(SORT_THREADS), 0, s, b.bin_counts, (const uint32_t *)b.codes, total, nbins, nblocks, sh, bin_span());
     launch_scan(b.bin_starts, b.bin_counts, nbins * nblocks, s);
     ZK_LAUNCH(k_bin_scatter, dim3(nblocks), dim3(SORT_THREADS), bin_scatter_lds_bytes(), s, b.lo, b.val, (const uint32_t *)b.bin_starts,
                        (const uint32_t *)b.codes, total, nbins, nblocks, sh, bin_span(), n, set_shift, p.batch > 1 ? p.batch_n : 0u, p.precomp);
diff --git a/rapidsnark-old_amd/csrc/operators.hip b/rapidsnark-old_amd/csrc/operators.hip
--- a/rapidsnark-old_amd/csrc/operators.hip
+++ b/rapidsnark-old_amd/csrc/operators.hip
@@ -260,4 +260,28 @@
     return guarded([&] { msm_generic<G2Affine, G2XYZZ, G2Acc>(out, bases, scalars, n, true); });
 }
 
-}
+int zk_msm_sort_dump(const uint8_t *scalars, uint64_t n, uint32_t window_bits, uint32_t table_mode, int32_t fuse_count, uint64_t sizes[3],
+                     uint32_t *offsets, uint32_t *entries, uint32_t *bin_counts) {
+    return guarded([&] {
+        need_device();
+        if (!scalars || !sizes || !n || n >= (1ull << 31)) throw std::invalid_argument("zk_msm_sort_dump: scalars, sizes and 0 < n < 2^31");
+        SortBufs sb;
+        sb.alloc(n, window_bits, table_mode);
+        sizes[0] = sb.offsets.n;
+        sizes[1] = sb.entries.n;
+        sizes[2] = sb.bin_counts.n;
+        if (!offsets && !entries && !bin_counts) return;
+        DevBuf<Fr> sc;
+        sc.alloc(n);
+        sc.upload(scalars, n, 0);
+        MsmScalarSrc src{};
+        src.scalars = sc.p;
+        sb.run(src, 0, fuse_count != 0);
+        HIP_TRY(hipStreamSynchronize(0));
+        if (offsets) HIP_TRY(hipMemcpy(offsets, sb.offsets.p, sb.offsets.bytes(), hipMemcpyDeviceToHost));
+        if (entries) HIP_TRY(hipMemcpy(entries, sb.entries.p, sb.entries.bytes(), hipMemcpyDeviceToHost));
+        if (bin_counts) HIP_TRY(hipMemcpy(bin_counts, sb.bin_counts.p, sb.bin_counts.bytes(), hipMemcpyDeviceToHost));
+    });
+}
+
+}
diff --git a/rapidsnark-old_amd/csrc/prover_create.hip b/rapidsnark-old_amd/csrc/prover_create.hip
--- a/rapidsnark-old_amd/csrc/prover_create.hip
+++ b/rapidsnark-old_amd/csrc/prover_create.hip
@@ -37,7 +37,7 @@
     if (!q.w2) HIP_TRY(hipHostMalloc((void **)&q.w2, q.w2_bytes, hipHostMallocDefault));
     for (auto &e : q.ev_l1)
         if (!e) HIP_TRY(hipEventCreateWithFlags(&e, hipEventDisableTiming));
-    for (hipEvent_t *e : {&q.ev_fork, &q.ev_join, &q.ev_sortw, &q.ev_main, &q.ev_done, &q.ev_chain})
+    for (hipEvent_t *e : {&q.ev_fork, &q.ev_join, &q.ev_sortw, &q.ev_main, &q.ev_done, &q.ev_chain, &q.ev_hred})
         if (!*e) HIP_TRY(hipEventCreateWithFlags(e, hipEventDisableTiming));
     for (auto &e : q.ev_tail)
         if (!e) HIP_TRY(hipEventCreateWithFlags(&e, hipEventDisableTiming));
@@ -271,7 +271,6 @@
     }
 
     p->abc.alloc(3 * p->nloc * p->batch);
-    p->h.alloc(p->nloc * p->batch);
     if (p->part) p->xb.alloc(3 * p->nloc);
     p->abc_use = p->abc.p;
     p->xb_use = p->xb.p;
@@ -286,7 +285,6 @@
             const char *ls = getenv("ZKHIP_LANE_STREAMS");
             x->one_stream = ls && atoi(ls) == 1;
             x->n_abc = 3 * p->nloc * p->batch;
-            x->n_h = p->nloc * p->batch;
             x->nh_sort = nh;
             x->wbits = wbits;
             x->precomp = p->table_mode;
@@ -357,7 +355,7 @@
             if (p->extra[lane - 1]) p->extra[lane - 1]->release_memory();
         {
             const size_t slot_b = p->slot[0].device_bytes(), wtns_b = (size_t)p->nVars * sizeof(Fr) * p->batch;
-            const size_t lane_b = p->abc.bytes() + p->h.bytes() + p->sort_h.bytes();
+            const size_t lane_b = p->abc.bytes() + p->sort_h.bytes();
             size_t need = 0;
             for (int i = 0; i < nslots; i++) {
                 if (!p->slot[i].allocated) need += slot_b;
diff --git a/rapidsnark-old_amd/csrc/prover_internal.hpp b/rapidsnark-old_amd/csrc/prover_internal.hpp
--- a/rapidsnark-old_amd/csrc/prover_internal.hpp
+++ b/rapidsnark-old_amd/csrc/prover_internal.hpp
@@ -72,7 +72,7 @@
     DevBuf<G1Affine> ptsA, ptsB1, ptsC, ptsH;
     DevBuf<G2Affine> ptsB2;
 
-    DevBuf<Fr> abc, h;
+    DevBuf<Fr> abc;
     SortBufs sort_h;
     struct ProofSlot {
         bool allocated = false, busy = false;
@@ -91,6 +91,7 @@
         DevBuf<G2XYZZ> wsum_g2;
         hipEvent_t ev_l1[5] = {nullptr, nullptr, nullptr, nullptr, nullptr};
         hipEvent_t ev_fork = nullptr, ev_join = nullptr, ev_sortw = nullptr, ev_main = nullptr, ev_done = nullptr, ev_chain = nullptr;
+        hipEvent_t ev_hred = nullptr;
         bool zeroed = false;
         bool defer_w = false;
         hipEvent_t ev_tail[5] = {nullptr, nullptr, nullptr, nullptr, nullptr};
@@ -138,7 +139,7 @@
             if (graph) (void)hipGraphDestroy(graph);
             if (ev_gdone) (void)hipEventDestroy(ev_gdone);
             for (auto &e : ev_l1) if (e) (void)hipEventDestroy(e);
-            for (hipEvent_t e : {ev_fork, ev_join, ev_sortw, ev_main, ev_done, ev_chain}) if (e) (void)hipEventDestroy(e);
+            for (hipEvent_t e : {ev_fork, ev_join, ev_sortw, ev_main, ev_done, ev_chain, ev_hred}) if (e) (void)hipEventDestroy(e);
             for (auto &e : ev_tail) if (e) (void)hipEventDestroy(e);
             for (auto &e : ev) if (e) (void)hipEventDestroy(e);
             if (w1) (void)hipHostFree(w1);
@@ -156,9 +157,9 @@
     uint32_t batch = 1;
     struct LaneExtra {
         hipStream_t stream = nullptr, stream2 = nullptr;
-        DevBuf<Fr> abc, h;
+        DevBuf<Fr> abc;
         SortBufs sort_h;
-        uint64_t n_abc = 0, n_h = 0, nh_sort = 0;
+        uint64_t n_abc = 0, nh_sort = 0;
         uint32_t wbits = 0, batch = 1;
         uint32_t precomp = 0;
         bool one_stream = false;
@@ -171,13 +172,12 @@
                 else HIP_TRY(hipStreamCreateWithFlags(&stream2, hipStreamNonBlocking));
             }
             if (!abc.p) abc.alloc(n_abc);
-            if (!h.p) h.alloc(n_h);
             sort_h.alloc(nh_sort, wbits, precomp, batch);
             ready = true;
         }
         void release_memory() {
             ready = false;
-            abc.release(); h.release(); sort_h.release();
+            abc.release(); sort_h.release();
         }
         ~LaneExtra() {
             if (stream2 && stream2 != stream) { (void)hipStreamSynchronize(stream2); (void)hipStreamDestroy(stream2); }
@@ -186,6 +186,7 @@
     };
     static constexpr int MAX_LANES = 8;
     std::unique_ptr<LaneExtra> extra[MAX_LANES - 1];
+    hipEvent_t sort_h_reader[MAX_LANES] = {};
     int lanes = 1;
     uint32_t wbits = 0;
     bool part = false;
diff --git a/rapidsnark-old_amd/csrc/prover_pipeline.hip b/rapidsnark-old_amd/csrc/prover_pipeline.hip
--- a/rapidsnark-old_amd/csrc/prover_pipeline.hip
+++ b/rapidsnark-old_amd/csrc/prover_pipeline.hip
@@ -137,36 +137,40 @@
     hipStream_t s, s2, sf;
     hipStream_t tail[5] = {nullptr, nullptr, nullptr, nullptr, nullptr};
     int ntails = 0;
-    Fr *abc, *h;
+    Fr *abc;
     SortBufs *sort_h;
     bool tm;
     uint32_t tbw, tbh, Ww;
     uint64_t ew, eh;
     MsmPlan pw;
     G1Acc *bA, *bB1, *bC, *bH;
+    int lane;
+    const uint32_t *offs_w, *offs_h;
     PhaseCtx(zk_prover *p_, int si) : p(p_), q(p_->slot[si]) {
-        const int lane = si % p->lanes;
+        lane = si % p->lanes;
         if (lane == 0) {
             s = p->stream; s2 = p->stream2; sf = p->stream_fin;
             if (q.use_tails) {
                 for (int m = 0; m < 5; m++) tail[m] = p->tail[m];
                 ntails = p->tail_streams;
             }
-            abc = p->abc_use; h = p->h.p; sort_h = &p->sort_h;
+            abc = p->abc_use; sort_h = &p->sort_h;
         } else {
             zk_prover::LaneExtra &x = *p->extra[lane - 1];
             x.ensure();
             s = x.stream; s2 = x.stream2; sf = x.stream;
-            abc = x.abc.p; h = x.h.p; sort_h = &x.sort_h;
+            abc = x.abc.p; sort_h = &x.sort_h;
         }
         tm = (p->flags & ZK_FLAG_TIMINGS) != 0;
         tbw = q.sort_w.total_buckets(); tbh = p->sort_h.total_buckets();
         ew = q.sort_w.max_entries(); eh = p->sort_h.max_entries();
         pw = q.sort_w.plan; Ww = pw.sets * msm_wsum_rc(pw);
         bA = q.buckets_g1.p; bB1 = bA + tbw; bC = bB1 + tbw; bH = bC + tbw;
+        offs_w = msm_reduce_skips_empty(pw) ? q.sort_w.offsets.p : nullptr;
+        offs_h = msm_reduce_skips_empty(sort_h->plan) ? sort_h->offsets.p : nullptr;
     }
     void mark(int i) const { if (tm) HIP_TRY(hipEventRecord(q.ev[i], s)); }
-    AccumTail tail_of(int m) const { AccumTail t; t.stream = tail[m]; t.l1_done = q.ev_l1[m]; t.buckets_zeroed = q.zeroed; t.chunk_min = q.l1_chunk_min; t.chunk_max = q.l1_chunk_max; return t; }
+    AccumTail tail_of(int m) const { AccumTail t; t.stream = tail[m]; t.l1_done = q.ev_l1[m]; t.skip_clear = q.zeroed || (m == 3 ? offs_h : offs_w) != nullptr; t.chunk_min = q.l1_chunk_min; t.chunk_max = q.l1_chunk_max; return t; }
     hipStream_t after(int m, hipStream_t own) const { return tail[m] ? tail[m] : own; }
     NttTables tables() const { return NttTables{p->logn, p->tw_fwd.p, p->tw_inv.p, p->tw_coset.p, p->tw_ninv.p}; }
 };
@@ -191,8 +195,8 @@
     AccumTail t4 = c.tail_of(4);
     if (g2_aside) t4.stream = c.sf;
     launch_msm_accum_g2(q.buckets_g2.p, q.sort_w.offsets.p, q.sort_w.entries.p, p->ptsB2.p, 0, 0, tbw, ew, q.acc_ws_g2.p, q.acc_key[4], q.acc_flag[4], s2, tm ? &q.ev[10] : nullptr, t4);
-    if (tails) launch_msm_reduce_g2(q.wsum_g2.p, q.scratch_g2.p, q.buckets_g2.p, 1, pw, c.tail[4]);
-    else if (g2_aside) launch_msm_reduce_g2(q.wsum_g2.p, q.scratch_g2.p, q.buckets_g2.p, 1, pw, c.sf);
+    if (tails) launch_msm_reduce_g2(q.wsum_g2.p, q.scratch_g2.p, q.buckets_g2.p, 1, pw, c.tail[4], c.offs_w);
+    else if (g2_aside) launch_msm_reduce_g2(q.wsum_g2.p, q.scratch_g2.p, q.buckets_g2.p, 1, pw, c.sf, c.offs_w);
     if (p->batch_abc) {
         AccumBatch b;
         memset(&b, 0, sizeof b);
@@ -205,18 +209,18 @@
         b.ws_stride = q.acc_stride;
         launch_msm_accum_g1_batch(c.bA, q.sort_w.offsets.p, q.sort_w.entries.p, b, tbw, ew, q.acc_ws_g1[0], q.acc_key[0], q.acc_flag[0], s2, tm ? &q.ev[8] : nullptr, c.tail_of(0));
         if (tm) for (int e : {13, 14, 15, 16}) HIP_TRY(hipEventRecord(q.ev[e], s2));
-        launch_msm_reduce_g1(q.wsum_g1.p, q.scratch_g1.p, c.bA, 3, pw, c.after(0, s2));
-        if (!tails && !g2_aside) launch_msm_reduce_g2(q.wsum_g2.p, q.scratch_g2.p, q.buckets_g2.p, 1, pw, s2);
+        launch_msm_reduce_g1(q.wsum_g1.p, q.scratch_g1.p, c.bA, 3, pw, c.after(0, s2), c.offs_w);
+        if (!tails && !g2_aside) launch_msm_reduce_g2(q.wsum_g2.p, q.scratch_g2.p, q.buckets_g2.p, 1, pw, s2, c.offs_w);
         HIP_TRY(hipEventRecord(q.ev_join, s2));
     } else {
     launch_msm_accum_g1(c.bA, q.sort_w.offsets.p, q.sort_w.entries.p, p->ptsA.p, 0, 0, tbw, ew, q.acc_ws_g1[0], q.acc_key[0], q.acc_flag[0], s2, tm ? &q.ev[8] : nullptr, c.tail_of(0));
-    if (tails) launch_msm_reduce_g1(q.wsum_g1.p, q.scratch_g1.p, c.bA, 1, pw, c.tail[0]);
+    if (tails) launch_msm_reduce_g1(q.wsum_g1.p, q.scratch_g1.p, c.bA, 1, pw, c.tail[0], c.offs_w);
     launch_msm_accum_g1(c.bB1, q.sort_w.offsets.p, q.sort_w.entries.p, p->ptsB1.p, 0, 0, tbw, ew, q.acc_ws_g1[1], q.acc_key[1], q.acc_flag[1], s2, tm ? &q.ev[13] : nullptr, c.tail_of(1));
     if (tails) {
-        launch_msm_reduce_g1(q.wsum_g1.p + Ww, q.scratch_g1.p + msm_reduce_scratch_points(1, pw), c.bB1, 1, pw, c.tail[1]);
+        launch_msm_reduce_g1(q.wsum_g1.p + Ww, q.scratch_g1.p + msm_reduce_scratch_points(1, pw), c.bB1, 1, pw, c.tail[1], c.offs_w);
     } else {
-        if (!g2_aside) launch_msm_reduce_g2(q.wsum_g2.p, q.scratch_g2.p, q.buckets_g2.p, 1, pw, s2);
-        launch_msm_reduce_g1(q.wsum_g1.p, q.scratch_g1.p, c.bA, 2, pw, s2);
+        if (!g2_aside) launch_msm_reduce_g2(q.wsum_g2.p, q.scratch_g2.p, q.buckets_g2.p, 1, pw, s2, c.offs_w);
+        launch_msm_reduce_g1(q.wsum_g1.p, q.scratch_g1.p, c.bA, 2, pw, s2, c.offs_w);
     }
     HIP_TRY(hipEventRecord(q.ev_join, s2));
     }
@@ -275,11 +279,11 @@
 
     c.mark(0);
     q.zeroed = !p->capturing && !p->use_graph;
-    if (q.zeroed) {
+    if (q.zeroed && !c.offs_w) {
         HIP_TRY(hipMemsetAsync(c.bA, 0, (size_t)3 * c.tbw * sizeof(G1Acc), s2));
         HIP_TRY(hipMemsetAsync(q.buckets_g2.p, 0, (size_t)c.tbw * sizeof(G2Acc), s2));
-        HIP_TRY(hipMemsetAsync(c.bH, 0, (size_t)c.tbh * sizeof(G1Acc), s));
-    }
+    }
+    if (q.zeroed && !c.offs_h) HIP_TRY(hipMemsetAsync(c.bH, 0, (size_t)c.tbh * sizeof(G1Acc), s));
     if (staged) {
         HIP_TRY(hipStreamWaitEvent(s, q.ev_h2d, 0));
         HIP_TRY(hipStreamWaitEvent(s2, q.ev_h2d, 0));
@@ -361,18 +365,26 @@
     const uint64_t nl = p->nloc;
     Fr *abc = c.abc;
     if (p->part && !p->have_peers) launch_chunk_unpack(abc, p->pk_use, 3, p->logn, p->log_shards, s);
-    launch_abc_to_h(c.h, abc, abc + nl, abc + 2 * nl, nl, s, q.count, 3 * nl);
-    if (q.count < p->batch) HIP_TRY(hipMemsetAsync(c.h + nl * q.count, 0, (size_t)(p->batch - q.count) * nl * sizeof(Fr), s));
     c.mark(2);
-    c.sort_h->run(c.h + (p->part ? 0 : p->sh.lo), s);
+    if (p->sort_h_reader[c.lane] && !p->capturing) HIP_TRY(hipStreamWaitEvent(s, p->sort_h_reader[c.lane], 0));
+    {
+        const Fr *a0 = abc + (p->part ? 0 : p->sh.lo);
+        const MsmScalarSrc hsrc{nullptr, a0, a0 + nl, a0 + 2 * nl, 3 * nl, c.sort_h->n / p->batch * q.count};
+        c.sort_h->run(hsrc, s);
+    }
     c.mark(3);
     launch_msm_accum_g1(c.bH, c.sort_h->offsets.p, c.sort_h->entries.p, p->ptsH.p, 0, 0, c.tbh, c.eh, q.acc_ws_g1[3], q.acc_key[3], q.acc_flag[3], s, c.tm ? &q.ev[17] : nullptr, c.tail_of(3));
     c.mark(4);
-    launch_msm_reduce_g1(q.wsum_g1.p + 3 * c.Ww, q.scratch_g1.p + msm_reduce_scratch_points(3, c.pw), c.bH, 1, p->sort_h.plan, c.after(3, s));
+    launch_msm_reduce_g1(q.wsum_g1.p + 3 * c.Ww, q.scratch_g1.p + msm_reduce_scratch_points(3, c.pw), c.bH, 1, p->sort_h.plan, c.after(3, s), c.offs_h);
+    if (!p->capturing) {
+        const bool aside = c.offs_h && c.after(3, s) != s;
+        if (aside) HIP_TRY(hipEventRecord(q.ev_hred, c.after(3, s)));
+        p->sort_h_reader[c.lane] = aside ? q.ev_hred : nullptr;
+    }
     if (!p->batch_abc) {
     HIP_TRY(hipStreamWaitEvent(s, q.ev_sortw, 0));
     launch_msm_accum_g1(c.bC, q.sort_w.offsets.p, q.sort_w.entries.p, p->ptsC.p, p->c_idx_min, p->c_idx_min, c.tbw, c.ew, q.acc_ws_g1[2], q.acc_key[2], q.acc_flag[2], s, c.tm ? &q.ev[15] : nullptr, c.tail_of(2));
-    launch_msm_reduce_g1(q.wsum_g1.p + 2 * c.Ww, q.scratch_g1.p + msm_reduce_scratch_points(2, c.pw), c.bC, 1, c.pw, c.after(2, s));
+    launch_msm_reduce_g1(q.wsum_g1.p + 2 * c.Ww, q.scratch_g1.p + msm_reduce_scratch_points(2, c.pw), c.bC, 1, c.pw, c.after(2, s), c.offs_w);
     }
     c.mark(5);
     HIP_TRY(hipEventRecord(q.ev_main, s));
diff --git a/rapidsnark-old_amd/lib.py b/rapidsnark-old_amd/lib.py
--- a/rapidsnark-old_amd/lib.py
+++ b/rapidsnark-old_amd/lib.py
@@ -180,7 +180,7 @@
 
 EXPORTS = ["zk_last_error", "zk_device_count", "zk_prover_create", "zk_prover_destroy", "zk_prove", "zk_prove_dev",
            "zk_prove_dev_submit", "zk_prove_submit", "zk_prove_batch_submit", "zk_prove_batch_collect", "zk_host_alloc", "zk_host_free", "zk_prove_collect", "zk_prover_reserve", "zk_prover_info", "zk_prove_msm_collect", "zk_prove_msm_dev", "zk_prove_msm", "zk_prove_finish", "zk_prover_timings", "zk_fr_mul_vec",
-           "zk_fq_mul_vec", "zk_fr_coef_accumulate", "zk_fr_ntt", "zk_fr_abc_to_h", "zk_msm_g1", "zk_msm_g2", "zk_proof_to_json",
+           "zk_fq_mul_vec", "zk_fr_coef_accumulate", "zk_fr_ntt", "zk_fr_abc_to_h", "zk_msm_g1", "zk_msm_g2", "zk_msm_sort_dump", "zk_proof_to_json",
            "zk_public_to_json", "zk_synth_chain_g1", "zk_synth_chain_g2", "zk_fixed_base_g1", "zk_fixed_base_g2", "zk_g1_mul", "zk_g2_mul", "zk_assemble",
            "zk_multi_prover_create", "zk_multi_prover_destroy", "zk_multi_prove", "zk_multi_prove_submit", "zk_multi_prove_collect",
            "zk_multi_prover_info", "zk_multi_prover_shard_info", "zk_shard_info", "zk_shard_set_exchange", "zk_shard_begin", "zk_shard_step",
@@ -257,6 +257,8 @@
     lib.zk_fr_abc_to_h.argtypes = [u8p, u8p, u8p, C.c_uint64]
     lib.zk_msm_g1.argtypes = [u8p, u8p, u8p, C.c_uint64]
     lib.zk_msm_g2.argtypes = [u8p, u8p, u8p, C.c_uint64]
+    if hasattr(lib, "zk_msm_sort_dump"):
+        lib.zk_msm_sort_dump.argtypes = [u8p, C.c_uint64, C.c_uint32, C.c_uint32, C.c_int32, C.POINTER(C.c_uint64), C.c_void_p, C.c_void_p, C.c_void_p]
     lib.zk_synth_chain_g1.argtypes = [u8p, C.c_uint64, u8p, u8p]
     lib.zk_synth_chain_g2.argtypes = [u8p, C.c_uint64, u8p, u8p]
     lib.zk_fixed_base_g1.argtypes = [u8p, u8p, u8p, C.c_uint64]
@@ -415,6 +417,17 @@
     return out.tobytes()
 
 
+def msm_sort_dump(scalars, window_bits=0, table_mode=0, fuse_count=True):
+    scalars = _buf(scalars)
+    n = scalars.size // 32
+    lib = load_library()
+    sizes = (C.c_uint64 * 3)()
+    check(lib.zk_msm_sort_dump(_ptr(scalars), n, window_bits, table_mode, 1 if fuse_count else 0, sizes, None, None, None))
+    out = [np.zeros(int(s), dtype=np.uint32) for s in sizes]
+    check(lib.zk_msm_sort_dump(_ptr(scalars), n, window_bits, table_mode, 1 if fuse_count else 0, sizes, *[a.ctypes.data for a in out]))
+    return out[0], out[1][:int(out[0][-1])], out[2]
+
+
 def proof_to_json(proof_bytes):
     p = zk_proof.from_buffer_copy(bytes(proof_bytes))
     lib = load_library()
```

Result: no change. 30.27, median of 2 (+0.3%).
